# EdwardSmith1884/GEOMetrics

Measured on AMD Instinct MI355X. Metric: meshes/sec (sample+Chamfer+tri_dist+0N-GCN fwd+bwd), 2562 verts/3000 pts, higher is better.
Workload: dtype f32; 1 GPU; BASELINE config 5 shard: 8 independent 2562-vert/5120-face meshes per GPU, full loss (face sampling 3000 pts + Chamfer NN vs 3000 GT pts + tri_distance 3000x5120 + point-to-surface) on top of a 3-layer 0N-GCN 963-192-192-192, fwd+bwd, single process (no collective), Adam step; meshes_per_gpu=8, global_batch=8, parallelism=dp1, launch=hipgraph, gemm_selection=tunableop file

## Files before the change

geometrics_amd/aggregation.py:

```python
import torch
import torch.nn.functional as F

from . import _lib
from . import backward_pass as _pass
from . import fused as _fused
from .products import _new_like

ACT_NONE, ACT_RELU, ACT_ELU = 0, 1, 2


def activation_code(activation):
    if activation is F.relu or activation is torch.relu:
        return ACT_RELU
    if activation is F.elu:
        return ACT_ELU
    return ACT_NONE


def relu_mask(s, k):
    words = _lib.lib().geom_zn_gcn_relu_mask_words(*s.shape, k)
    return torch.empty(words, dtype=torch.int16, device=s.device) if words else None


def _table(csr, transposed):
    col, val, over = (csr.ell_col_t, csr.ell_val_t, csr.over_t) if transposed else (csr.ell_col, csr.ell_val, csr.over)
    return (csr.ell_w, _lib.ptr(col), _lib.ptr(val)) + tuple(map(_lib.ptr, over or (None, None, None)))


def _table_took(csr, name, *args):
    code = _lib.status(name, *args) if csr.ell_w else _lib.EUNSUPPORTED
    if code != _lib.EUNSUPPORTED:
        _lib.check(code, name)
    return code != _lib.EUNSUPPORTED


def forward(s, bias_c, csr, k, act, out, want_mask=False, head=None):
    b, nv, c = s.shape
    mask = relu_mask(s, k) if want_mask and act == ACT_RELU and csr.ell_w else None
    operands = (s.data_ptr(), _lib.ptr(bias_c), act, out.data_ptr())
    with torch.cuda.device(s.device):
        if head is not None:
            base, scale, pos = head
            _lib.call("geom_zn_gcn_aggregate_ell_head_fwd_f32", b, nv, c, k, *_table(csr, False), *operands, _lib.ptr(mask),
                      base.data_ptr(), float(scale), pos.data_ptr())
        elif not _table_took(csr, "geom_zn_gcn_aggregate_ell_fwd_f32", b, nv, c, k, *_table(csr, False), *operands, _lib.ptr(mask)):
            mask = None
            _lib.call("geom_zn_gcn_aggregate_fwd_f32", b, nv, c, k, csr.rowptr.data_ptr(), csr.col.data_ptr(), csr.val.data_ptr(),
                      *operands)
    return mask


def takes_product_below(below, csr, c, k, rows, needs_support):
    return bool(below is not None and below.wt is not None and below.wanted and needs_support and _fused.plan(rows)["bwd"]
                and below.wt.dim() == 2 and below.wt.shape[0] == c and _fused.supported(csr, c, k, below.wt.shape[1]))


def backward(g, csr, k, act, out, mask, want_bias, bias=None, arena=None, head=None, below=None):
    grad_pos, scale, (b, nv, c) = head if head is not None else (None, 0.0, g.shape)
    device = g.device if head is None else grad_pos.device
    grad_support = _new_like(g, "grad_support", arena, descending=True) if head is None \
        else torch.empty(b, nv, c, dtype=torch.float32, device=device)
    rows = _fused.partial_rows(b, nv) if below is not None else None
    bg = _pass.NO_BIAS_GRADIENT
    if want_bias:
        scratch = (rows, c) if below is not None else _lib.lib().geom_zn_gcn_bwd_scratch_floats(b, nv, c)
        bg = _pass.bias_gradient(bias, c, device, scratch, opted_in=arena is not None)
    ell_w = csr.ell_w
    results = (grad_support.data_ptr(), _lib.ptr(bg.now), _lib.ptr(bg.scratch))
    with torch.cuda.device(device):
        if below is not None:
            _fused.layer_backward(g, out, mask, csr, k, act, below.wt, g_out=grad_support, grad_in=below.take_dx(b, nv),
                                  colsum_partial=bg.scratch, grad_pos=grad_pos, head_scale=scale, shape=(b, nv, c))
            below.stamp(grad_support)
        elif head is not None:
            _lib.call("geom_zn_gcn_aggregate_ell_head_bwd_f32", b, nv, c, k, *_table(csr, True), grad_pos.data_ptr(), scale,
                      _lib.ptr(mask), act, *results)
        elif not _table_took(csr, "geom_zn_gcn_aggregate_ell_bwd_f32", b, nv, c, k, *_table(csr, True), g.data_ptr(), _lib.ptr(out),
                             _lib.ptr(mask), act, *results):
            ell_w = 0
            _lib.call("geom_zn_gcn_aggregate_bwd_f32", b, nv, c, k, csr.rowptr_t.data_ptr(), csr.col_t.data_ptr(),
                      csr.val_t.data_ptr(), g.data_ptr(), _lib.ptr(out), act, *results)
    if below is not None:
        bg.finish(rows)
    elif bg.defer:
        bg.finish(int(_lib.lib().geom_zn_gcn_bwd_partial_rows(b, nv, c, k, ell_w)))
    return grad_support, bg.out


def narrow_head_forward(s, bias_c, csr, k, act, base, scale, pos, want_sign):
    b, nv, c = s.shape
    sign = torch.empty(b * nv, dtype=torch.int16, device=s.device) if want_sign and act == ACT_RELU else None
    with torch.cuda.device(s.device):
        _lib.call("geom_zn_gcn_narrow_head_fwd_f32", b, nv, c, k, *_table(csr, False), s.data_ptr(), _lib.ptr(bias_c), act,
                  base.data_ptr(), float(scale), pos.data_ptr(), _lib.ptr(sign))
    return sign


def narrow_head_backward(grad_pos, scale, sign, csr, k, act, shape, want_bias, bias=None):
    b, nv, c = shape
    gs4 = torch.empty(b * nv, 4, dtype=torch.float32, device=grad_pos.device)
    rows = int(_lib.lib().geom_zn_gcn_bwd_partial_rows(b, nv, c, k, csr.ell_w))
    bg = _pass.bias_gradient(bias, c, grad_pos.device, (rows, c)) if want_bias else _pass.NO_BIAS_GRADIENT
    with torch.cuda.device(grad_pos.device):
        _lib.call("geom_zn_gcn_narrow_head_bwd_f32", b, nv, c, k, *_table(csr, True), grad_pos.data_ptr(), float(scale),
                  _lib.ptr(sign), act, gs4.data_ptr(), _lib.ptr(bg.scratch))
    bg.finish(rows)
    return gs4, bg.out
```

geometrics_amd/backward_pass.py:

```python
import contextlib
import ctypes
import threading
import types
import weakref
from collections import namedtuple

import torch

from . import _lib
from . import dense as _dense_kernels


_DEFAULTS = {"defer": False,
             "late": False,
             "collect": None}
switches = types.SimpleNamespace(
    ready_hooks=[],
    optimizer=None,
    zero_fill=False,
    **_DEFAULTS)
_entered = []
_entered_lock = threading.Lock()


@contextlib.contextmanager
def _switched(**values):
    with _entered_lock:
        _entered.append(values)
        _apply()
    try:
        yield
    finally:
        with _entered_lock:
            del _entered[next(i for i, entry in enumerate(_entered) if entry is values)]
            _apply()


def _apply():
    current = dict(_DEFAULTS)
    for values in _entered:
        current.update(values)
    for name, value in current.items():
        setattr(switches, name, value)


def deferred_parameter_gradients(enabled=True):
    return _switched(defer=enabled)


@contextlib.contextmanager
def late_input_gradients(on_parameter_gradients=None, enabled=True, collect=None):
    hooks = [on_parameter_gradients] if on_parameter_gradients is not None else []
    switches.ready_hooks.extend(hooks)
    try:
        with _switched(late=enabled, collect=collect):
            yield
    finally:
        for hook in hooks:
            switches.ready_hooks.remove(hook)


def set_optimizer(opt):
    prev, switches.optimizer = switches.optimizer, opt
    return prev


_gradient_targets = {}


def bind_gradient_targets(params, tensors):
    for p, t in zip(params, tensors):
        key = id(p)
        if t is None:
            _gradient_targets.pop(key, None)
            continue
        if t.shape != p.shape or t.dtype != p.dtype or t.device != p.device or not t.is_contiguous():
            raise ValueError("a gradient target must match its parameter's shape, dtype and device and be contiguous")
        _gradient_targets[key] = (weakref.ref(p, lambda _r, k=key: _gradient_targets.pop(k, None)), t)


def _gradient_buffer(param, like):
    hit = _gradient_targets.get(id(param)) if param is not None else None
    if (hit is not None and hit[0]() is param and hit[1].shape == like.shape and param.grad is None
            and _user_count(param) <= 1):
        return hit[1].detach()
    return torch.zeros_like(like) if switches.zero_fill else torch.empty_like(like)


_users = {}


def parameter_ref(param, node, needs_grad):
    if param is None:
        return None
    if needs_grad:
        key = id(param)
        entry = _users.get(key)
        if entry is None or entry[0]() is not param:
            entry = _users[key] = (weakref.ref(param, lambda _ref, k=key: _users.pop(k, None)), weakref.WeakSet())
        entry[1].add(node)
    return weakref.ref(param)


def _user_count(param):
    entry = _users.get(id(param))
    return len(entry[1]) if entry is not None and entry[0]() is param else 0


def _alias(t):
    return torch.empty(0, dtype=t.dtype, device=t.device).set_(t.untyped_storage(), t.storage_offset(), t.size(), t.stride())


def _engine_pass():
    return (hasattr(torch._C, "_current_graph_task_id") and torch._C._current_graph_task_id() >= 0
            and not torch.is_grad_enabled())


def may_defer(param, opted_in=False):
    if not (switches.defer or opted_in) or param is None or not _engine_pass():
        return False
    if not param.is_leaf or _user_count(param) > 1:
        return False
    return param.grad is None and not param._backward_hooks and not getattr(param, "_post_accumulate_grad_hooks", None)


def may_postpone_input_gradient(x):
    if not (switches.late and switches.defer) or not _engine_pass():
        return False
    return x.is_leaf and not x._backward_hooks and not getattr(x, "_post_accumulate_grad_hooks", None)


def _check_landed(param_ref, out):
    param = param_ref() if param_ref is not None else None
    if param is None or param.grad is None or param.grad.data_ptr() == out.data_ptr():
        return
    if param.grad.shape == out.shape or param.grad.numel() == out.numel():
        param.grad.copy_(out.view_as(param.grad))
    else:
        raise RuntimeError("geometrics_amd: a deferred parameter gradient did not reach its parameter (shape %s vs %s)"
                           % (tuple(param.grad.shape), tuple(out.shape)))


_Colsum = namedtuple("_Colsum", "partials rows cols out stream param")
_Reduce = namedtuple("_Reduce", "rows cin c workspace out stream param")
_Product = namedtuple("_Product", "x g out stream param launch_run")
_Late = namedtuple("_Late", "launch out stream leaf")


class _Pass:
    __slots__ = ("colsums", "reduces", "products", "late")

    def __init__(self):
        self.colsums, self.reduces, self.products, self.late = [], [], [], []

    def finish(self):
        colsums, reduces, self.colsums, self.reduces = self.colsums, self.reduces, [], []
        streams = {job.stream for job in colsums + reduces}
        if (reduces and colsums and len(streams) == 1 and all(job.cols % 4 == 0 for job in colsums)
                and 2 * len(reduces) + len(colsums) <= _lib.DENSE_MAX_REDUCE_JOBS):
            _launch_joint(reduces, colsums, streams.pop())
        else:
            _launch_colsums(colsums)
            _launch_reduces(reduces)
        products, self.products = self.products[::-1], []
        if products:
            products[0].launch_run(products)
        for job in reduces + colsums + products:
            _check_landed(job.param, job.out)
        for hook in list(switches.ready_hooks):
            hook()
        late, self.late, launches = self.late, [], []
        for job in late:
            launches.append(_on_stream(job.stream, job.launch))
            x = job.leaf()
            if x is not None and x.grad is None:
                x.grad = job.out.view(x.shape)
            elif x is not None:
                launches.append(_on_stream(job.stream, lambda x=x, out=job.out: x.grad.add_(out.view_as(x.grad))))
        if switches.collect is not None:
            switches.collect.extend(launches)
        else:
            for launch in launches:
                launch()


def _on_stream(stream, fn):
    def launch():
        with torch.cuda.stream(stream), torch.no_grad():
            fn()
    return launch


def _ints(seq):
    return (ctypes.c_int * len(seq))(*seq)


def _ptrs(tensors):
    return (ctypes.c_void_p * len(tensors))(*[t.data_ptr() for t in tensors])


def _colsum_args(jobs):
    return (len(jobs), _ptrs([j.partials for j in jobs]), _ints([j.rows for j in jobs]), _ints([j.cols for j in jobs]),
            _ptrs([j.out for j in jobs]))


def _by_stream(jobs):
    groups = {}
    for job in jobs:
        groups.setdefault(job.stream, []).append(job)
    return groups.items()


def _launch_colsums(jobs):
    for stream, group in _by_stream(jobs):
        with torch.cuda.device(stream.device):
            for c0 in range(0, len(group), _lib.COLSUM_MAX_JOBS):
                _lib.check(_lib.status("geom_colsum_batch_f32", *_colsum_args(group[c0:c0 + _lib.COLSUM_MAX_JOBS]),
                                       stream=stream.cuda_stream), "geom_colsum_batch_f32")


def _launch_reduces(jobs):
    for stream, group in _by_stream(jobs):
        _dense_kernels.reduce([(j.rows, j.cin, j.c, j.workspace, j.out, None) for j in group], stream.cuda_stream)


def _launch_joint(reduces, colsums, stream):
    weights = (len(reduces), _ints([j.rows for j in reduces]), _ints([j.cin for j in reduces]), _ints([j.c for j in reduces]),
               _ptrs([j.workspace for j in reduces]), _ptrs([j.out for j in reduces]))
    biases = _colsum_args(colsums)
    opt = switches.optimizer
    slots = None
    if opt is not None:
        index = {id(p): k for k, p in enumerate(opt.params)}
        slots = [index.get(id(job.param())) if job.param is not None else None for job in reduces + colsums]
        if None in slots or sorted(slots) != list(range(len(opt.params))) or opt.params[0].device != stream.device:
            slots = None
    with torch.cuda.device(stream.device):
        if slots is None:
            _lib.check(_lib.status("geom_dense_reduce2_f32", *weights, None, *biases, stream=stream.cuda_stream),
                       "geom_dense_reduce2_f32")
        else:
            pick = lambda seq, ks: _ptrs([seq[k] for k in ks])
            wk, bk = slots[:len(reduces)], slots[len(reduces):]
            params = [p.data for p in opt.params]
            _lib.check(_lib.status(
                "geom_dense_reduce_adam_f32",
                *weights, pick(params, wk), pick(opt.exp_avg, wk), pick(opt.exp_avg_sq, wk),
                *biases, pick(params, bk), pick(opt.exp_avg, bk), pick(opt.exp_avg_sq, bk), float(opt.lr), float(opt.betas[0]),
                float(opt.betas[1]), float(opt.eps), opt.state.data_ptr(), stream=stream.cuda_stream), "geom_dense_reduce_adam_f32")
            opt._stepped_in_backward = True


_passes = {}
_passes_lock = threading.Lock()


def _current():
    task = torch._C._current_graph_task_id()
    with _passes_lock:
        record = _passes.get(task)
        if record is not None:
            return record
        for stale in [t for t in _passes if t < task - 64]:
            del _passes[stale]
        record = _passes[task] = _Pass()
    torch.autograd.Variable._execution_engine.queue_callback(lambda: _finish(task, record))
    return record


def _finish(task, record):
    try:
        record.finish()
    finally:
        with _passes_lock:
            _passes.pop(task, None)


def pending(*kinds):
    with _passes_lock:
        return sum(len(getattr(record, kind)) for record in _passes.values() for kind in kinds or _Pass.__slots__)


class BiasGradient(namedtuple("BiasGradient", "out scratch defer bias")):
    __slots__ = ()

    @property
    def now(self):
        return None if self.defer else self.out

    def finish(self, rows):
        if self.out is None:
            return
        stream = torch.cuda.current_stream(self.out.device)
        if self.defer:
            _current().colsums.append(_Colsum(self.scratch, rows, self.out.shape[0], _alias(self.out), stream, weakref.ref(self.bias)))
        else:
            _launch_colsums([_Colsum(self.scratch, rows, self.out.shape[0], self.out, stream, None)])


NO_BIAS_GRADIENT = BiasGradient(None, None, False, None)


def bias_gradient(bias, c, device, scratch_shape, opted_in=False):
    out = _gradient_buffer(bias, bias) if bias is not None and bias.shape == (c,) and bias.dtype == torch.float32 \
        else torch.empty(c, dtype=torch.float32, device=device)
    scratch = torch.empty(scratch_shape, dtype=torch.float32, device=device)
    return BiasGradient(out, scratch, may_defer(bias, opted_in), bias)


def weight_gradient(param_ref, w, rows, cin, c, workspace):
    param = param_ref()
    out = _gradient_buffer(param, w)
    if may_defer(param):
        stream = torch.cuda.current_stream(w.device)
        _current().reduces.append(_Reduce(rows, cin, c, workspace, _alias(out).view(cin, c), stream, param_ref))
    else:
        _dense_kernels.reduce([(rows, cin, c, workspace, out.view(cin, c), None)])
    return out


def postpone_weight_product(x, g, out, param_ref, launch_run):
    _current().products.append(_Product(x, g, _alias(out).view(x.shape[1], g.shape[1]), torch.cuda.current_stream(out.device),
                                        param_ref, launch_run))


def postpone_input_gradient(launch, out, leaf):
    _current().late.append(_Late(launch, out, torch.cuda.current_stream(out.device), weakref.ref(leaf)))
```

geometrics_amd/csrc/dense_gemm.hip:

```cpp
#include "buffer_access.h"
#include "adam_math.h"
#include <type_traits>

namespace {

using geom::f32x4;
using geom::f3u;
typedef float f32x2 __attribute__((ext_vector_type(2)));
struct __attribute__((packed, aligned(4))) f4u { float x, y, z, w; };

constexpr int DG_THREADS = 256;
constexpr int DG_WAVES = 4;
constexpr int DG_BK = 32;
constexpr int DG_KS = 8;
constexpr int SPLIT_RB = 6;
constexpr int SPLIT_RB_NARROW = 3;
constexpr int LD_TC = 34;

__host__ __device__ constexpr int ld_rc(int r) { return ((r + 15) / 32) * 32 + 16; }

#ifndef DG_PROBE_NO_FETCH
#define DG_PROBE_NO_FETCH 0
#endif
#ifndef DG_PROBE_NO_ISSUE
#define DG_PROBE_NO_ISSUE 0
#endif
#ifndef DG_PROBE_NO_STORE
#define DG_PROBE_NO_STORE 0
#endif
#ifndef DG_PROBE_NO_BARRIER
#define DG_PROBE_NO_BARRIER 0
#endif
#ifndef DG_PROBE_NO_G
#define DG_PROBE_NO_G 0
#endif
constexpr bool DG_FETCH = !DG_PROBE_NO_FETCH, DG_ISSUE = !DG_PROBE_NO_ISSUE, DG_STORE = !DG_PROBE_NO_STORE,
               DG_BARRIER = !DG_PROBE_NO_BARRIER, DG_G = !DG_PROBE_NO_G;


template <int W>
using ldg_t = std::conditional_t<W == 4, f32x4, std::conditional_t<W == 3, f3u, float>>;
template <int W>
__device__ __forceinline__ ldg_t<W> ldg(const float *base, unsigned byte_off)
{
    const char *p = reinterpret_cast<const char *>(base) + byte_off;
    if constexpr (W == 4) {
        const f4u v = *reinterpret_cast<const f4u *>(p);
        return (f32x4){v.x, v.y, v.z, v.w};
    } else {
        return *reinterpret_cast<const ldg_t<W> *>(p);
    }
}

template <int R, int W>
struct PanelTC {
    static constexpr int WIDTH = W, TPR = 32 / W, ROWS = DG_THREADS / TPR;
    static constexpr int PASSES = (R + ROWS - 1) / ROWS;
    static constexpr bool EXACT = R % ROWS == 0;
    static_assert(W == 4 || EXACT, "the 4-byte form covers whole passes");
    ldg_t<W> v[2][PASSES];
    unsigned off[PASSES];
    template <typename RowOff>
    __device__ __forceinline__ void prepare(RowOff rowoff, unsigned )
    {
#pragma unroll
        for (int p = 0; p < PASSES; ++p) {
            const int r = p * ROWS + threadIdx.x / TPR;
            off[p] = ((unsigned)rowoff(W == 1 || r < R ? r : R - 1) + (threadIdx.x % TPR) * W) * 4u;
        }
    }
    static __device__ __forceinline__ const float *stage_base(const float *g, unsigned , int t0) { return g + t0; }
    static __device__ __forceinline__ unsigned stage_limit(unsigned total, unsigned , int t0) { return (total - W - (unsigned)t0) * 4u; }
    template <int SET>
    __device__ __forceinline__ void issue_pass(int p, const float *base, unsigned limit) { v[SET][p] = ldg<W>(base, min(off[p], limit)); }
    template <bool ZERO, int SET>
    __device__ __forceinline__ void store_pass(int p, float *lds, int t0, int tmax) const
    {
        const int tl = (threadIdx.x % TPR) * W;
        const int r = p * ROWS + threadIdx.x / TPR;
        if (EXACT || r < R) {
            const bool tin = !ZERO || t0 + tl < tmax;
            float *d = lds + r * LD_TC + tl;
            if constexpr (W == 4) {
                reinterpret_cast<float2 *>(d)[0] = make_float2(tin ? v[SET][p][0] : 0.f, tin ? v[SET][p][1] : 0.f);
                reinterpret_cast<float2 *>(d)[1] = make_float2(tin ? v[SET][p][2] : 0.f, tin ? v[SET][p][3] : 0.f);
            } else {
                *d = tin ? v[SET][p] : 0.f;
            }
        }
    }
};

template <int R, int W>
struct PanelRC {
    static constexpr int WIDTH = W, Q = R / W;
    static constexpr int PASSES = (32 * Q + DG_THREADS - 1) / DG_THREADS;
    static constexpr bool EXACT = (32 * Q) % DG_THREADS == 0;
    ldg_t<W> v[2][PASSES];
    unsigned off[PASSES];
    template <typename ColOff>
    __device__ __forceinline__ void prepare(ColOff coloff, unsigned ld)
    {
#pragma unroll
        for (int p = 0; p < PASSES; ++p) {
            const int e = threadIdx.x + p * DG_THREADS;
            const int tl = EXACT ? e / Q : min(e / Q, 31);
            off[p] = ((unsigned)tl * ld + (unsigned)coloff((e % Q) * W)) * 4u;
        }
    }
    static __device__ __forceinline__ const float *stage_base(const float *g, unsigned ld, int t0) { return g + (int64_t)t0 * ld; }
    static __device__ __forceinline__ unsigned stage_limit(unsigned total, unsigned ld, int t0) { return (total - W - (unsigned)t0 * ld) * 4u; }
    template <int SET>
    __device__ __forceinline__ void issue_pass(int p, const float *base, unsigned limit) { v[SET][p] = ldg<W>(base, min(off[p], limit)); }
    template <bool ZERO, int SET>
    __device__ __forceinline__ void store_pass(int p, float *lds, int t0, int tmax) const
    {
        const int e = threadIdx.x + p * DG_THREADS;
        const int tl = EXACT ? e / Q : min(e / Q, 31);
        ldg_t<W> x = v[SET][p];
        if (ZERO && !(t0 + tl < tmax)) x = ldg_t<W>{};
        *reinterpret_cast<ldg_t<W> *>(lds + tl * ld_rc(R) + (e % Q) * W) = x;
    }
};

template <int RB, int NCW, bool EXTRA>
struct Frags {
    float a[2][RB + 1], b[2][NCW + 1];
};

template <int RB, int NCW, bool A_TC, bool B_TC, int RA, int RBW, bool EXTRA>
__device__ __forceinline__ void fetch_frags(Frags<RB, NCW, EXTRA> &f, int buf, const float *la, const float *lb, int s, int wave,
                                            int xcb)
{
    const int x = threadIdx.x & 15, g = (threadIdx.x >> 4) & 3;
    const float *pa = A_TC ? la + x * LD_TC + g : la + g * ld_rc(RA) + x;
    const float *pb = B_TC ? lb + (wave * NCW * 16 + x) * LD_TC + g : lb + g * ld_rc(RBW) + wave * NCW * 16 + x;
#pragma unroll
    for (int i = 0; i < RB; ++i) f.a[buf][i] = A_TC ? pa[i * 16 * LD_TC + 4 * s] : pa[4 * s * ld_rc(RA) + i * 16];
#pragma unroll
    for (int j = 0; j < NCW; ++j) f.b[buf][j] = B_TC ? pb[j * 16 * LD_TC + 4 * s] : pb[4 * s * ld_rc(RBW) + j * 16];
    if (EXTRA) {
        const float *pbx = B_TC ? lb + (xcb * 16 + x) * LD_TC + g : lb + g * ld_rc(RBW) + xcb * 16 + x;
        f.a[buf][RB] = A_TC ? pa[RB * 16 * LD_TC + 4 * s] : pa[4 * s * ld_rc(RA) + RB * 16];
        f.b[buf][NCW] = B_TC ? pbx[4 * s] : pbx[4 * s * ld_rc(RBW)];
    }
}

struct StageIO {
    int st_t0, st_tmax;
    const float *a_base, *b_base;
    unsigned a_limit, b_limit;
};

template <int RB, int NCW, bool A_TC, bool B_TC, int RA, int RBW, bool EXTRA, int A_FLOATS, int SET, class PA, class PB, class Tail>
__device__ __forceinline__ void gemm_stage(const float *cur, float *wr, f32x4 (&acc)[RB][NCW], f32x4 &accx,
                                           Frags<RB, NCW, EXTRA> &f, PA &pa, PB &pb, const StageIO &io, int wave, int xcb,
                                           Tail tail)
{
    constexpr int U = PA::PASSES + PB::PASSES;
#pragma unroll
    for (int s = 0; s < DG_KS; ++s) {
        if (DG_FETCH && s + 1 < DG_KS) fetch_frags<RB, NCW, A_TC, B_TC, RA, RBW, EXTRA>(f, (s + 1) & 1, cur, cur + A_FLOATS, s + 1, wave, xcb);
        else if (DG_FETCH) fetch_frags<RB, NCW, A_TC, B_TC, RA, RBW, EXTRA>(f, 0, wr, wr + A_FLOATS, 0, wave, xcb);
        if (DG_ISSUE && s < 4) {
#pragma unroll
            for (int u = s * U / 4; u < (s + 1) * U / 4; ++u) {
                if (u < PA::PASSES) pa.template issue_pass<SET>(u, io.a_base, io.a_limit);
                else pb.template issue_pass<SET>(u - PA::PASSES, io.b_base, io.b_limit);
            }
        } else if (DG_STORE && s >= 4 && s < 7) {
#pragma unroll
            for (int u = (s - 4) * U / 3; u < (s - 3) * U / 3; ++u) {
                if (u < PA::PASSES) pa.template store_pass<true, SET ^ 1>(u, wr, io.st_t0, io.st_tmax);
                else pb.template store_pass<false, SET ^ 1>(u - PA::PASSES, wr + A_FLOATS, io.st_t0, io.st_tmax);
            }
        }
        if (s == DG_KS - 1) tail();
#pragma unroll
        for (int i = 0; i < RB; ++i)
#pragma unroll
            for (int j = 0; j < NCW; ++j)
                acc[i][j] = __builtin_amdgcn_mfma_f32_16x16x4f32(f.b[s & 1][j], f.a[s & 1][i], acc[i][j], 0, 0, 0);
        if (EXTRA) accx = __builtin_amdgcn_mfma_f32_16x16x4f32(f.b[s & 1][NCW], f.a[s & 1][RB], accx, 0, 0, 0);
#pragma unroll
        for (int m = 0; m < RB * NCW + (EXTRA ? 1 : 0); ++m) {
            __builtin_amdgcn_sched_group_barrier(0x008, 1, 0);
            __builtin_amdgcn_sched_group_barrier(0x100, 1, 0);
            if (s < 4) __builtin_amdgcn_sched_group_barrier(0x020, 1, 0);
            else __builtin_amdgcn_sched_group_barrier(0x200, 1, 0);
            __builtin_amdgcn_sched_group_barrier(0x006, 2, 0);
        }
        __builtin_amdgcn_sched_barrier(0);
        if (s == 6) {
            if (DG_BARRIER) __syncthreads();
            __builtin_amdgcn_sched_barrier(0);
        }
    }
}

enum { EPI_PLAIN = 0, EPI_ZN = 1 };

struct RowArgs {
    const float *a;
    int64_t lda;
    const float *b;
    int64_t ldb;
    float *c;
    int64_t ldc;
    int I, J, T;
    int n_tiles;
    int left_rb;
    int n_chunks;
    int ksplit;
    float *sup;
    const float *bias;
    unsigned short *mask;
};

template <int RB, int NCW, bool B_TC, bool A_VEC, int EPI, bool HAS_X>
__device__ __forceinline__ void rows_body(const RowArgs &q, float *lds, const int w, const int G)
{
    constexpr int RA = (RB + 1) * 16;
    constexpr int RAL = HAS_X ? RA : RB * 16;
    constexpr int CW = NCW * 64;
    constexpr int A_FLOATS = RA * LD_TC;
    constexpr int B_FLOATS = B_TC ? CW * LD_TC : 32 * ld_rc(CW);
    constexpr int BUF = A_FLOATS + B_FLOATS;
    const int wave = threadIdx.x >> 6;
    const int xrow0 = HAS_X ? (q.n_tiles * RB + w / NCW) * 16 : 0;
    const int xcb = (w % NCW) * DG_WAVES + wave;
    const int nst = (q.T + DG_BK - 1) / DG_BK;
    int my_tiles = w < q.n_tiles ? (q.n_tiles - 1 - w) / G + 1 : 0;
    if (my_tiles == 0 && HAS_X) my_tiles = 1;
    const int total = my_tiles * q.n_chunks * nst;
    if (total == 0) return;

    typedef PanelTC<RAL, A_VEC ? 4 : 1> PA;
    typedef typename std::conditional<B_TC, PanelTC<CW, 4>, PanelRC<CW, 4>>::type PB;
    PA pa;
    PB pb;
    const unsigned a_total = (unsigned)q.I * (unsigned)q.lda;
    const unsigned b_total = B_TC ? (unsigned)q.J * (unsigned)q.ldb : (unsigned)q.T * (unsigned)q.ldb;
    int l_tile = w, l_chunk = 0, l_st = 0, l_count = 0;
    auto prepare_a = [&]() {
        const int tile = l_tile;
        pa.prepare([=](int r) -> unsigned {
            int row = r < RB * 16 ? (tile < q.n_tiles ? tile : 0) * RB * 16 + r : xrow0 + (r - RB * 16);
            row = row < q.I ? row : q.I - 1;
            return (unsigned)row * (unsigned)q.lda;
        }, (unsigned)q.lda);
    };
    auto prepare_b = [&]() {
        const int j0 = l_chunk * CW;
        if constexpr (B_TC) {
            pb.prepare([=](int r) -> unsigned { const int j = j0 + r; return (unsigned)(j < q.J ? j : q.J - 1) * (unsigned)q.ldb; }, (unsigned)q.ldb);
        } else {
            pb.prepare([=](int r) -> unsigned { const int j = j0 + r; return (unsigned)(j < q.J ? j : q.J - 4); }, (unsigned)q.ldb);
        }
    };
    StageIO io;
    auto aim = [&]() {
        io.a_base = PA::stage_base(q.a, (unsigned)q.lda, l_st * DG_BK);
        io.a_limit = PA::stage_limit(a_total, (unsigned)q.lda, l_st * DG_BK);
        io.b_base = PB::stage_base(q.b, (unsigned)q.ldb, l_st * DG_BK);
        io.b_limit = PB::stage_limit(b_total, (unsigned)q.ldb, l_st * DG_BK);
    };
    bool wrapped = false;
    auto step = [&]() {
        const int more = l_count + 1 < total ? 1 : 0;
        l_count += more;
        const int nl = l_st + more;
        wrapped = nl == nst;
        l_st = wrapped ? 0 : nl;
    };
    auto rewire = [&]() {
        if (!wrapped) return;
        if (++l_chunk == q.n_chunks) {
            l_chunk = 0, l_tile += G;
            prepare_a();
        }
        if (q.n_chunks > 1) prepare_b();
    };
    auto advance = [&]() { step(); rewire(); };
    prepare_a();
    prepare_b();
    aim();
#pragma unroll
    for (int p = 0; p < PA::PASSES; ++p) pa.template issue_pass<0>(p, io.a_base, io.a_limit);
#pragma unroll
    for (int p = 0; p < PB::PASSES; ++p) pb.template issue_pass<0>(p, io.b_base, io.b_limit);
    advance();
    aim();
    io.st_t0 = l_st * DG_BK;
#pragma unroll
    for (int p = 0; p < PA::PASSES; ++p) pa.template issue_pass<1>(p, io.a_base, io.a_limit);
#pragma unroll
    for (int p = 0; p < PB::PASSES; ++p) pb.template issue_pass<1>(p, io.b_base, io.b_limit);
#pragma unroll
    for (int p = 0; p < PA::PASSES; ++p) pa.template store_pass<true, 0>(p, lds, 0, q.T);
#pragma unroll
    for (int p = 0; p < PB::PASSES; ++p) pb.template store_pass<false, 0>(p, lds + A_FLOATS, 0, q.T);
    advance();
    aim();
    io.st_tmax = q.T;
    __syncthreads();
    Frags<RB, NCW, HAS_X> fr;
    fetch_frags<RB, NCW, true, B_TC, RA, CW, HAS_X>(fr, 0, lds, lds + A_FLOATS, 0, wave, xcb);

    const int x = threadIdx.x & 15, g = (threadIdx.x >> 4) & 3;
    f32x4 acc[RB][NCW], accx = {0.f, 0.f, 0.f, 0.f};
#pragma unroll
    for (int i = 0; i < RB; ++i)
#pragma unroll
        for (int j = 0; j < NCW; ++j) acc[i][j] = (f32x4){0.f, 0.f, 0.f, 0.f};
    int c_tile = w, c_chunk = 0, c_st = 0, c_pass = 0;
    int buf = 0;

    auto after_stage = [&]() {
        rewire();
        if (++c_st < nst) return;
        c_st = 0;
        const int j0 = c_chunk * CW;
        auto emit = [&](const f32x4 &val, int row, int cb) {
            const int j = j0 + cb * 16 + 4 * g;
            if (row >= q.I || j >= q.J) return;
            f32x4 v = val;
            if (EPI == EPI_ZN) {
                if (j < q.ksplit) {
                    *reinterpret_cast<f32x4 *>(q.sup + (int64_t)row * q.ksplit + j) = v;
                    return;
                }
                const f32x4 bb = q.bias ? *reinterpret_cast<const f32x4 *>(q.bias + j) : (f32x4){0.f, 0.f, 0.f, 0.f};
                unsigned bits = 0u;
#pragma unroll
                for (int r = 0; r < 4; ++r) {
                    const float t = v[r] + bb[r];
                    v[r] = t > 0.f ? t : 0.f;
                    bits |= (t > 0.f ? 1u : 0u) << r;
                }
                if (q.mask) {
                    unsigned m = bits << (4 * g);
                    m |= __shfl_xor(m, 16);
                    m |= __shfl_xor(m, 32);
                    if (g == 0) q.mask[(int64_t)row * (q.J >> 4) + (j >> 4)] = (unsigned short)m;
                }
            }
            float *dst = q.c + (int64_t)row * q.ldc + j;
            if (j + 3 < q.J) {
                *reinterpret_cast<f4u *>(dst) = f4u{v[0], v[1], v[2], v[3]};
            } else {
#pragma unroll
                for (int r = 0; r < 4; ++r)
                    if (j + r < q.J) dst[r] = v[r];
            }
        };
        if (c_tile < q.n_tiles) {
#pragma unroll
            for (int i = 0; i < RB; ++i)
#pragma unroll
                for (int jj = 0; jj < NCW; ++jj) emit(acc[i][jj], (c_tile * RB + i) * 16 + x, wave * NCW + jj);
        }
        if (HAS_X && c_pass == 0) emit(accx, xrow0 + x, xcb);
#pragma unroll
        for (int i = 0; i < RB; ++i)
#pragma unroll
            for (int jj = 0; jj < NCW; ++jj) acc[i][jj] = (f32x4){0.f, 0.f, 0.f, 0.f};
        accx = (f32x4){0.f, 0.f, 0.f, 0.f};
        if (++c_chunk == q.n_chunks) c_chunk = 0, c_tile += G, ++c_pass;
    };

    for (int it = 0; it < total; it += 2) {
        {
            const float *cur = lds + buf * BUF;
            float *wr = lds + (buf ^ 1) * BUF;
            gemm_stage<RB, NCW, true, B_TC, RA, CW, HAS_X, A_FLOATS, 0>(cur, wr, acc, accx, fr, pa, pb, io, wave, xcb, [&]() {
                io.st_t0 = l_st * DG_BK;
                step();
                aim();
                buf ^= 1;
            });
            after_stage();
        }
        if (it + 1 < total) {
            const float *cur = lds + buf * BUF;
            float *wr = lds + (buf ^ 1) * BUF;
            gemm_stage<RB, NCW, true, B_TC, RA, CW, HAS_X, A_FLOATS, 1>(cur, wr, acc, accx, fr, pa, pb, io, wave, xcb, [&]() {
                io.st_t0 = l_st * DG_BK;
                step();
                aim();
                buf ^= 1;
            });
            after_stage();
        }
    }
}

template <int RB, int NCW, bool B_TC, bool A_VEC, int EPI>
__global__ __launch_bounds__(DG_THREADS) void dense_rows_kernel(RowArgs q)
{
    constexpr int RA = (RB + 1) * 16;
    constexpr int CW = NCW * 64;
    __shared__ __attribute__((aligned(16))) float lds[2 * (RA * LD_TC + (B_TC ? CW * LD_TC : 32 * ld_rc(CW)))];
    if ((int)blockIdx.x < q.left_rb * NCW) rows_body<RB, NCW, B_TC, A_VEC, EPI, true>(q, lds, blockIdx.x, gridDim.x);
    else rows_body<RB, NCW, B_TC, A_VEC, EPI, false>(q, lds, blockIdx.x, gridDim.x);
}

struct SplitArgs {
    const float *a;
    int64_t lda;
    const float *b;
    int64_t ldb;
    float *part;
    int I, J, T;
    int full_tiles, s_full, left_rb, s_left;
    float *colsum;
};

template <int RB>
__device__ __forceinline__ int split_row(int i, int x)
{
    constexpr int N4 = RB / 4, N2 = (RB % 4) / 2;
    if (i < 4 * N4) return 64 * (i >> 2) + 4 * x + (i & 3);
    if (i < 4 * N4 + 2 * N2) return 64 * N4 + 2 * x + (i - 4 * N4);
    return 64 * N4 + 32 * N2 + x;
}

template <int RB>
__device__ __forceinline__ void split_frags(float (&f)[RB], const float *row, int x)
{
    constexpr int N4 = RB / 4, N2 = (RB % 4) / 2, N1 = RB % 2;
#pragma unroll
    for (int q = 0; q < N4; ++q) {
        const f32x4 v = *reinterpret_cast<const f32x4 *>(row + 64 * q + 4 * x);
        f[4 * q] = v[0], f[4 * q + 1] = v[1], f[4 * q + 2] = v[2], f[4 * q + 3] = v[3];
    }
    if constexpr (N2 == 1) {
        const f32x2 v = *reinterpret_cast<const f32x2 *>(row + 64 * N4 + 2 * x);
        f[4 * N4] = v[0], f[4 * N4 + 1] = v[1];
    }
    if constexpr (N1 == 1) f[RB - 1] = row[64 * N4 + 32 * N2 + x];
}

template <int RB, int RA, int A_FLOATS, int SET, class PA, class Tail>
__device__ __forceinline__ void split_stage(const float *cur, float *wr, f32x4 (&acc)[RB][3], float (&fa)[2][RB], f3u (&bq)[2][DG_KS],
                                            PA &pa, const StageIO &io, unsigned b_lane, unsigned b_step, Tail tail)
{
    constexpr int U = PA::PASSES;
    constexpr int KS = DG_KS;
    constexpr int LOADS = KS / 2;
    constexpr int STORES = KS - 1 - LOADS;
    const int x = threadIdx.x & 15, g = (threadIdx.x >> 4) & 3;
    const float *b_base = io.b_base;
    const unsigned b_limit = io.b_limit;
#pragma unroll
    for (int s = 0; s < KS; ++s) {
        if (DG_FETCH) {
            const float *src = s + 1 < KS ? cur : wr;
            const int sn = s + 1 < KS ? s + 1 : 0;
            split_frags<RB>(fa[(s + 1) & 1], src + (4 * sn + g) * ld_rc(RA), x);
        }
        if (DG_ISSUE && s < LOADS) {
#pragma unroll
            for (int u = s * U / LOADS; u < (s + 1) * U / LOADS; ++u) pa.template issue_pass<SET>(u, io.a_base, io.a_limit);
        } else if (DG_STORE && s >= LOADS && s < KS - 1) {
#pragma unroll
            for (int u = (s - LOADS) * U / STORES; u < (s - LOADS + 1) * U / STORES; ++u)
                pa.template store_pass<true, SET ^ 1>(u, wr, io.st_t0, io.st_tmax);
        }
        if (s == KS - 1) tail();
        const f3u b = bq[SET][s];
#pragma unroll
        for (int i = 0; i < RB; ++i) {
            acc[i][0] = __builtin_amdgcn_mfma_f32_16x16x4f32(b.x, fa[s & 1][i], acc[i][0], 0, 0, 0);
            acc[i][1] = __builtin_amdgcn_mfma_f32_16x16x4f32(b.y, fa[s & 1][i], acc[i][1], 0, 0, 0);
            acc[i][2] = __builtin_amdgcn_mfma_f32_16x16x4f32(b.z, fa[s & 1][i], acc[i][2], 0, 0, 0);
        }
        if (DG_G) bq[SET][s] = ldg<3>(b_base, min(b_lane + (unsigned)s * b_step, b_limit));
#pragma unroll
        for (int m = 0; m < RB * 3; ++m) {
            __builtin_amdgcn_sched_group_barrier(0x008, 1, 0);
            __builtin_amdgcn_sched_group_barrier(0x100, 1, 0);
            if (s < LOADS) __builtin_amdgcn_sched_group_barrier(0x020, 1, 0);
            else __builtin_amdgcn_sched_group_barrier(0x200, 1, 0);
            __builtin_amdgcn_sched_group_barrier(0x006, 2, 0);
        }
        __builtin_amdgcn_sched_barrier(0);
        if (s == KS - 2) {
            if (DG_BARRIER) __syncthreads();
            __builtin_amdgcn_sched_barrier(0);
        }
    }
}

template <int RB, int RBP, bool A_VEC>
__device__ __forceinline__ void split_body(const SplitArgs &q, float *lds, int i0, int split, int nsplit, int slot, bool want_cs)
{
    constexpr int RA = RB * 16;
    constexpr int CW = 192;
    constexpr int A_FLOATS = 32 * ld_rc(RA);
    constexpr int BUF = A_FLOATS;
    constexpr int KS = DG_KS;
    const int wave = threadIdx.x >> 6;
    const int x = threadIdx.x & 15, g = (threadIdx.x >> 4) & 3;
    const int n4 = (q.T + 3) / 4;
    const int t_begin = (int)((int64_t)n4 * split / nsplit) * 4;
    const int t_end = min((int)((int64_t)n4 * (split + 1) / nsplit) * 4, q.T);
    const int nst = (t_end - t_begin + DG_BK - 1) / DG_BK;

    f32x4 acc[RB][3];
#pragma unroll
    for (int i = 0; i < RB; ++i)
#pragma unroll
        for (int j = 0; j < 3; ++j) acc[i][j] = (f32x4){0.f, 0.f, 0.f, 0.f};
    float cs0 = 0.f, cs1 = 0.f, cs2 = 0.f;

    typedef PanelRC<RA, A_VEC ? 4 : 1> PA;
    PA pa;
    if (nst > 0) {
        pa.prepare([=](int r) -> unsigned { const int i = i0 + r; return (unsigned)(i + PA::WIDTH - 1 < q.I ? i : q.I - PA::WIDTH); }, (unsigned)q.lda);
        const unsigned a_total = (unsigned)q.T * (unsigned)q.lda, b_total = (unsigned)q.T * (unsigned)q.ldb;
        const int jc = min(wave * 48 + 3 * x, q.J - 3);
        const unsigned b_step = 4u * (unsigned)q.ldb * 4u;
        const unsigned b_lane = ((unsigned)g * (unsigned)q.ldb + (unsigned)jc) * 4u;
        StageIO io;
        int l_st = 0;
        auto aim = [&]() {
            const int t0 = t_begin + l_st * DG_BK;
            io.a_base = PA::stage_base(q.a, (unsigned)q.lda, t0);
            io.a_limit = PA::stage_limit(a_total, (unsigned)q.lda, t0);
            io.b_base = q.b + (int64_t)t0 * q.ldb;
            io.b_limit = (b_total - 3u - (unsigned)t0 * (unsigned)q.ldb) * 4u;
        };
        auto advance = [&]() { l_st = l_st + 1 < nst ? l_st + 1 : l_st; };
        f3u bq[2][KS];
        float fa[2][RB];
        aim();
#pragma unroll
        for (int p = 0; p < PA::PASSES; ++p) pa.template issue_pass<0>(p, io.a_base, io.a_limit);
#pragma unroll
        for (int s = 0; s < KS; ++s) bq[0][s] = ldg<3>(io.b_base, min(b_lane + (unsigned)s * b_step, io.b_limit));
        advance();
        aim();
        io.st_t0 = t_begin + l_st * DG_BK;
#pragma unroll
        for (int p = 0; p < PA::PASSES; ++p) pa.template issue_pass<1>(p, io.a_base, io.a_limit);
#pragma unroll
        for (int s = 0; s < KS; ++s) bq[1][s] = ldg<3>(io.b_base, min(b_lane + (unsigned)s * b_step, io.b_limit));
#pragma unroll
        for (int p = 0; p < PA::PASSES; ++p) pa.template store_pass<true, 0>(p, lds, t_begin, t_end);
        advance();
        aim();
        io.st_tmax = t_end;
        __syncthreads();
        split_frags<RB>(fa[0], lds + g * ld_rc(RA), x);
        int buf = 0;
        auto tail = [&]() {
            io.st_t0 = t_begin + l_st * DG_BK;
            advance();
            aim();
            buf ^= 1;
        };
        auto colsum_stage = [&](const f3u (&b)[KS], int st) {
            const int t0 = t_begin + st * DG_BK + g;
#pragma unroll
            for (int s = 0; s < KS; ++s) {
                const bool in = t0 + 4 * s < t_end;
                cs0 += in ? b[s].x : 0.f, cs1 += in ? b[s].y : 0.f, cs2 += in ? b[s].z : 0.f;
            }
        };
        for (int st = 0; st < nst; st += 2) {
            {
                const float *cur = lds + buf * BUF;
                float *wr = lds + (buf ^ 1) * BUF;
                if (want_cs) colsum_stage(bq[0], st);
                split_stage<RB, RA, A_FLOATS, 0>(cur, wr, acc, fa, bq, pa, io, b_lane, b_step, tail);
            }
            if (st + 1 < nst) {
                const float *cur = lds + buf * BUF;
                float *wr = lds + (buf ^ 1) * BUF;
                if (want_cs) colsum_stage(bq[1], st + 1);
                split_stage<RB, RA, A_FLOATS, 1>(cur, wr, acc, fa, bq, pa, io, b_lane, b_step, tail);
            }
        }
    }
    float *dst = q.part + (int64_t)slot * (RBP * 16) * CW;
    const int j0 = wave * 48 + 12 * g;
#pragma unroll
    for (int i = 0; i < RB; ++i) {
        float e[12];
#pragma unroll
        for (int r = 0; r < 4; ++r)
#pragma unroll
            for (int u = 0; u < 3; ++u) e[3 * r + u] = acc[i][u][r];
        f32x4 *d = reinterpret_cast<f32x4 *>(dst + split_row<RB>(i, x) * CW + j0);
        d[0] = (f32x4){e[0], e[1], e[2], e[3]};
        d[1] = (f32x4){e[4], e[5], e[6], e[7]};
        d[2] = (f32x4){e[8], e[9], e[10], e[11]};
    }
    if (want_cs) {
        float t0 = cs0, t1 = cs1, t2 = cs2;
#pragma unroll
        for (int k = 1; k < 4; ++k) {
            t0 += __shfl(cs0, x + 16 * k), t1 += __shfl(cs1, x + 16 * k), t2 += __shfl(cs2, x + 16 * k);
        }
        const int j = wave * 48 + 3 * x;
        if (g == 0 && j + 2 < q.J) {
            float *o = q.colsum + (int64_t)split * q.J + j;
            o[0] = t0, o[1] = t1, o[2] = t2;
        }
    }
}

template <int RB, int NCW, bool A_VEC>
__device__ __forceinline__ void split_dispatch(const SplitArgs &q, float *lds, const int w)
{
    static_assert(NCW == 3, "the split body owns 48 columns per wave");
    const int nfull = q.full_tiles * q.s_full;
    if (w < nfull) {
        const int tile = w % q.full_tiles, split = w / q.full_tiles;
        split_body<RB, RB, true>(q, lds, tile * RB * 16, split, q.s_full, tile * q.s_full + split, q.colsum != nullptr && tile == 0);
    } else {
        const int e = (w - nfull) / q.s_left, split = (w - nfull) % q.s_left;
        split_body<1, RB, A_VEC>(q, lds, (q.full_tiles * RB + e) * 16, split, q.s_left, w, false);
    }
}

template <int RB, int NCW, bool A_VEC>
__global__ __launch_bounds__(DG_THREADS) void dense_split_kernel(SplitArgs q)
{
    __shared__ __attribute__((aligned(16))) float lds[2 * 32 * ld_rc(RB * 16)];
    split_dispatch<RB, NCW, A_VEC>(q, lds, blockIdx.x);
}

template <int RB, int SRB, bool X_VEC>
__global__ __launch_bounds__(DG_THREADS, 2) void dense_bwd_pair_kernel(RowArgs r, SplitArgs q, int n_row)
{
    constexpr int LDS_ROWS = 2 * ((RB + 1) * 16 * LD_TC + 192 * LD_TC);
    constexpr int LDS_SPLIT = 2 * 32 * ld_rc(SRB * 16);
    __shared__ __attribute__((aligned(16))) float lds[LDS_ROWS > LDS_SPLIT ? LDS_ROWS : LDS_SPLIT];
    const int w = blockIdx.x;
    if (w < n_row) {
        if (w < r.left_rb * 3) rows_body<RB, 3, true, true, EPI_PLAIN, true>(r, lds, w, n_row);
        else rows_body<RB, 3, true, true, EPI_PLAIN, false>(r, lds, w, n_row);
    } else {
        split_dispatch<SRB, 3, X_VEC>(q, lds, w - n_row);
    }
}

constexpr int NP_CW = 192;
constexpr int NP_RA = SPLIT_RB_NARROW * 16;
constexpr int NP_CHUNK = 128;
constexpr int NP_DX_ROWS = 64;
struct NarrowPairArgs {
    const float *x;
    const float *g4;
    const float *w;
    float *grad_x;
    float *part;
    int rows, full_tiles, s_full;
};

__device__ __forceinline__ void narrow_dw_role(const NarrowPairArgs &q, const int w)
{
    constexpr int XP = NP_CHUNK * (NP_RA / 4) / DG_THREADS;
    static_assert(NP_CHUNK * (NP_RA / 4) % DG_THREADS == 0 && NP_CHUNK <= DG_THREADS, "whole staging passes");
    __shared__ __attribute__((aligned(16))) float xs[2][NP_CHUNK * NP_RA];
    __shared__ f32x4 gs[2][NP_CHUNK];
    const int tid = threadIdx.x;
    const int tile = w % q.full_tiles, split = w / q.full_tiles;
    const int slot = tile * q.s_full + split, i0 = tile * NP_RA;
    const int n4 = (q.rows + 3) / 4;
    const int t_begin = (int)((int64_t)n4 * split / q.s_full) * 4;
    const int t_end = min((int)((int64_t)n4 * (split + 1) / q.s_full) * 4, q.rows);
    const int nch = (t_end - t_begin + NP_CHUNK - 1) / NP_CHUNK;
    float *dst = q.part + (int64_t)slot * NP_RA * NP_CW;

    f32x4 xr[XP], gr = {0.f, 0.f, 0.f, 0.f};
    auto load = [&](int ch) {
        const int t0 = t_begin + ch * NP_CHUNK;
#pragma unroll
        for (int p = 0; p < XP; ++p) {
            const int e = p * DG_THREADS + tid;
            const int t = min(t0 + e / (NP_RA / 4), q.rows - 1);
            xr[p] = *reinterpret_cast<const f32x4 *>(q.x + (int64_t)t * NP_CW + i0 + (e % (NP_RA / 4)) * 4);
        }
        if (tid < NP_CHUNK) gr = *reinterpret_cast<const f32x4 *>(q.g4 + (int64_t)min(t0 + tid, q.rows - 1) * 4);
    };
    if (nch > 0) load(0);
    for (int e = tid; e < NP_RA * (NP_CW / 4); e += DG_THREADS)
        if (e % (NP_CW / 4) != 0) *reinterpret_cast<f32x4 *>(dst + (int64_t)e * 4) = (f32x4){0.f, 0.f, 0.f, 0.f};
    float a0 = 0.f, a1 = 0.f, a2 = 0.f;
    for (int ch = 0; ch < nch; ++ch) {
        const int buf = ch & 1;
#pragma unroll
        for (int p = 0; p < XP; ++p) {
            const int e = p * DG_THREADS + tid;
            *reinterpret_cast<f32x4 *>(&xs[buf][(e / (NP_RA / 4)) * NP_RA + (e % (NP_RA / 4)) * 4]) = xr[p];
        }
        if (tid < NP_CHUNK) gs[buf][tid] = gr;
        __syncthreads();
        if (ch + 1 < nch) load(ch + 1);
        if (tid < NP_RA) {
            const int n = min(NP_CHUNK, t_end - (t_begin + ch * NP_CHUNK));
#pragma unroll 8
            for (int t = 0; t < n; ++t) {
                const float xv = xs[buf][t * NP_RA + tid];
                const f32x4 gv = gs[buf][t];
                a0 = __builtin_fmaf(xv, gv[0], a0);
                a1 = __builtin_fmaf(xv, gv[1], a1);
                a2 = __builtin_fmaf(xv, gv[2], a2);
            }
        }
    }
    if (tid < NP_RA) *reinterpret_cast<f32x4 *>(dst + (int64_t)tid * NP_CW) = (f32x4){a0, a1, a2, 0.f};
}

__device__ __forceinline__ void narrow_dx_role(const NarrowPairArgs &q, const int w)
{
    constexpr int GROUPS = NP_CW / 4;
    constexpr int PASSES = NP_DX_ROWS * GROUPS / DG_THREADS;
    constexpr int CLASSES = 3;
    static_assert((DG_THREADS * CLASSES) % GROUPS == 0 && PASSES % CLASSES == 0, "the column groups of a thread repeat every 3 passes");
    const int tid = threadIdx.x;
    const int64_t row0 = (int64_t)w * NP_DX_ROWS;
    float wr[CLASSES][4][3];
#pragma unroll
    for (int cl = 0; cl < CLASSES; ++cl) {
        const int cg = (cl * DG_THREADS + tid) % GROUPS;
#pragma unroll
        for (int i = 0; i < 4; ++i) {
            const f32x4 v = *reinterpret_cast<const f32x4 *>(q.w + (int64_t)(4 * cg + i) * NP_CW);
            wr[cl][i][0] = v[0], wr[cl][i][1] = v[1], wr[cl][i][2] = v[2];
        }
    }
#pragma unroll
    for (int p = 0; p < PASSES; ++p) {
        const int e = p * DG_THREADS + tid;
        const int64_t row = row0 + e / GROUPS;
        const int cg = e % GROUPS;
        if (row < q.rows) {
            const f32x4 gv = *reinterpret_cast<const f32x4 *>(q.g4 + row * 4);
            f32x4 o;
#pragma unroll
            for (int i = 0; i < 4; ++i) {
                const float *wi = wr[p % CLASSES][i];
                o[i] = __builtin_fmaf(gv[2], wi[2], __builtin_fmaf(gv[1], wi[1], __builtin_fmaf(gv[0], wi[0], 0.f)));
            }
            *reinterpret_cast<f32x4 *>(q.grad_x + row * NP_CW + 4 * cg) = o;
        }
    }
}

__global__ __launch_bounds__(DG_THREADS) void dense_bwd_narrow_kernel(NarrowPairArgs q, int n_split)
{
    const int w = blockIdx.x;
    if (w < n_split) narrow_dw_role(q, w);
    else narrow_dx_role(q, w - n_split);
}

struct ReduceJob {
    const float *part;
    float *out;
    int I, J, RA, CW, full_tiles, s_full, s_left;
    int outs;
};
struct ReduceJobs {
    ReduceJob job[GEOM_DENSE_MAX_REDUCE_JOBS];
    int first[GEOM_DENSE_MAX_REDUCE_JOBS + 1];
    int n;
};
struct ReduceAdam {
    float *p[GEOM_DENSE_MAX_REDUCE_JOBS], *m[GEOM_DENSE_MAX_REDUCE_JOBS], *v[GEOM_DENSE_MAX_REDUCE_JOBS];
    float lr, b1, b2, eps;
    float *state;
    int vec;
};

constexpr int RED_THREADS = 256;
inline int reduce_outs(int slots) { return slots <= 32 ? 64 : slots <= 64 ? 32 : slots <= 128 ? 16 : slots <= 256 ? 8 : 4; }
__device__ __forceinline__ void reduce_body(const ReduceJobs &jobs, const ReduceAdam &adam, const int block, const int nblocks,
                                            f32x4 *part, float *st)
{
    float *const state = adam.state;
    int jb = 0;
    while (jb + 1 < jobs.n && block >= jobs.first[jb + 1]) ++jb;
    const ReduceJob q = jobs.job[jb];
    const int bx = block - jobs.first[jb];
    const int jq = q.J >> 2;
    const int outs = q.outs, groups = RED_THREADS / outs;
    float s_t = 0.f, s_b1 = 0.f, s_b2 = 0.f;
    if (state && threadIdx.x == 0) {
        s_t = __hip_atomic_load(state + 0, __ATOMIC_RELAXED, __HIP_MEMORY_SCOPE_AGENT);
        s_b1 = __hip_atomic_load(state + 1, __ATOMIC_RELAXED, __HIP_MEMORY_SCOPE_AGENT);
        s_b2 = __hip_atomic_load(state + 2, __ATOMIC_RELAXED, __HIP_MEMORY_SCOPE_AGENT);
    }
    const int o = threadIdx.x % outs, sg = threadIdx.x / outs;
    const int e = bx * outs + o;
    const bool live = e < q.I * jq;
    f32x4 t = {0.f, 0.f, 0.f, 0.f};
    int i = 0, j = 0;
    if (live) {
        i = e / jq, j = (e % jq) * 4;
        int tile = i / q.RA, il = i % q.RA;
        const bool full = tile < q.full_tiles;
        const int n = full ? q.s_full : q.s_left;
        int slot0 = tile * q.s_full;
        if (!full) {
            const int r = i - q.full_tiles * q.RA;
            slot0 = q.full_tiles * q.s_full + (r >> 4) * q.s_left, il = r & 15;
        }
        const int64_t pitch = (int64_t)q.RA * q.CW;
        const float *p = q.part + ((int64_t)slot0 * q.RA + il) * q.CW + j;
        const int s0 = (int)((int64_t)n * sg / groups), s1 = (int)((int64_t)n * (sg + 1) / groups);
        for (int s = s0; s < s1; s += 8) {
            f32x4 a[8];
#pragma unroll
            for (int k = 0; k < 8; ++k)
                if (s + k < s1) a[k] = *reinterpret_cast<const f32x4 *>(p + (int64_t)(s + k) * pitch);
#pragma unroll
            for (int k = 0; k < 8; ++k)
                if (s + k < s1) t = t + a[k];
        }
    }
    const int64_t at = (int64_t)i * q.J + j;
    float *pp = state ? adam.p[jb] : nullptr;
    const bool vec = pp && adam.vec;
    f32x4 a = {0.f, 0.f, 0.f, 0.f}, bm = a, cv = a;
    if (vec && sg == 0 && live) {
        a = *reinterpret_cast<const f32x4 *>(pp + at);
        bm = *reinterpret_cast<const f32x4 *>(adam.m[jb] + at);
        cv = *reinterpret_cast<const f32x4 *>(adam.v[jb] + at);
    }
    part[sg * outs + o] = t;
    if (state && threadIdx.x == 0) st[0] = s_t, st[1] = s_b1, st[2] = s_b2;
    __syncthreads();
    geom::AdamStep as{};
    if (state) as = geom::adam_step_from(st, adam.lr, adam.b1, adam.b2);
    if (sg == 0 && live) {
        f32x4 r = part[o];
        for (int k = 1; k < groups; ++k) r = r + part[k * outs + o];
        float *dst = q.out + at;
        if (vec) {
            f32x4 *p4 = reinterpret_cast<f32x4 *>(pp + at), *m4 = reinterpret_cast<f32x4 *>(adam.m[jb] + at),
                  *v4 = reinterpret_cast<f32x4 *>(adam.v[jb] + at);
#pragma unroll
            for (int k = 0; k < 4; ++k) {
                float pa = a[k], pb = bm[k], pc = cv[k];
                geom::adam_update(pa, r[k], pb, pc, adam.b1, adam.b2, adam.eps, 1.f, as.step_size, as.bc2_sqrt);
                a[k] = pa, bm[k] = pb, cv[k] = pc;
            }
            *reinterpret_cast<f32x4 *>(dst) = r;
            *m4 = bm, *v4 = cv, *p4 = a;
        } else {
            dst[0] = r[0], dst[1] = r[1], dst[2] = r[2], dst[3] = r[3];
            if (pp) {
                float *pm = adam.m[jb] + at, *pv = adam.v[jb] + at;
                pp += at;
#pragma unroll
                for (int k = 0; k < 4; ++k) {
                    float a = pp[k], b = pm[k], c = pv[k];
                    geom::adam_update(a, r[k], b, c, adam.b1, adam.b2, adam.eps, 1.f, as.step_size, as.bc2_sqrt);
                    pm[k] = b, pv[k] = c, pp[k] = a;
                }
            }
        }
    }
    if (state) geom::adam_arrive(state, as, block, nblocks);
}

__global__ __launch_bounds__(RED_THREADS) void dense_reduce_kernel(ReduceJobs jobs, ReduceAdam adam)
{
    __shared__ f32x4 part[RED_THREADS];
    __shared__ float st[3];
    reduce_body(jobs, adam, blockIdx.x, gridDim.x, part, st);
}


int num_cus()
{
    static int cus = 0;
    if (!cus) {
        int dev = 0;
        hipDeviceProp_t prop;
        if (hipGetDevice(&dev) == hipSuccess && hipGetDeviceProperties(&prop, dev) == hipSuccess) cus = prop.multiProcessorCount;
        if (cus <= 0) cus = 256;
    }
    return cus;
}

struct RowGeo {
    int rb, n_tiles, left_rb, grid;
};
RowGeo row_geometry(int rows, int ncw, int cus)
{
    const int n_rb = (rows + 15) / 16;
    RowGeo best{0, 0, 0, 0};
    long best_cost = -1;
    const int cand[] = {5, 6, 4, 3, 2, 1};
    for (int rb : cand) {
        int n_tiles = n_rb / rb, left = n_rb % rb;
        if (left * ncw > cus || (n_tiles == 0 && left == 0)) continue;
        const int grid = n_tiles < cus ? (n_tiles > left * ncw ? n_tiles : left * ncw) : cus;
        if (grid <= 0) continue;
        const int passes = (n_tiles + grid - 1) / grid;
        const long cost = (long)(passes > 0 ? passes : 1) * rb * ncw + (left ? 1 : 0);
        if (best_cost < 0 || cost < best_cost) best = RowGeo{rb, n_tiles, left, grid}, best_cost = cost;
    }
    return best;
}

template <int LO, int HI, class Launch>
int dispatch_rb(int rb, Launch launch)
{
    if constexpr (LO <= HI) {
        if (rb != LO) return dispatch_rb<LO + 1, HI>(rb, launch);
        launch(std::integral_constant<int, LO>{});
        return geom::launch_status();
    } else {
        return GEOM_EINVAL;
    }
}

template <int NCW, bool B_TC, bool A_VEC, int EPI>
int launch_rows_rb(const RowArgs &q, const RowGeo &geo, hipStream_t s)
{
    return dispatch_rb<1, 6>(geo.rb, [&](auto rb) {
        hipLaunchKernelGGL((dense_rows_kernel<decltype(rb)::value, NCW, B_TC, A_VEC, EPI>), dim3(geo.grid), dim3(DG_THREADS), 0, s, q);
    });
}

inline bool aligned16(const void *p) { return ((uintptr_t)p & 15) == 0; }

RowArgs input_gradient_args(int rows, int cin, int c, const float *g, const float *w, float *grad_x, int ncw, const RowGeo &geo)
{
    return RowArgs{g, c, w, c, grad_x, cin, rows, cin, c, geo.n_tiles, geo.left_rb, (cin + ncw * 64 - 1) / (ncw * 64), 0, nullptr,
                   nullptr, nullptr};
}

struct SplitGeo {
    int rb, full_tiles, left_rb, s_full, s_left, slots;
    int64_t partial_floats() const { return (int64_t)slots * rb * 16 * 192; }
    int64_t colsum_offset() const { return partial_floats(); }
};
inline int split_rb(int cin) { return cin <= 192 ? SPLIT_RB_NARROW : SPLIT_RB; }
SplitGeo split_geometry(int cin, int rows, int cus)
{
    SplitGeo g;
    g.rb = split_rb(cin);
    const int ra = g.rb * 16;
    g.full_tiles = cin / ra;
    g.left_rb = (cin % ra + 15) / 16;
    const int n4 = (rows + 3) / 4;
    g.s_full = g.full_tiles ? (int)((int64_t)cus * g.rb / (g.full_tiles * g.rb + g.left_rb)) : 0;
    if (g.full_tiles && g.s_full < 1) g.s_full = 1;
    g.s_left = 0;
    if (g.left_rb) {
        const int rest = cus - g.full_tiles * g.s_full;
        g.s_left = rest / g.left_rb > 0 ? rest / g.left_rb : 1;
    }
    if (g.s_full > n4) g.s_full = n4;
    if (g.s_left > n4) g.s_left = n4;
    g.slots = g.full_tiles * g.s_full + g.left_rb * g.s_left;
    return g;
}

SplitArgs split_args(int rows, int cin, int c, const float *x, const float *g, float *workspace, bool want_colsum, const SplitGeo &geo)
{
    return SplitArgs{x, cin, g, c, workspace, cin, c, rows, geo.full_tiles, geo.s_full, geo.left_rb, geo.s_left,
                     want_colsum ? workspace + geo.colsum_offset() : nullptr};
}

int check_backward(bool dx, bool dw, int rows, int cin, int c, const float *x, const float *g, const float *w, const float *grad_x,
                   const float *workspace)
{
    if (rows < (dw ? 1 : 0) || cin <= 0 || c <= 0) return GEOM_EINVAL;
    if ((dw ? c % 12 != 0 || c > 192 : c % 4 != 0) || (int64_t)rows * (cin > c ? cin : c) >= (1LL << 30)) return GEOM_EUNSUPPORTED;
    if (rows == 0) return 0;
    if (!g || !aligned16(g)) return GEOM_EINVAL;
    if (dx && (!w || !grad_x || !aligned16(w))) return GEOM_EINVAL;
    if (dw && (!x || !workspace || !aligned16(workspace))) return GEOM_EINVAL;
    return 0;
}

}

extern "C" int geom_dense_fwd_f32(int rows, int cin, int c, const float *x, const float *w, int ksplit, const float *bias,
                                  float *out, float *sup, uint16_t *mask, void *stream)
{
    if (rows < 0 || cin <= 0 || c <= 0) return GEOM_EINVAL;
    if (c % 16 != 0 || c > 192 || (int64_t)rows * cin >= (1LL << 30)) return GEOM_EUNSUPPORTED;
    if (rows == 0) return 0;
    if (!x || !w || !out || !aligned16(w) || !aligned16(out)) return GEOM_EINVAL;
    const bool zn = ksplit > 0;
    if (zn && (ksplit % 16 != 0 || ksplit >= c || !sup || !aligned16(sup) || (bias && !aligned16(bias)))) return GEOM_EINVAL;
    const RowGeo geo = row_geometry(rows, 3, num_cus());
    RowArgs q{x, cin, w, c, out, c, rows, c, cin, geo.n_tiles, geo.left_rb, 1, zn ? ksplit : 0, sup, bias, mask};
    hipStream_t s = static_cast<hipStream_t>(stream);
    const bool avec = cin % 4 == 0 && aligned16(x);
    if (zn) return avec ? launch_rows_rb<3, false, true, EPI_ZN>(q, geo, s) : launch_rows_rb<3, false, false, EPI_ZN>(q, geo, s);
    return avec ? launch_rows_rb<3, false, true, EPI_PLAIN>(q, geo, s) : launch_rows_rb<3, false, false, EPI_PLAIN>(q, geo, s);
}

extern "C" int geom_dense_bwd_input_f32(int rows, int cin, int c, const float *g, const float *w, float *grad_x, void *stream)
{
    const int code = check_backward(true, false, rows, cin, c, nullptr, g, w, grad_x, nullptr);
    if (code || rows == 0) return code;
    hipStream_t s = static_cast<hipStream_t>(stream);
    const int ncw = cin > 192 ? 4 : 3;
    const RowGeo geo = row_geometry(rows, ncw, num_cus());
    const RowArgs q = input_gradient_args(rows, cin, c, g, w, grad_x, ncw, geo);
    return ncw == 4 ? launch_rows_rb<4, true, true, EPI_PLAIN>(q, geo, s) : launch_rows_rb<3, true, true, EPI_PLAIN>(q, geo, s);
}

extern "C" int64_t geom_dense_bwd_weight_workspace_floats(int rows, int cin, int c)
{
    if (rows <= 0 || cin <= 0 || c <= 0 || c > 192) return 0;
    const SplitGeo g = split_geometry(cin, rows, num_cus());
    return g.partial_floats() + (int64_t)(g.s_full > 0 ? g.s_full : g.s_left) * c;
}

extern "C" int geom_dense_bwd_weight_f32(int rows, int cin, int c, const float *x, const float *g, float *workspace,
                                         int want_colsum, void *stream)
{
    const int code = check_backward(false, true, rows, cin, c, x, g, nullptr, nullptr, workspace);
    if (code) return code;
    const SplitGeo geo = split_geometry(cin, rows, num_cus());
    if (want_colsum && geo.full_tiles == 0) return GEOM_EUNSUPPORTED;
    const SplitArgs q = split_args(rows, cin, c, x, g, workspace, want_colsum != 0, geo);
    const dim3 grid(geo.slots), block(DG_THREADS);
    hipStream_t s = static_cast<hipStream_t>(stream);
    const bool xvec = cin % 4 == 0 && aligned16(x);
    if (geo.rb == SPLIT_RB_NARROW) {
        if (xvec) hipLaunchKernelGGL((dense_split_kernel<SPLIT_RB_NARROW, 3, true>), grid, block, 0, s, q);
        else hipLaunchKernelGGL((dense_split_kernel<SPLIT_RB_NARROW, 3, false>), grid, block, 0, s, q);
    } else {
        if (xvec) hipLaunchKernelGGL((dense_split_kernel<SPLIT_RB, 3, true>), grid, block, 0, s, q);
        else hipLaunchKernelGGL((dense_split_kernel<SPLIT_RB, 3, false>), grid, block, 0, s, q);
    }
    return geom::launch_status();
}

extern "C" int geom_dense_bwd_f32(int rows, int cin, int c, const float *x, const float *g, const float *w, float *grad_x,
                                  float *workspace, int want_colsum, void *stream)
{
    int code = check_backward(true, true, rows, cin, c, x, g, w, grad_x, workspace);
    if (code) return code;
    const int cus = num_cus();
    const bool xvec = cin % 4 == 0 && aligned16(x);
    const RowGeo rg = row_geometry(rows, 3, cus);
    const SplitGeo sg = split_geometry(cin, rows, cus);
    if (cin > 192 || !xvec || (want_colsum && sg.full_tiles == 0) || rg.rb < 2 || rg.rb > 5) {
        code = geom_dense_bwd_input_f32(rows, cin, c, g, w, grad_x, stream);
        if (code) return code;
        return geom_dense_bwd_weight_f32(rows, cin, c, x, g, workspace, want_colsum, stream);
    }
    const RowArgs r = input_gradient_args(rows, cin, c, g, w, grad_x, 3, rg);
    const SplitArgs q = split_args(rows, cin, c, x, g, workspace, want_colsum != 0, sg);
    hipStream_t s = static_cast<hipStream_t>(stream);
    static_assert(SPLIT_RB_NARROW == 3, "cin <= 192 (the pair mode's range) takes the narrow split tiles");
    return dispatch_rb<2, 5>(rg.rb, [&](auto rb) {
        hipLaunchKernelGGL((dense_bwd_pair_kernel<decltype(rb)::value, SPLIT_RB_NARROW, true>), dim3(rg.grid + sg.slots),
                           dim3(DG_THREADS), 0, s, r, q, rg.grid);
    });
}

extern "C" int geom_dense_bwd_narrow_f32(int rows, int cin, int c, const float *x, const float *g4, const float *w, float *grad_x,
                                         float *workspace, void *stream)
{
    if (rows < 1 || cin <= 0 || c <= 0) return GEOM_EINVAL;
    if (cin != NP_CW || c != NP_CW || (int64_t)rows * NP_CW >= (1LL << 30)) return GEOM_EUNSUPPORTED;
    if (!x || !g4 || !workspace || !aligned16(x) || !aligned16(g4) || !aligned16(workspace)) return GEOM_EINVAL;
    if (grad_x && (!w || !aligned16(w) || !aligned16(grad_x))) return GEOM_EINVAL;
    const SplitGeo sg = split_geometry(cin, rows, num_cus());
    if (sg.rb != SPLIT_RB_NARROW || sg.left_rb != 0 || sg.full_tiles < 1) return GEOM_EUNSUPPORTED;
    const NarrowPairArgs q{x, g4, w, grad_x, workspace, rows, sg.full_tiles, sg.s_full};
    const int n_dx = grad_x ? (rows + NP_DX_ROWS - 1) / NP_DX_ROWS : 0;
    hipLaunchKernelGGL(dense_bwd_narrow_kernel, dim3(sg.slots + n_dx), dim3(DG_THREADS), 0, static_cast<hipStream_t>(stream), q, sg.slots);
    return geom::launch_status();
}

namespace {
void flat_grid(ReduceJobs &jobs, int n)
{
    jobs.n = n;
    jobs.first[0] = 0;
    for (int j = 0; j < n; ++j) {
        ReduceJob &q = jobs.job[j];
        q.outs = reduce_outs(q.s_full > q.s_left ? q.s_full : q.s_left);
        jobs.first[j + 1] = jobs.first[j] + (q.I * (q.J >> 2) + q.outs - 1) / q.outs;
    }
}

inline bool bad_layer(const float *workspace, const float *grad_w, int rows, int cin, int c)
{
    return !workspace || !grad_w || rows <= 0 || cin <= 0 || c <= 0 || c > 192 || c % 4;
}

int build_reduce_jobs(ReduceJobs &jobs, int count, const int *rows, const int *cin, const int *c, const float *const *workspaces,
                      float *const *grad_w, int ncs, const float *const *cs_partials, const int *cs_rows, const int *cs_cols,
                      float *const *cs_outs)
{
    if (count < 0 || ncs < 0) return GEOM_EINVAL;
    if (count && (!rows || !cin || !c || !workspaces || !grad_w)) return GEOM_EINVAL;
    if (ncs && (!cs_partials || !cs_rows || !cs_cols || !cs_outs)) return GEOM_EINVAL;
    if (count + ncs > GEOM_DENSE_MAX_REDUCE_JOBS) return GEOM_ETOOBIG;
    int n = 0;
    for (int l = 0; l < count; ++l) {
        if (bad_layer(workspaces[l], grad_w[l], rows[l], cin[l], c[l])) return GEOM_EINVAL;
        const SplitGeo g = split_geometry(cin[l], rows[l], num_cus());
        jobs.job[n++] = ReduceJob{workspaces[l], grad_w[l], cin[l], c[l], g.rb * 16, 192, g.full_tiles, g.s_full, g.s_left, 0};
    }
    for (int i = 0; i < ncs; ++i) {
        if (!cs_partials[i] || !cs_outs[i] || cs_rows[i] < 0 || cs_cols[i] <= 0 || cs_cols[i] % 4) return GEOM_EINVAL;
        jobs.job[n++] = ReduceJob{cs_partials[i], cs_outs[i], 1, cs_cols[i], 1, cs_cols[i], 1, cs_rows[i], 0, 0};
    }
    flat_grid(jobs, n);
    return 0;
}

int launch_reduce(const ReduceJobs &jobs, const ReduceAdam &adam, void *stream)
{
    hipLaunchKernelGGL(dense_reduce_kernel, dim3(jobs.first[jobs.n]), dim3(RED_THREADS), 0, static_cast<hipStream_t>(stream), jobs, adam);
    return geom::launch_status();
}
}

extern "C" int geom_dense_reduce2_f32(int count, const int *rows, const int *cin, const int *c, const float *const *workspaces,
                                      float *const *grad_w, float *const *grad_bias, int ncs, const float *const *cs_partials,
                                      const int *cs_rows, const int *cs_cols, float *const *cs_outs, void *stream)
{
    if (grad_bias) return GEOM_EINVAL;
    if (count + ncs == 0) return 0;
    ReduceJobs jobs;
    const int code = build_reduce_jobs(jobs, count, rows, cin, c, workspaces, grad_w, ncs, cs_partials, cs_rows, cs_cols, cs_outs);
    return code ? code : launch_reduce(jobs, ReduceAdam{}, stream);
}

extern "C" int geom_dense_reduce_adam_f32(int count, const int *rows, const int *cin, const int *c,
                                          const float *const *workspaces, float *const *grad_w, float *const *w_p,
                                          float *const *w_m, float *const *w_v, int ncs, const float *const *cs_partials,
                                          const int *cs_rows, const int *cs_cols, float *const *cs_outs, float *const *b_p,
                                          float *const *b_m, float *const *b_v, float lr, float beta1, float beta2, float eps,
                                          float *state, void *stream)
{
    if (count + ncs == 0 || !state) return GEOM_EINVAL;
    if ((count && (!w_p || !w_m || !w_v)) || (ncs && (!b_p || !b_m || !b_v))) return GEOM_EINVAL;
    ReduceJobs jobs;
    const int code = build_reduce_jobs(jobs, count, rows, cin, c, workspaces, grad_w, ncs, cs_partials, cs_rows, cs_cols, cs_outs);
    if (code) return code;
    ReduceAdam adam{};
    for (int l = 0; l < count; ++l) {
        adam.p[l] = w_p[l], adam.m[l] = w_m[l], adam.v[l] = w_v[l];
        if (w_p[l] && (!w_m[l] || !w_v[l])) return GEOM_EINVAL;
    }
    for (int i = 0; i < ncs; ++i) {
        adam.p[count + i] = b_p[i], adam.m[count + i] = b_m[i], adam.v[count + i] = b_v[i];
        if (b_p[i] && (!b_m[i] || !b_v[i])) return GEOM_EINVAL;
    }
    adam.lr = lr, adam.b1 = beta1, adam.b2 = beta2, adam.eps = eps, adam.state = state;
    uintptr_t bits = 0;
    for (int j = 0; j < jobs.n; ++j)
        if (adam.p[j]) bits |= (uintptr_t)adam.p[j] | (uintptr_t)adam.m[j] | (uintptr_t)adam.v[j] | (uintptr_t)jobs.job[j].out;
    adam.vec = (bits & 15) == 0;
    return launch_reduce(jobs, adam, stream);
}

extern "C" int geom_dense_reduce_f32(int count, const int *rows, const int *cin, const int *c, const float *const *workspaces,
                                     float *const *grad_w, float *const *grad_bias, void *stream)
{
    constexpr int MAX = GEOM_DENSE_MAX_REDUCE_JOBS / 2;
    if (count < 0 || count > MAX) return GEOM_ETOOBIG;
    if (count == 0) return 0;
    if (!rows || !cin || !c || !workspaces || !grad_w) return GEOM_EINVAL;
    const float *cs_partials[MAX];
    float *cs_outs[MAX];
    int cs_rows[MAX], cs_cols[MAX], ncs = 0;
    for (int l = 0; l < count; ++l) {
        if (bad_layer(workspaces[l], grad_w[l], rows[l], cin[l], c[l])) return GEOM_EINVAL;
        if (!grad_bias || !grad_bias[l]) continue;
        const SplitGeo g = split_geometry(cin[l], rows[l], num_cus());
        if (g.full_tiles == 0) return GEOM_EUNSUPPORTED;
        cs_partials[ncs] = workspaces[l] + g.colsum_offset(), cs_outs[ncs] = grad_bias[l];
        cs_rows[ncs] = g.s_full, cs_cols[ncs] = c[l], ++ncs;
    }
    ReduceJobs jobs;
    const int code = build_reduce_jobs(jobs, count, rows, cin, c, workspaces, grad_w, ncs, cs_partials, cs_rows, cs_cols, cs_outs);
    return code ? code : launch_reduce(jobs, ReduceAdam{}, stream);
}
```

geometrics_amd/csrc/zn_gcn.hip:

```cpp
#include <type_traits>

#include "buffer_access.h"

namespace {

using namespace geom;

constexpr int GCN_THREADS = 256;

struct GcnArgs {
    const int *rowptr, *col;
    const float *val;
    const float *x;
    const float *bias;
    const float *saved;
    float *y;
    int64_t rows;
    int nv, c, k;
};

template <int VEC>
struct PackVector;
template <>
struct PackVector<4> { using type = float4; };
template <>
struct PackVector<2> { using type = float2; };
template <>
struct PackVector<1> { using type = float; };

__device__ __forceinline__ float *elements(float4 &v) { return &v.x; }
__device__ __forceinline__ float *elements(float2 &v) { return &v.x; }
__device__ __forceinline__ float *elements(float &v) { return &v; }
__device__ __forceinline__ const float *elements(const float4 &v) { return &v.x; }
__device__ __forceinline__ const float *elements(const float2 &v) { return &v.x; }
__device__ __forceinline__ const float *elements(const float &v) { return &v; }

template <int VEC>
struct Pack {
    using Vector = typename PackVector<VEC>::type;
    Vector v;
    __device__ __forceinline__ void load(const float *p) { v = *reinterpret_cast<const Vector *>(p); }
    __device__ __forceinline__ void store(float *p) const { *reinterpret_cast<Vector *>(p) = v; }
    __device__ __forceinline__ float &at(int i) { return elements(v)[i]; }
    __device__ __forceinline__ float at(int i) const { return elements(v)[i]; }
    static __device__ __forceinline__ Pack zero()
    {
        Pack p;
#pragma unroll
        for (int i = 0; i < VEC; ++i) p.at(i) = 0.f;
        return p;
    }
    __device__ __forceinline__ void add(const Pack &o)
    {
#pragma unroll
        for (int i = 0; i < VEC; ++i) at(i) += o.at(i);
    }
    __device__ __forceinline__ void add_scaled(float w, const Pack &o)
    {
#pragma unroll
        for (int i = 0; i < VEC; ++i) at(i) += w * o.at(i);
    }
    template <int ACT>
    __device__ __forceinline__ void act_bwd_from(const Pack &out)
    {
#pragma unroll
        for (int i = 0; i < VEC; ++i) at(i) = act_bwd<ACT>(at(i), out.at(i));
    }
    __device__ __forceinline__ void keep_where(unsigned bits)
    {
#pragma unroll
        for (int i = 0; i < VEC; ++i) at(i) = (bits & (1u << i)) ? at(i) : 0.f;
    }
    template <int ACT, bool WIDE = false>
    __device__ __forceinline__ void bias_act(const float *bias, int col)
    {
        if (WIDE) {
            if (bias) {
                Pack b;
                b.load(bias + col);
                add(b);
            }
#pragma unroll
            for (int i = 0; i < VEC; ++i) at(i) = act_fwd<ACT>(at(i));
        } else {
#pragma unroll
            for (int i = 0; i < VEC; ++i) {
                float t = at(i);
                if (bias) t += bias[col + i];
                at(i) = act_fwd<ACT>(t);
            }
        }
    }
    __device__ __forceinline__ unsigned positive_bits() const
    {
        unsigned bits = 0u;
#pragma unroll
        for (int i = 0; i < VEC; ++i) bits |= at(i) > 0.f ? 1u << i : 0u;
        return bits;
    }
    __device__ __forceinline__ void take_from(const Pack &o, int first)
    {
#pragma unroll
        for (int i = 0; i < VEC; ++i)
            if (i >= first) at(i) = o.at(i);
    }
    __device__ __forceinline__ void store_below(float *row, int c0, int k) const
    {
        if (c0 + VEC <= k) {
            store(row + c0);
        } else {
#pragma unroll
            for (int i = 0; i < VEC; ++i)
                if (c0 + i < k) row[c0 + i] = at(i);
        }
    }
    __device__ __forceinline__ void store_from(float *row, int c0, int k) const
    {
        if (c0 >= k) {
            store(row + c0);
        } else {
#pragma unroll
            for (int i = 0; i < VEC; ++i)
                if (c0 + i >= k) row[c0 + i] = at(i);
        }
    }
    __device__ __forceinline__ void store_elements(float *p) const
    {
#pragma unroll
        for (int i = 0; i < VEC; ++i) p[i] = at(i);
    }
};

constexpr int GCN_NB = 8;
constexpr int GCN_BWD_ITERS = 2;

struct Source {
    const float *x;
    const float *saved;
    const unsigned short *mask;
    int kg, j;
    const float *head;
    float head_scale;
    int c;
};

template <int VEC_, int ACT_, bool BACKWARD_, bool MASK_ = false, bool HEAD_ = false>
struct TermKind {
    static_assert((!MASK_ && !HEAD_) || VEC_ == 4, "sign mask and head are the fast kernel's");
    static constexpr int VEC = VEC_, ACT = ACT_;
    static constexpr bool BACKWARD = BACKWARD_, MASK = MASK_, HEAD = HEAD_;
};

template <class KIND, int VEC>
__device__ __forceinline__ void term_load(Pack<VEC> &v, Pack<VEC> &out, unsigned &bits, const Source &s, int64_t row, int col)
{
    if (KIND::BACKWARD && KIND::HEAD) {
        v = Pack<VEC>::zero();
        if (col == 0) {
            const float *gp = s.head + row * 3;
#pragma unroll
            for (int i = 0; i < 3 && i < VEC; ++i) v.at(i) = s.head_scale * gp[i];
        }
    } else {
        v.load(s.x + row * s.c + col);
    }
    if (KIND::BACKWARD && KIND::MASK) bits = s.mask[row * s.kg + s.j];
    else if (KIND::BACKWARD && KIND::ACT != ACT_NONE) out.load(s.saved + row * s.c + col);
}

template <class KIND, int VEC>
__device__ __forceinline__ void term_finish(Pack<VEC> &v, const Pack<VEC> &out, unsigned bits)
{
    if (KIND::BACKWARD && KIND::MASK) v.keep_where(bits);
    else if (KIND::BACKWARD && KIND::ACT != ACT_NONE) v.template act_bwd_from<KIND::ACT>(out);
}

template <class KIND, int VEC>
__device__ __forceinline__ void term_add(Pack<VEC> &acc, float w, Pack<VEC> &v, const Pack<VEC> &out, unsigned bits)
{
    term_finish<KIND>(v, out, bits);
    acc.add_scaled(w, v);
}

template <class KIND, int VEC>
__device__ __forceinline__ void own_element(Pack<VEC> &own, const Source &s, int64_t row, int col)
{
    Pack<VEC> out;
    unsigned bits = 0u;
    term_load<KIND>(own, out, bits, s, row, col);
    term_finish<KIND>(own, out, bits);
}

template <class KIND, int VEC>
__device__ __forceinline__ void add_csr_run(Pack<VEC> &acc, const Source &s, const int *col, const float *val, int e, int e1,
                                            int64_t mesh_row0, int64_t row, int c0)
{
    for (; e < e1; e += GCN_NB) {
        int64_t nb[GCN_NB];
        float w[GCN_NB];
#pragma unroll
        for (int j = 0; j < GCN_NB; ++j) {
            const bool in = e + j < e1;
            nb[j] = in ? mesh_row0 + col[e + j] : row;
            w[j] = in ? val[e + j] : 0.f;
        }
        Pack<VEC> sv[GCN_NB], ov[GCN_NB];
        unsigned bits[GCN_NB] = {};
#pragma unroll
        for (int j = 0; j < GCN_NB; ++j) term_load<KIND>(sv[j], ov[j], bits[j], s, nb[j], c0);
#pragma unroll
        for (int j = 0; j < GCN_NB; ++j)
            if (e + j < e1) term_add<KIND>(acc, w[j], sv[j], ov[j], bits[j]);
    }
}

template <int W>
__device__ __forceinline__ void load_table_row(const int *col, const float *val, int r, int (&nb)[W], float (&w)[W])
{
#pragma unroll
    for (int n = 0; n < W; n += 4) {
        const int4 ci = *reinterpret_cast<const int4 *>(col + (size_t)r * W + n);
        const float4 wi = *reinterpret_cast<const float4 *>(val + (size_t)r * W + n);
        nb[n] = ci.x, nb[n + 1] = ci.y, nb[n + 2] = ci.z, nb[n + 3] = ci.w;
        w[n] = wi.x, w[n + 1] = wi.y, w[n + 2] = wi.z, w[n + 3] = wi.w;
    }
}

template <class KIND, int W, int VEC>
__device__ __forceinline__ void load_table_slots(Pack<VEC> (&sv)[W], Pack<VEC> (&ov)[W], unsigned (&bits)[W], const Source &s,
                                                 const int (&nb)[W], int64_t mesh_row0, int r, int c0)
{
#pragma unroll
    for (int n = 0; n < W; ++n) term_load<KIND>(sv[n], ov[n], bits[n], s, mesh_row0 + (nb[n] >= 0 ? nb[n] : r), c0);
}

template <class KIND, int W, int VEC>
__device__ __forceinline__ void add_table_slots(Pack<VEC> &acc, Pack<VEC> (&sv)[W], const Pack<VEC> (&ov)[W], const unsigned (&bits)[W],
                                                const int (&nb)[W], const float (&w)[W])
{
#pragma unroll
    for (int n = 0; n < W; ++n)
        if (nb[n] >= 0) term_add<KIND>(acc, w[n], sv[n], ov[n], bits[n]);
}

template <int VEC>
__device__ __forceinline__ void write_colsum_partial(float *lds, const Pack<VEC> &colsum, bool active, int rl, int rows_in_flight,
                                                     int c, int c0, float *partial_row)
{
    if (active) colsum.store_elements(lds + rl * c + c0);
    __syncthreads();
    if (active && rl == 0) {
#pragma unroll
        for (int i = 0; i < VEC; ++i) {
            float t = 0.f;
            for (int l = 0; l < rows_in_flight; ++l) t += lds[l * c + c0 + i];
            partial_row[c0 + i] = t;
        }
    }
}

template <int VEC, int ACT, bool BACKWARD>
__global__ __launch_bounds__(GCN_THREADS) void zn_aggregate_kernel(GcnArgs a, int groups, int rows_in_flight,
                                                                    int rows_per_block, float *colsum_partial)
{
    using KIND = TermKind<VEC, ACT, BACKWARD>;
    extern __shared__ float lds_colsum[];
    const int g = threadIdx.x % groups;
    const int rl = threadIdx.x / groups;
    const int c0 = g * VEC;
    const bool active = rl < rows_in_flight;
    const int r_begin = blockIdx.x * rows_per_block;
    const int r_end = min(r_begin + rows_per_block, a.nv);
    const int64_t mesh_row0 = (int64_t)blockIdx.y * a.nv;
    const Source src{.x = a.x, .saved = a.saved, .c = a.c};

    Pack<VEC> colsum = Pack<VEC>::zero();

    if (active) {
        for (int r = r_begin + rl; r < r_end; r += rows_in_flight) {
            const int64_t row = mesh_row0 + r;
            Pack<VEC> acc, own;
            const bool pass = c0 + VEC > a.k;
            if (BACKWARD || pass) own_element<KIND>(own, src, row, c0);
            if (c0 < a.k) {
                acc = Pack<VEC>::zero();
                add_csr_run<KIND>(acc, src, a.col, a.val, a.rowptr[r], a.rowptr[r + 1], mesh_row0, row, c0);
                if (pass) acc.take_from(own, a.k - c0);
            } else {
                acc = own;
            }
            if (BACKWARD) colsum.add(own);
            else acc.template bias_act<ACT>(a.bias, c0);
            acc.store(a.y + row * a.c + c0);
        }
    }

    if (BACKWARD && colsum_partial)
        write_colsum_partial(lds_colsum, colsum, active, rl, rows_in_flight, a.c, c0,
                             colsum_partial + ((size_t)blockIdx.y * gridDim.x + blockIdx.x) * a.c);
}

constexpr int CS_COLS = 16, CS_LANES = 64;
__device__ __forceinline__ void reduce_partials(float (&part)[CS_LANES][CS_COLS], int blocks, int c, const float *partial, float *out)
{
    const int cl = threadIdx.x % CS_COLS, lane = threadIdx.x / CS_COLS;
    const int col = blockIdx.x * CS_COLS + cl;
    float t = 0.f;
    if (col < c) {
#pragma unroll 8
        for (int b = lane; b < blocks; b += CS_LANES) t += partial[(size_t)b * c + col];
    }
    part[lane][cl] = t;
    __syncthreads();
    if (lane == 0 && col < c) {
        float acc = 0.f;
        for (int l = 0; l < CS_LANES; ++l) acc += part[l][cl];
        out[col] = acc;
    }
}

__global__ __launch_bounds__(CS_COLS *CS_LANES) void colsum_final_kernel(int blocks, int c, const float *partial,
                                                                         float *out)
{
    __shared__ float part[CS_LANES][CS_COLS];
    reduce_partials(part, blocks, c, partial, out);
}

struct ColsumJobs {
    const float *partial[GEOM_COLSUM_MAX_JOBS];
    float *out[GEOM_COLSUM_MAX_JOBS];
    int blocks[GEOM_COLSUM_MAX_JOBS], c[GEOM_COLSUM_MAX_JOBS];
};

__global__ __launch_bounds__(CS_COLS *CS_LANES) void colsum_batch_kernel(ColsumJobs jobs)
{
    __shared__ float part[CS_LANES][CS_COLS];
    const int job = blockIdx.y;
    if ((int)blockIdx.x * CS_COLS >= jobs.c[job]) return;
    reduce_partials(part, jobs.blocks[job], jobs.c[job], jobs.partial[job], jobs.out[job]);
}

struct GcnGeometry {
    int groups, rows_in_flight, rows_per_block;
    int chunks;
    int64_t blocks;
};

inline GcnGeometry gcn_geometry(int b, int nv, int c, int vec, bool backward)
{
    GcnGeometry g;
    g.groups = c / vec;
    g.rows_in_flight = g.groups >= GCN_THREADS ? 1 : GCN_THREADS / g.groups;
    g.rows_per_block = g.rows_in_flight * (backward ? GCN_BWD_ITERS : 1);
    g.chunks = (nv + g.rows_per_block - 1) / g.rows_per_block;
    g.blocks = (int64_t)g.chunks * b;
    return g;
}

inline bool gcn_vec4(int c, int ) { return c % 4 == 0; }

inline int check_sizes(int b, int nv, int c, int k) { return (b < 0 || nv < 0 || c < 0 || k < 0 || k > c) ? GEOM_EINVAL : 0; }

template <bool BACKWARD>
int check_gradient_operands(int act, bool has_saved, const float *grad_bias, const float *scratch)
{
    return ((BACKWARD && act != ACT_NONE && !has_saved) || (grad_bias && !scratch)) ? GEOM_EINVAL : 0;
}

inline int finish_launch(bool backward, int64_t blocks, int c, const float *partial, float *grad_bias, hipStream_t s)
{
    if (backward && partial && grad_bias)
        hipLaunchKernelGGL(colsum_final_kernel, dim3((c + CS_COLS - 1) / CS_COLS), dim3(CS_COLS * CS_LANES), 0, s, (int)blocks, c,
                           partial, grad_bias);
    return geom::launch_status();
}

template <int V>
using Const = std::integral_constant<int, V>;

template <class F>
bool with_act(int act, F &&f)
{
    switch (act) {
    case ACT_NONE: f(Const<ACT_NONE>{}); return true;
    case ACT_RELU: f(Const<ACT_RELU>{}); return true;
    case ACT_ELU: f(Const<ACT_ELU>{}); return true;
    default: return false;
    }
}

template <class F>
void with_width(int w, F &&f) { w == 8 ? f(Const<8>{}) : f(Const<16>{}); }

template <class F>
void with_vec(int vec, F &&f) { vec == 4 ? f(Const<4>{}) : vec == 2 ? f(Const<2>{}) : f(Const<1>{}); }

template <int VEC, bool BACKWARD>
int launch(const GcnArgs &a, int act, float *colsum_partial, float *grad_bias, void *stream)
{
    const int meshes = (int)(a.rows / a.nv);
    const GcnGeometry geo = gcn_geometry(meshes, a.nv, a.c, VEC, BACKWARD);
    if (geo.groups > GCN_THREADS) return GEOM_ETOOBIG;
    if (meshes > 65535 || geo.blocks > 0x7fffffffLL) return GEOM_ETOOBIG;
    dim3 grid((unsigned)geo.chunks, (unsigned)meshes), block(GCN_THREADS);
    const size_t lds = (BACKWARD && colsum_partial) ? (size_t)geo.rows_in_flight * a.c * sizeof(float) : 0;
    hipStream_t s = static_cast<hipStream_t>(stream);
    const bool known = with_act(act, [&](auto ACT) {
        hipLaunchKernelGGL((zn_aggregate_kernel<VEC, decltype(ACT)::value, BACKWARD>), grid, block, lds, s, a, geo.groups,
                           geo.rows_in_flight, geo.rows_per_block, colsum_partial);
    });
    return known ? finish_launch(BACKWARD, geo.blocks, a.c, colsum_partial, grad_bias, s) : GEOM_EINVAL;
}

struct EllArgs {
    const int *col;
    const float *val;
    const float *x, *bias, *saved;
    float *y;
    int nv, c, k;
    unsigned short *mask;
    const int *over_ptr, *over_col;
    const float *over_val;
    int b, chunks;
    const float *head_in;
    float *head_out;
    float head_scale;
};

template <int ACT, bool BACKWARD, int W, int NC, bool MASK = false, bool HEAD = false>
__global__ __launch_bounds__(GCN_THREADS) void zn_aggregate_ell_kernel(EllArgs a, int rows_per_block, int iters,
                                                                        float *colsum_partial)
{
    static_assert(!MASK || (ACT == ACT_RELU && NC == 2), "the sign mask is the ReLU / split-3 fast path");
    extern __shared__ float lds_cs[];
    const int kg = a.k >> 2;
    const int j = threadIdx.x % kg;
    const int rl = threadIdx.x / kg;
    int mesh_i, chunk_i;
    if (!geom::xcd_assign(blockIdx.x, a.b, a.chunks, mesh_i, chunk_i)) return;
    const int64_t mesh_row0 = (int64_t)mesh_i * a.nv;
    const int c0 = 4 * j;
    using KIND = TermKind<4, ACT, BACKWARD, MASK, HEAD>;
    const Source src{.x = a.x, .saved = a.saved, .mask = a.mask, .kg = kg, .j = j, .head = a.head_in, .head_scale = a.head_scale, .c = a.c};
    float4 csum[NC + 1];
#pragma unroll
    for (int i = 0; i <= NC; ++i) csum[i] = make_float4(0.f, 0.f, 0.f, 0.f);

    for (int it = 0; it < iters; ++it) {
    const int r = (chunk_i * iters + it) * rows_per_block + rl;
    const bool active = rl < rows_per_block && r < a.nv;
    float4 own[NC + 1];
#pragma unroll
    for (int i = 0; i <= NC; ++i) own[i] = make_float4(0.f, 0.f, 0.f, 0.f);

    if (active) {
        const int64_t row = mesh_row0 + r;
        const float *xrow = a.x + row * a.c;
        int nb[W];
        float w[W];
        load_table_row<W>(a.col, a.val, r, nb, w);
        constexpr int TAIL = (ACT == ACT_NONE && NC == 2) ? 16 : 8;
        int e0 = 0, e1 = 0;
        if (a.over_ptr) e0 = a.over_ptr[r], e1 = a.over_ptr[r + 1];
        unsigned own_bits = 0u;
        if (BACKWARD && MASK) own_bits = a.mask[row * kg + j];
#pragma unroll
        for (int i = BACKWARD ? 0 : 1; i <= NC; ++i) {
            if (BACKWARD && HEAD) {
                if (i == 0 && j == 0) {
                    const float *gp = a.head_in + row * 3;
                    own[0] = make_float4(a.head_scale * gp[0], a.head_scale * gp[1], a.head_scale * gp[2], 0.f);
                }
            } else
            own[i] = *reinterpret_cast<const float4 *>(xrow + c0 + a.k * i);
            if (BACKWARD && MASK) {
                const unsigned m = own_bits >> (4 * i);
                own[i].x = (m & 1u) ? own[i].x : 0.f;
                own[i].y = (m & 2u) ? own[i].y : 0.f;
                own[i].z = (m & 4u) ? own[i].z : 0.f;
                own[i].w = (m & 8u) ? own[i].w : 0.f;
            } else if (BACKWARD && ACT != ACT_NONE) {
                const float4 o = *reinterpret_cast<const float4 *>(a.saved + row * a.c + c0 + a.k * i);
                own[i].x = act_bwd<ACT>(own[i].x, o.x);
                own[i].y = act_bwd<ACT>(own[i].y, o.y);
                own[i].z = act_bwd<ACT>(own[i].z, o.z);
                own[i].w = act_bwd<ACT>(own[i].w, o.w);
            }
        }
        Pack<4> sv[W], ov[W];
        unsigned nbits[W] = {};
        load_table_slots<KIND>(sv, ov, nbits, src, nb, mesh_row0, r, c0);
        int tcol[TAIL];
        float tval[TAIL];
        if (e0 < e1) {
#pragma unroll
            for (int t = 0; t < TAIL; ++t) {
                const int ee = e0 + t < e1 ? e0 + t : e1 - 1;
                tcol[t] = a.over_col[ee];
                tval[t] = a.over_val[ee];
            }
        }
        Pack<4> acc = Pack<4>::zero();
        add_table_slots<KIND>(acc, sv, ov, nbits, nb, w);
        for (int e = e0; e < e1; e += TAIL) {
            int64_t nrow[TAIL];
            float wv[TAIL];
            Pack<4> tv[TAIL], to[TAIL];
            unsigned tb[TAIL] = {};
#pragma unroll
            for (int t = 0; t < TAIL; ++t) {
                nrow[t] = mesh_row0 + tcol[t];
                wv[t] = tval[t];
                term_load<KIND>(tv[t], to[t], tb[t], src, nrow[t], c0);
            }
            if (e + TAIL < e1) {
#pragma unroll
                for (int t = 0; t < TAIL; ++t) {
                    const int ee = e + TAIL + t < e1 ? e + TAIL + t : e1 - 1;
                    tcol[t] = a.over_col[ee];
                    tval[t] = a.over_val[ee];
                }
            }
#pragma unroll
            for (int t = 0; t < TAIL; ++t)
                if (e + t < e1) term_add<KIND>(acc, wv[t], tv[t], to[t], tb[t]);
        }
        float *yrow = a.y + row * a.c;
        unsigned sign_bits = 0u;
#pragma unroll
        for (int i = 0; i <= NC; ++i) {
            Pack<4> v;
            v.v = i == 0 ? acc.v : own[i];
            if (!BACKWARD) {
                v.template bias_act<ACT, true>(a.bias, c0 + a.k * i);
                if (MASK) sign_bits |= v.positive_bits() << (4 * i);
            }
            v.store(yrow + c0 + a.k * i);
            if (!BACKWARD && HEAD && i == 0 && j == 0) {
                const float *bp = a.head_in + row * 3;
                float *pp = a.head_out + row * 3;
#pragma unroll
                for (int e = 0; e < 3; ++e) pp[e] = bp[e] + a.head_scale * v.at(e);
            }
        }
        if (!BACKWARD && MASK) a.mask[row * kg + j] = (unsigned short)sign_bits;
    }
    if (BACKWARD) {
#pragma unroll
        for (int i = 0; i <= NC; ++i)
            csum[i].x += own[i].x, csum[i].y += own[i].y, csum[i].z += own[i].z, csum[i].w += own[i].w;
    }
    }

    if (BACKWARD && colsum_partial) {
        if (rl < rows_per_block) {
#pragma unroll
            for (int i = 0; i <= NC; ++i)
                *reinterpret_cast<float4 *>(lds_cs + rl * a.c + c0 + a.k * i) = csum[i];
        }
        __syncthreads();
        for (int c = threadIdx.x; c < a.c; c += GCN_THREADS) {
            float t = 0.f;
            for (int l = 0; l < rows_per_block; ++l) t += lds_cs[l * a.c + c];
            colsum_partial[((size_t)mesh_i * a.chunks + chunk_i) * a.c + c] = t;
        }
    }
}

enum EllRoute { ELL_NONE, ELL_FAST3, ELL_FAST10, ELL_ANY };

inline int ell_any_vec(int c) { return c % 4 == 0 ? 4 : c % 2 == 0 ? 2 : 1; }
inline int ell_nc(int c, int k) { return (k > 0 && k % 4 == 0 && c % k == 0) ? c / k - 1 : -1; }

inline EllRoute ell_route(int c, int k, int w)
{
    if (w != 8 && w != 16) return ELL_NONE;
    const int nc = ell_nc(c, k);
    if ((nc == 2 || nc == 9) && (k >> 2) <= GCN_THREADS) return nc == 2 ? ELL_FAST3 : ELL_FAST10;
    return (c > 0 && c / ell_any_vec(c) <= GCN_THREADS) ? ELL_ANY : ELL_NONE;
}

struct EllGeometry { int rows_per_block, iters, chunks; int64_t blocks; };

inline EllGeometry ell_geometry(int b, int nv, int k, bool backward)
{
    EllGeometry g;
    g.rows_per_block = GCN_THREADS / (k >> 2);
    g.iters = backward ? 2 : 1;
    g.chunks = (nv + g.rows_per_block * g.iters - 1) / (g.rows_per_block * g.iters);
    g.blocks = (int64_t)g.chunks * b;
    return g;
}

template <int VEC, int ACT, bool BACKWARD, int W>
__global__ __launch_bounds__(GCN_THREADS) void zn_aggregate_ell_any_kernel(EllArgs a, int groups, int rows_in_flight, int rows_per_block,
                                                                            float *colsum_partial)
{
    using KIND = TermKind<VEC, ACT, BACKWARD>;
    extern __shared__ float lds_colsum[];
    const int r_begin = blockIdx.x * rows_per_block;
    const int r_end = min(r_begin + rows_per_block, a.nv);
    const int64_t mesh_row0 = (int64_t)blockIdx.y * a.nv;
    const Source src{.x = a.x, .saved = a.saved, .c = a.c};

    const int kgs = (a.k + VEC - 1) / VEC;
    for (int item = threadIdx.x; item < (r_end - r_begin) * kgs; item += GCN_THREADS) {
        const int r = r_begin + item / kgs, c0 = (item % kgs) * VEC;
        const int64_t row = mesh_row0 + r;
        int nb[W];
        float w[W];
        load_table_row<W>(a.col, a.val, r, nb, w);
        int e0 = 0, e1 = 0;
        if (a.over_ptr) e0 = a.over_ptr[r], e1 = a.over_ptr[r + 1];
        Pack<VEC> sv[W], ov[W];
        unsigned nbits[W] = {};
        load_table_slots<KIND>(sv, ov, nbits, src, nb, mesh_row0, r, c0);
        Pack<VEC> acc = Pack<VEC>::zero();
        add_table_slots<KIND>(acc, sv, ov, nbits, nb, w);
        add_csr_run<KIND>(acc, src, a.over_col, a.over_val, e0, e1, mesh_row0, row, c0);
        if (!BACKWARD) acc.template bias_act<ACT>(a.bias, c0);
        acc.store_below(a.y + row * a.c, c0, a.k);
    }

    const int g = threadIdx.x % groups;
    const int rl = threadIdx.x / groups;
    const int c0 = g * VEC;
    const bool active = rl < rows_in_flight;
    const bool pass = c0 + VEC > a.k;

    Pack<VEC> colsum = Pack<VEC>::zero();

    if (active && (BACKWARD || pass)) {
        for (int r = r_begin + rl; r < r_end; r += rows_in_flight) {
            const int64_t row = mesh_row0 + r;
            Pack<VEC> own;
            own_element<KIND>(own, src, row, c0);
            if (BACKWARD) colsum.add(own);
            else own.template bias_act<ACT>(a.bias, c0);
            own.store_from(a.y + row * a.c, c0, a.k);
        }
    }

    if (BACKWARD && colsum_partial)
        write_colsum_partial(lds_colsum, colsum, active, rl, rows_in_flight, a.c, c0,
                             colsum_partial + ((size_t)blockIdx.y * gridDim.x + blockIdx.x) * a.c);
}

inline GcnGeometry ell_any_geometry(int b, int nv, int c, bool backward)
{
    GcnGeometry g;
    g.groups = c / ell_any_vec(c);
    g.rows_in_flight = GCN_THREADS / g.groups;
    const int64_t tiles = ((int64_t)b * nv + g.rows_in_flight - 1) / g.rows_in_flight;
    int64_t iters = (tiles + 1023) / 1024;
    const int64_t lo = backward ? GCN_BWD_ITERS : 1, hi = 64;
    iters = iters < lo ? lo : iters > hi ? hi : iters;
    g.rows_per_block = g.rows_in_flight * (int)iters;
    g.chunks = (nv + g.rows_per_block - 1) / g.rows_per_block;
    g.blocks = (int64_t)g.chunks * b;
    return g;
}

template <bool BACKWARD>
int dispatch_ell(EllArgs a, int b, int w, int act, float *grad_bias, float *scratch, void *stream)
{
    if (const int code = check_sizes(b, a.nv, a.c, a.k)) return code;
    const EllRoute route = ell_route(a.c, a.k, w);
    const bool fast = route == ELL_FAST3 || route == ELL_FAST10;
    if (route == ELL_NONE || (!fast && (a.head_in || a.mask))) return GEOM_EUNSUPPORTED;
    if (b == 0 || a.nv == 0) return 0;
    if (!a.col || !a.val || !a.y || (!a.x && !(BACKWARD && a.head_in))) return GEOM_EINVAL;
    if (a.head_in && (route != ELL_FAST3 || !((act == ACT_RELU && a.mask) || act == ACT_NONE) || (!BACKWARD && !a.head_out)))
        return GEOM_EUNSUPPORTED;
    if (a.mask && !(act == ACT_RELU && route == ELL_FAST3)) return GEOM_EINVAL;
    if (const int code = check_gradient_operands<BACKWARD>(act, a.saved || a.mask, grad_bias, scratch)) return code;
    if (a.over_ptr && (!a.over_col || !a.over_val)) return GEOM_EINVAL;
    if ((((uintptr_t)a.col | (uintptr_t)a.val) % 16) != 0) return GEOM_EINVAL;
    if ((((uintptr_t)a.x | (uintptr_t)a.y | (uintptr_t)a.saved | (uintptr_t)(fast ? a.bias : nullptr)) % (fast ? 16 : 4 * ell_any_vec(a.c))) != 0)
        return GEOM_EINVAL;
    if (b > 65535) return GEOM_ETOOBIG;
    float *partial = scratch;
    hipStream_t s = static_cast<hipStream_t>(stream);
    if (!fast) {
        const GcnGeometry geo = ell_any_geometry(b, a.nv, a.c, BACKWARD);
        const size_t lds = (BACKWARD && partial) ? (size_t)geo.rows_in_flight * a.c * sizeof(float) : 0;
        const dim3 grid((unsigned)geo.chunks, (unsigned)b);
        const bool known = with_act(act, [&](auto ACT) { with_width(w, [&](auto W) { with_vec(ell_any_vec(a.c), [&](auto VEC) {
            hipLaunchKernelGGL((zn_aggregate_ell_any_kernel<decltype(VEC)::value, decltype(ACT)::value, BACKWARD, decltype(W)::value>),
                               grid, dim3(GCN_THREADS), lds, s, a, geo.groups, geo.rows_in_flight, geo.rows_per_block, partial);
        }); }); });
        return known ? finish_launch(BACKWARD, geo.blocks, a.c, partial, grad_bias, s) : GEOM_EINVAL;
    }
    const EllGeometry geo = ell_geometry(b, a.nv, a.k, BACKWARD);
    const size_t lds = (BACKWARD && partial) ? (size_t)geo.rows_per_block * a.c * sizeof(float) : 0;
    a.b = b, a.chunks = geo.chunks;
    const dim3 grid(geom::xcd_grid(b, geo.chunks));
    const bool known = with_act(act, [&](auto ACT) { with_width(w, [&](auto W) {
        constexpr int A = decltype(ACT)::value;
        auto go = [&](auto NC, auto MASK, auto HEAD) {
            hipLaunchKernelGGL((zn_aggregate_ell_kernel<A, BACKWARD, decltype(W)::value, decltype(NC)::value, decltype(MASK)::value, decltype(HEAD)::value>),
                               grid, dim3(GCN_THREADS), lds, s, a, geo.rows_per_block, geo.iters, partial);
        };
        if constexpr (A == ACT_RELU) {
            if (a.head_in) return go(Const<2>{}, std::true_type{}, std::true_type{});
            if (a.mask) return go(Const<2>{}, std::true_type{}, std::false_type{});
        } else if constexpr (A == ACT_NONE) {
            if (a.head_in) return go(Const<2>{}, std::false_type{}, std::true_type{});
        }
        if (route == ELL_FAST3) go(Const<2>{}, std::false_type{}, std::false_type{});
        else go(Const<9>{}, std::false_type{}, std::false_type{});
    }); });
    return known ? finish_launch(BACKWARD, geo.blocks, a.c, partial, grad_bias, s) : GEOM_EINVAL;
}

constexpr int NARROW_THREADS = 64;
constexpr int NARROW_PARTIAL_ROWS = 32;

struct NarrowHeadArgs {
    const int *col;
    const float *val;
    const int *over_ptr, *over_col;
    const float *over_val;
    const float *support, *bias;
    const float *base;
    float *pos;
    const float *grad_pos;
    unsigned short *sign;
    float *gs;
    float *partial;
    float scale;
    int nv, c, b, chunks;
};

template <int ACT, int W>
__global__ __launch_bounds__(NARROW_THREADS) void zn_narrow_head_fwd_kernel(NarrowHeadArgs a)
{
    int mesh_i, chunk_i;
    if (!geom::xcd_assign(blockIdx.x, a.b, a.chunks, mesh_i, chunk_i)) return;
    const int r = chunk_i * NARROW_THREADS + threadIdx.x;
    if (r >= a.nv) return;
    const int64_t mesh_row0 = (int64_t)mesh_i * a.nv, row = mesh_row0 + r;
    using KIND = TermKind<4, ACT, false>;
    const Source src{.x = a.support, .c = a.c};
    int nb[W];
    float w[W];
    load_table_row<W>(a.col, a.val, r, nb, w);
    int e0 = 0, e1 = 0;
    if (a.over_ptr) e0 = a.over_ptr[r], e1 = a.over_ptr[r + 1];
    Pack<4> sv[W], ov[W];
    unsigned nbits[W] = {};
    load_table_slots<KIND>(sv, ov, nbits, src, nb, mesh_row0, r, 0);
    Pack<4> acc = Pack<4>::zero();
    add_table_slots<KIND>(acc, sv, ov, nbits, nb, w);
    add_csr_run<KIND>(acc, src, a.over_col, a.over_val, e0, e1, mesh_row0, row, 0);
    acc.template bias_act<ACT, true>(a.bias, 0);
    if (ACT == ACT_RELU && a.sign) a.sign[row] = (unsigned short)acc.positive_bits();
    const float *bp = a.base + row * 3;
    float *pp = a.pos + row * 3;
#pragma unroll
    for (int e = 0; e < 3; ++e) pp[e] = bp[e] + a.scale * acc.at(e);
}

template <int ACT, int W>
__global__ __launch_bounds__(NARROW_THREADS) void zn_narrow_head_bwd_kernel(NarrowHeadArgs a)
{
    __shared__ float4 own_lds[NARROW_PARTIAL_ROWS];
    int mesh_i, chunk_i;
    if (!geom::xcd_assign(blockIdx.x, a.b, a.chunks, mesh_i, chunk_i)) return;
    const int rl = threadIdx.x;
    const int r = chunk_i * NARROW_PARTIAL_ROWS + rl;
    const int64_t mesh_row0 = (int64_t)mesh_i * a.nv, row = mesh_row0 + r;
    using KIND = TermKind<4, ACT, true, ACT == ACT_RELU, true>;
    const Source src{.mask = a.sign, .kg = 1, .j = 0, .head = a.grad_pos, .head_scale = a.scale, .c = a.c};
    if (rl < NARROW_PARTIAL_ROWS) {
        Pack<4> own = Pack<4>::zero();
        if (r < a.nv) {
            int nb[W];
            float w[W];
            load_table_row<W>(a.col, a.val, r, nb, w);
            int e0 = 0, e1 = 0;
            if (a.over_ptr) e0 = a.over_ptr[r], e1 = a.over_ptr[r + 1];
            own_element<KIND>(own, src, row, 0);
            Pack<4> sv[W], ov[W];
            unsigned nbits[W] = {};
            load_table_slots<KIND>(sv, ov, nbits, src, nb, mesh_row0, r, 0);
            Pack<4> acc = Pack<4>::zero();
            add_table_slots<KIND>(acc, sv, ov, nbits, nb, w);
            add_csr_run<KIND>(acc, src, a.over_col, a.over_val, e0, e1, mesh_row0, row, 0);
            acc.store(a.gs + row * 4);
        }
        own_lds[rl] = own.v;
    }
    if (!a.partial) return;
    __syncthreads();
    float *prow = a.partial + ((size_t)mesh_i * a.chunks + chunk_i) * a.c;
    for (int col = threadIdx.x; col < a.c; col += NARROW_THREADS) {
        float t = 0.f;
        if (col < 4) {
            constexpr int HALF = NARROW_PARTIAL_ROWS / 2;
            for (int l = 0; l < HALF; ++l) {
                float cs = 0.f;
                cs += elements(own_lds[l])[col];
                cs += elements(own_lds[l + HALF])[col];
                t += cs;
            }
        }
        prow[col] = t;
    }
}

template <bool BACKWARD>
int dispatch_narrow_head(NarrowHeadArgs a, int k, int w, int act, void *stream)
{
    if (const int code = check_sizes(a.b, a.nv, a.c, k)) return code;
    if (ell_route(a.c, k, w) != ELL_FAST3 || (act != ACT_RELU && act != ACT_NONE)) return GEOM_EUNSUPPORTED;
    const EllGeometry wide = ell_geometry(a.b > 0 ? a.b : 1, a.nv > 0 ? a.nv : 1, k, true);
    if (wide.rows_per_block * wide.iters != NARROW_PARTIAL_ROWS) return GEOM_EUNSUPPORTED;
    if (!BACKWARD && (!a.base || !a.pos)) return GEOM_EINVAL;
    if (BACKWARD && !a.grad_pos) return GEOM_EINVAL;
    if (a.b == 0 || a.nv == 0) return 0;
    if (!a.col || !a.val || (BACKWARD ? !a.gs : !a.support)) return GEOM_EINVAL;
    if (BACKWARD && act == ACT_RELU && !a.sign) return GEOM_EINVAL;
    if (act == ACT_NONE && a.sign) return GEOM_EINVAL;
    if (a.over_ptr && (!a.over_col || !a.over_val)) return GEOM_EINVAL;
    if ((((uintptr_t)a.col | (uintptr_t)a.val | (uintptr_t)a.support | (uintptr_t)a.bias | (uintptr_t)a.gs) % 16) != 0) return GEOM_EINVAL;
    if (a.b > 65535) return GEOM_ETOOBIG;
    a.chunks = BACKWARD ? wide.chunks : (a.nv + NARROW_THREADS - 1) / NARROW_THREADS;
    const dim3 grid(geom::xcd_grid(a.b, a.chunks));
    hipStream_t s = static_cast<hipStream_t>(stream);
    with_act(act, [&](auto ACT) { with_width(w, [&](auto W) {
        constexpr int A = decltype(ACT)::value == ACT_RELU ? ACT_RELU : ACT_NONE;
        if (BACKWARD) hipLaunchKernelGGL((zn_narrow_head_bwd_kernel<A, decltype(W)::value>), grid, dim3(NARROW_THREADS), 0, s, a);
        else hipLaunchKernelGGL((zn_narrow_head_fwd_kernel<A, decltype(W)::value>), grid, dim3(NARROW_THREADS), 0, s, a);
    }); });
    return geom::launch_status();
}

template <bool BACKWARD>
int dispatch(GcnArgs a, int b, int act, float *grad_bias, float *scratch, void *stream)
{
    if (const int code = check_sizes(b, a.nv, a.c, a.k)) return code;
    if (b == 0 || a.nv == 0 || a.c == 0) return 0;
    if (!a.rowptr || !a.x || !a.y || (a.k > 0 && (!a.col || !a.val))) return GEOM_EINVAL;
    if (const int code = check_gradient_operands<BACKWARD>(act, a.saved != nullptr, grad_bias, scratch)) return code;
    a.rows = (int64_t)b * a.nv;
    const bool vec4 = gcn_vec4(a.c, a.k);
    if (vec4 && (((uintptr_t)a.x | (uintptr_t)a.y | (uintptr_t)a.saved) % 16 != 0))
        return GEOM_EINVAL;
    if (!vec4 && a.c > GCN_THREADS) return GEOM_ETOOBIG;
    return vec4 ? launch<4, BACKWARD>(a, act, scratch, grad_bias, stream) : launch<1, BACKWARD>(a, act, scratch, grad_bias, stream);
}

}

extern "C" int geom_zn_gcn_aggregate_fwd_f32(int b, int nv, int c, int k, const int *rowptr, const int *col,
                                             const float *val, const float *support, const float *bias,
                                             int act, float *out, void *stream)
{
    GcnArgs a{rowptr, col, val, support, bias, nullptr, out, 0, nv, c, k};
    return dispatch<false>(a, b, act, nullptr, nullptr, stream);
}

extern "C" int64_t geom_zn_gcn_bwd_scratch_floats(int b, int nv, int c)
{
    if (b <= 0 || nv <= 0 || c <= 0) return 0;
    const int64_t b4 = (c % 4 == 0) ? gcn_geometry(b, nv, c, 4, true).blocks : 0;
    const int64_t b1 = gcn_geometry(b, nv, c, 1, true).blocks;
    return (b4 > b1 ? b4 : b1) * c;
}

extern "C" int64_t geom_zn_gcn_bwd_partial_rows(int b, int nv, int c, int k, int ell_w)
{
    if (b <= 0 || nv <= 0 || c <= 0 || k < 0 || k > c) return 0;
    if (!ell_w) return gcn_geometry(b, nv, c, gcn_vec4(c, k) ? 4 : 1, true).blocks;
    const EllRoute route = ell_route(c, k, ell_w);
    if (route == ELL_ANY) return ell_any_geometry(b, nv, c, true).blocks;
    return route == ELL_NONE ? 0 : ell_geometry(b, nv, k, true).blocks;
}

extern "C" int geom_colsum_batch_f32(int count, const float *const *partials, const int *rows, const int *cols,
                                     float *const *outs, void *stream)
{
    if (count < 0 || count > GEOM_COLSUM_MAX_JOBS) return GEOM_ETOOBIG;
    if (count == 0) return 0;
    if (!partials || !rows || !cols || !outs) return GEOM_EINVAL;
    ColsumJobs jobs;
    int widest = 0;
    for (int i = 0; i < count; ++i) {
        if (!partials[i] || !outs[i] || rows[i] < 0 || cols[i] <= 0) return GEOM_EINVAL;
        jobs.partial[i] = partials[i], jobs.out[i] = outs[i], jobs.blocks[i] = rows[i], jobs.c[i] = cols[i];
        widest = cols[i] > widest ? cols[i] : widest;
    }
    hipLaunchKernelGGL(colsum_batch_kernel, dim3((widest + CS_COLS - 1) / CS_COLS, count), dim3(CS_COLS * CS_LANES), 0,
                       static_cast<hipStream_t>(stream), jobs);
    return geom::launch_status();
}

extern "C" int geom_zn_gcn_aggregate_bwd_f32(int b, int nv, int c, int k, const int *rowptrT, const int *colT,
                                             const float *valT, const float *grad_out, const float *out,
                                             int act, float *grad_support, float *grad_bias, float *scratch,
                                             void *stream)
{
    GcnArgs a{rowptrT, colT, valT, grad_out, nullptr, out, grad_support, 0, nv, c, k};
    return dispatch<true>(a, b, act, grad_bias, scratch, stream);
}

extern "C" int geom_zn_gcn_aggregate_ell_fwd_f32(int b, int nv, int c, int k, int w, const int *ell_col,
                                                 const float *ell_val, const int *over_ptr, const int *over_col,
                                                 const float *over_val, const float *support, const float *bias,
                                                 int act, float *out, uint16_t *relu_mask, void *stream)
{
    EllArgs a{.col = ell_col, .val = ell_val, .x = support, .bias = bias, .y = out, .nv = nv, .c = c, .k = k, .mask = relu_mask,
              .over_ptr = over_ptr, .over_col = over_col, .over_val = over_val};
    return dispatch_ell<false>(a, b, w, act, nullptr, nullptr, stream);
}

extern "C" int geom_zn_gcn_aggregate_ell_head_fwd_f32(int b, int nv, int c, int k, int w, const int *ell_col,
                                                      const float *ell_val, const int *over_ptr, const int *over_col,
                                                      const float *over_val, const float *support, const float *bias,
                                                      int act, float *out, uint16_t *relu_mask, const float *base,
                                                      float scale, float *pos, void *stream)
{
    if (!base || !pos) return GEOM_EINVAL;
    EllArgs a{.col = ell_col, .val = ell_val, .x = support, .bias = bias, .y = out, .nv = nv, .c = c, .k = k, .mask = relu_mask,
              .over_ptr = over_ptr, .over_col = over_col, .over_val = over_val, .head_in = base, .head_out = pos, .head_scale = scale};
    return dispatch_ell<false>(a, b, w, act, nullptr, nullptr, stream);
}

extern "C" int64_t geom_zn_gcn_relu_mask_words(int b, int nv, int c, int k)
{
    if (b <= 0 || nv <= 0 || ell_nc(c, k) != 2) return 0;
    return (int64_t)b * nv * (k >> 2);
}

extern "C" int geom_zn_gcn_aggregate_ell_bwd_f32(int b, int nv, int c, int k, int w, const int *ell_colT,
                                                 const float *ell_valT, const int *over_ptrT, const int *over_colT,
                                                 const float *over_valT, const float *grad_out, const float *out,
                                                 const uint16_t *relu_mask, int act, float *grad_support,
                                                 float *grad_bias, float *scratch, void *stream)
{
    EllArgs a{.col = ell_colT, .val = ell_valT, .x = grad_out, .saved = out, .y = grad_support, .nv = nv, .c = c, .k = k,
              .mask = const_cast<uint16_t *>(relu_mask), .over_ptr = over_ptrT, .over_col = over_colT, .over_val = over_valT};
    return dispatch_ell<true>(a, b, w, act, grad_bias, scratch, stream);
}

extern "C" int geom_zn_gcn_aggregate_ell_head_bwd_f32(int b, int nv, int c, int k, int w, const int *ell_colT,
                                                      const float *ell_valT, const int *over_ptrT, const int *over_colT,
                                                      const float *over_valT, const float *grad_pos, float scale,
                                                      const uint16_t *relu_mask, int act, float *grad_support,
                                                      float *grad_bias, float *scratch, void *stream)
{
    if (!grad_pos) return GEOM_EINVAL;
    EllArgs a{.col = ell_colT, .val = ell_valT, .y = grad_support, .nv = nv, .c = c, .k = k, .mask = const_cast<uint16_t *>(relu_mask),
              .over_ptr = over_ptrT, .over_col = over_colT, .over_val = over_valT, .head_in = grad_pos, .head_scale = scale};
    return dispatch_ell<true>(a, b, w, act, grad_bias, scratch, stream);
}

extern "C" int geom_zn_gcn_narrow_head_fwd_f32(int b, int nv, int c, int k, int w, const int *ell_col, const float *ell_val,
                                               const int *over_ptr, const int *over_col, const float *over_val,
                                               const float *support, const float *bias, int act, const float *base,
                                               float scale, float *pos, uint16_t *sign_words, void *stream)
{
    NarrowHeadArgs a{.col = ell_col, .val = ell_val, .over_ptr = over_ptr, .over_col = over_col, .over_val = over_val,
                     .support = support, .bias = bias, .base = base, .pos = pos, .sign = sign_words, .scale = scale,
                     .nv = nv, .c = c, .b = b};
    return dispatch_narrow_head<false>(a, k, w, act, stream);
}

extern "C" int geom_zn_gcn_narrow_head_bwd_f32(int b, int nv, int c, int k, int w, const int *ell_colT, const float *ell_valT,
                                               const int *over_ptrT, const int *over_colT, const float *over_valT,
                                               const float *grad_pos, float scale, const uint16_t *sign_words, int act,
                                               float *grad_support4, float *partials, void *stream)
{
    NarrowHeadArgs a{.col = ell_colT, .val = ell_valT, .over_ptr = over_ptrT, .over_col = over_colT, .over_val = over_valT,
                     .grad_pos = grad_pos, .sign = const_cast<uint16_t *>(sign_words), .gs = grad_support4, .partial = partials,
                     .scale = scale, .nv = nv, .c = c, .b = b};
    return dispatch_narrow_head<true>(a, k, w, act, stream);
}
```

geometrics_amd/dense.py:

```python
import ctypes
import os

import torch

from . import _lib


def supported(cin, c, rows=1):
    return 0 < c <= 192 and c % 16 == 0 and cin > 0 and rows * max(cin, c) < 2 ** 30


def plan(rows, cin, c):
    ok = supported(cin, c, rows)
    pair = ok and cin <= 192 and cin % 4 == 0 and rows >= 512
    ok = ok and c % 48 == 0
    pair = pair and ok
    return {"fwd": "lib", "dx": "mfma" if pair else "lib", "dw": "mfma" if ok and rows >= 512 else "lib", "pair": pair}


WIDE_DX_MIN_ROWS = 16384


def wide_dx_plan(rows, cin, c):
    return c == 192 and cin > 192 and rows >= WIDE_DX_MIN_ROWS


wide_dx = None


def wide_dx_takes(g, w, out=None):
    mode = wide_dx if wide_dx is not None else (os.environ.get("GEOM_WIDE_DX") or None)
    if mode not in (None, "lib", "split"):
        raise ValueError("GEOM_WIDE_DX / dense.wide_dx must be 'lib' or 'split' (got %r)" % (mode,))
    if mode == "lib" or w.dim() != 2 or g.dim() < 2:
        return False
    cin, c = w.shape
    rows = g.numel() // max(c, 1)
    if not (c == 192 and g.shape[-1] == c and cin > 192 and rows >= 1 and rows * max(cin, c) < 2 ** 29):
        return False
    for t in (g, w) + (() if out is None else (out,)):
        if not (t.is_cuda and t.dtype == torch.float32 and t.is_contiguous() and t.device == g.device):
            return False
    if g.data_ptr() % 16 or w.data_ptr() % 16 or (out is not None and tuple(out.shape) != (rows, cin)):
        return False
    return mode == "split" or wide_dx_plan(rows, cin, c)


def wide_dx_planes(w):
    if not (w.is_cuda and w.dtype == torch.float32 and w.dim() == 2 and w.is_contiguous()):
        raise ValueError("wide_dx_planes: a contiguous 2-D float32 tensor on a HIP device")
    cin, c = w.shape
    planes = torch.empty(3 * int(_lib.lib().geom_dense_dx_split_cinpad(cin)) * c, dtype=torch.int16, device=w.device)
    with torch.cuda.device(w.device):
        _lib.call("geom_dense_dx_split_planes_f32", cin, c, w.data_ptr(), planes.data_ptr())
    return planes


def wide_dx_planes_matrix(planes):
    nt = int(_lib.lib().geom_dense_dx_split_cinpad(1)) // 16
    return planes.view(-1, 6, nt, 3, 4, 16, 8).permute(3, 0, 2, 5, 1, 4, 6).reshape(3, -1, 192)


def backward_input_split(g, w, out=None):
    rows, c = g.shape
    cin = w.shape[0]
    if not (g.is_cuda and g.dtype == torch.float32 and g.dim() == 2 and g.is_contiguous()):
        raise ValueError("backward_input_split: g must be a contiguous float32 tensor on a HIP device")
    planes = wide_dx_planes(w)
    out = torch.empty(rows, cin, dtype=torch.float32, device=g.device) if out is None else out
    if not (_row_major(out) and out.dtype == torch.float32 and out.device == g.device and tuple(out.shape) == (rows, cin)):
        raise ValueError("backward_input_split: out must be a float32 [%d, %d] tensor with contiguous rows on g's device" % (rows, cin))
    with torch.cuda.device(g.device):
        _lib.call("geom_dense_dx_split_f32", rows, cin, c, g.data_ptr(), planes.data_ptr(), out.data_ptr(), out.stride(0) if rows > 1 else cin)
    return out


def forward(x, w, out=None):
    rows, cin = x.shape
    c = w.shape[1]
    out = torch.empty(rows, c, dtype=torch.float32, device=x.device) if out is None else out
    with torch.cuda.device(x.device):
        _lib.call("geom_dense_fwd_f32", rows, cin, c, x.data_ptr(), w.data_ptr(), 0, None, out.data_ptr(), None, None)
    return out


def forward_split(x, w, bias, ksplit, out, sup, mask):
    rows, cin = x.shape
    c = w.shape[1]
    with torch.cuda.device(x.device):
        _lib.call("geom_dense_fwd_f32", rows, cin, c, x.data_ptr(), w.data_ptr(), ksplit, _lib.ptr(bias), out.data_ptr(),
                  sup.data_ptr(), _lib.ptr(mask))


def backward_input(g, w, out=None):
    rows, c = g.shape
    cin = w.shape[0]
    out = torch.empty(rows, cin, dtype=torch.float32, device=g.device) if out is None else out
    with torch.cuda.device(g.device):
        _lib.call("geom_dense_bwd_input_f32", rows, cin, c, g.data_ptr(), w.data_ptr(), out.data_ptr())
    return out


def weight_workspace(rows, cin, c, device):
    n = int(_lib.lib().geom_dense_bwd_weight_workspace_floats(rows, cin, c))
    return torch.empty(n, dtype=torch.float32, device=device)


launch_probe = None


def backward_weight_partials(x, g, workspace, want_colsum=False):
    rows, cin = x.shape
    c = g.shape[1]
    probe = launch_probe
    with torch.cuda.device(x.device):
        if probe is not None:
            start, end = torch.cuda.Event(enable_timing=True), torch.cuda.Event(enable_timing=True)
            start.record()
        _lib.call("geom_dense_bwd_weight_f32", rows, cin, c, x.data_ptr(), g.data_ptr(), workspace.data_ptr(),
                  1 if want_colsum else 0)
        if probe is not None:
            end.record()
            probe.append((rows, cin, c, start, end))


def backward_pair(x, g, w, grad_x, workspace, want_colsum=False):
    rows, cin = x.shape
    c = g.shape[1]
    with torch.cuda.device(x.device):
        _lib.call("geom_dense_bwd_f32", rows, cin, c, x.data_ptr(), g.data_ptr(), w.data_ptr(), grad_x.data_ptr(),
                  workspace.data_ptr(), 1 if want_colsum else 0)


def backward_narrow(x, g4, w, grad_x, workspace):
    rows, cin = x.shape
    with torch.cuda.device(x.device):
        _lib.call("geom_dense_bwd_narrow_f32", rows, cin, w.shape[1], x.data_ptr(), g4.data_ptr(), w.data_ptr(), _lib.ptr(grad_x),
                  workspace.data_ptr())


def reduce(jobs, stream=None):
    n = len(jobs)
    if n == 0:
        return
    if n > _lib.DENSE_MAX_LAYERS:
        for i in range(0, n, _lib.DENSE_MAX_LAYERS):
            reduce(jobs[i:i + _lib.DENSE_MAX_LAYERS], stream)
        return
    ints = lambda k: (ctypes.c_int * n)(*[j[k] for j in jobs])
    ptrs = lambda k: (ctypes.c_void_p * n)(*[None if j[k] is None else j[k].data_ptr() for j in jobs])
    dev = jobs[0][3].device
    with torch.cuda.device(dev):
        _lib.check(_lib.status("geom_dense_reduce_f32", n, ints(0), ints(1), ints(2), ptrs(3), ptrs(4), ptrs(5), stream=stream),
                   "geom_dense_reduce_f32")


def backward_weight(x, g, want_bias=False):
    rows, cin = x.shape
    c = g.shape[1]
    ws = weight_workspace(rows, cin, c, x.device)
    backward_weight_partials(x, g, ws, want_bias)
    gw = torch.empty(cin, c, dtype=torch.float32, device=x.device)
    gb = torch.empty(c, dtype=torch.float32, device=x.device) if want_bias else None
    reduce([(rows, cin, c, ws, gw, gb)])
    return gw, gb


def any_supported(rows, cin, c):
    return rows >= 256 and cin > 0 and c > 0 and rows * max(cin, c) * 4 < 2 ** 31 - 1


def _row_major(t):
    return t.dim() == 2 and t.stride(1) == 1 and t.stride(0) >= t.shape[1]


def gemm(a, b, trans_a=False, trans_b=False, out=None, workspace=None):
    if not (_row_major(a) and _row_major(b)):
        raise ValueError("gemm operands must be 2-D with contiguous rows")
    for name, t in (("a", a), ("b", b), ("out", out), ("workspace", workspace)):
        if t is None:
            continue
        if not t.is_cuda or t.dtype != torch.float32:
            raise ValueError("gemm: %s must be a float32 tensor on a HIP device (got %s on %s)" % (name, t.dtype, t.device))
        if t.device != a.device:
            raise ValueError("gemm: %s is on %s, a on %s" % (name, t.device, a.device))
    k, m = (a.shape if trans_a else a.shape[::-1])
    n, kb = (b.shape if trans_b else b.shape[::-1])
    if k != kb:
        raise ValueError("gemm: summed extents differ (%d vs %d)" % (k, kb))
    if out is None:
        out = torch.empty(m, n, dtype=torch.float32, device=a.device)
    elif not _row_major(out) or tuple(out.shape) != (m, n):
        raise ValueError("gemm: out must be [%d, %d] with contiguous rows" % (m, n))
    need = int(_lib.lib().geom_gemm_workspace_floats(m, n, k))
    if need and (workspace is None or workspace.numel() < need):
        workspace = torch.empty(need, dtype=torch.float32, device=a.device)
    with torch.cuda.device(a.device):
        _lib.call("geom_gemm_f32", m, n, k, a.data_ptr(), a.stride(0), 1 if trans_a else 0, b.data_ptr(), b.stride(0),
                  0 if trans_b else 1, out.data_ptr(), out.stride(0), _lib.ptr(workspace) if need else None, need)
    return out


def split_bf16_planes(w):
    if not (w.is_cuda and w.dtype == torch.float32 and w.dim() == 2 and w.is_contiguous()):
        raise ValueError("split_bf16_planes: a contiguous 2-D float32 tensor on a HIP device")
    k, n = w.shape
    kpad = int(_lib.lib().geom_split_bf16_kpad(k))
    planes = torch.empty(3, n, kpad, dtype=torch.int16, device=w.device)
    with torch.cuda.device(w.device):
        _lib.call("geom_split_bf16_planes_f32", k, n, w.data_ptr(), planes.data_ptr())
    return planes


def gemm_split_bf16(a, planes, terms=6, out=None):
    if not (a.is_cuda and a.dtype == torch.float32 and a.dim() == 2 and a.is_contiguous()):
        raise ValueError("gemm_split_bf16: a contiguous 2-D float32 tensor on a HIP device")
    m, k = a.shape
    n = planes.shape[1]
    if planes.shape[2] != int(_lib.lib().geom_split_bf16_kpad(k)):
        raise ValueError("gemm_split_bf16: the planes belong to another k")
    out = torch.empty(m, n, dtype=torch.float32, device=a.device) if out is None else out
    with torch.cuda.device(a.device):
        _lib.call("geom_gemm_split_bf16_f32", m, k, n, a.data_ptr(), planes.data_ptr(), out.data_ptr(), int(terms))
    return out
```

geometrics_amd/layers.py:

```python
import math
import os
import weakref

import torch
import torch.nn.functional as F
from torch import nn
from torch.nn import Module
from torch.nn.parameter import Parameter

from . import _lib
from . import aggregation as _agg
from . import backward_pass as _pass
from . import fused as _fused
from . import products as _products
from .backward_pass import (_alias, _gradient_buffer, bind_gradient_targets, deferred_parameter_gradients,
                            late_input_gradients)
from .products import _dense, _new_like, current_slabs, weight_gradient_batching
from .aggregation import ACT_ELU as _ACT_ELU, ACT_NONE as _ACT_NONE, ACT_RELU as _ACT_RELU
from .aggregation import activation_code as _activation_code, backward as aggregate_backward, forward as aggregate_forward


class _Csr:
    __slots__ = ("rowptr", "col", "val", "rowptr_t", "col_t", "val_t", "nv", "nnz",
                 "ell_w", "ell_col", "ell_val", "ell_col_t", "ell_val_t", "inv_deg", "over", "over_t",
                 "symmetric_structure",
                 "_deform_tail")


_csr_cache = {}


def _to_csr(dense):
    nz = dense.nonzero()
    rows, cols = nz[:, 0], nz[:, 1]
    counts = torch.bincount(rows, minlength=dense.shape[0])
    rowptr = torch.zeros(dense.shape[0] + 1, dtype=torch.int64, device=dense.device)
    rowptr[1:] = torch.cumsum(counts, 0)
    return rowptr.to(torch.int32), cols.to(torch.int32).contiguous(), dense[rows, cols].to(torch.float32).contiguous()


def _to_ell(rowptr, col, val, width):
    nv = rowptr.numel() - 1
    lens = (rowptr[1:] - rowptr[:-1]).long()
    rows = torch.repeat_interleave(torch.arange(nv, device=col.device), lens)
    slot = torch.arange(col.numel(), device=col.device) - rowptr[:-1].long()[rows]
    ell_col = torch.full((nv, width), -1, dtype=torch.int32, device=col.device)
    ell_val = torch.zeros((nv, width), dtype=torch.float32, device=col.device)
    head = slot < width
    ell_col[rows[head], slot[head]] = col[head]
    ell_val[rows[head], slot[head]] = val[head]
    over = None
    if not bool(head.all()):
        over_ptr = torch.zeros(nv + 1, dtype=torch.int64, device=col.device)
        over_ptr[1:] = torch.cumsum((lens - width).clamp_min(0), 0)
        over = (over_ptr.to(torch.int32).contiguous(), col[~head].contiguous(), val[~head].contiguous())
    return ell_col.contiguous(), ell_val.contiguous(), over


def _ell_width(lens_a, lens_b):
    n = max(int(lens_a.numel()), 1)
    for w in (8, 16):
        if max(int((lens_a > w).sum()), int((lens_b > w).sum())) <= 0.05 * n:
            return w
    return 0


def _finish_csr(c):
    c.nv = int(c.rowptr.numel()) - 1
    c.nnz = int(c.col.numel())
    c.inv_deg = (1.0 / ((c.rowptr[1:] - c.rowptr[:-1]).float() - 1.0)).contiguous()
    c.ell_w = _ell_width(c.rowptr[1:] - c.rowptr[:-1], c.rowptr_t[1:] - c.rowptr_t[:-1]) if c.nv else 0
    c.symmetric_structure = bool(torch.equal(c.rowptr, c.rowptr_t) and torch.equal(c.col, c.col_t))
    c.ell_col = c.ell_val = c.ell_col_t = c.ell_val_t = c.over = c.over_t = None
    if c.ell_w:
        c.ell_col, c.ell_val, c.over = _to_ell(c.rowptr, c.col, c.val, c.ell_w)
        c.ell_col_t, c.ell_val_t, c.over_t = _to_ell(c.rowptr_t, c.col_t, c.val_t, c.ell_w)
    return c


def csr_from_parts(rowptr, col, val, rowptr_t, col_t, val_t):
    c = _Csr()
    c.rowptr, c.col, c.val, c.rowptr_t, c.col_t, c.val_t = rowptr, col, val, rowptr_t, col_t, val_t
    with torch.no_grad():
        return _finish_csr(c)


def adjacency_csr(adj):
    if isinstance(adj, _Csr):
        return adj
    if hasattr(adj, "csr") and isinstance(adj.csr, _Csr):
        return adj.csr
    if adj.dim() != 2 or adj.shape[0] != adj.shape[1]:
        raise RuntimeError("adjacency must be a square [V,V] tensor, got %s" % (tuple(adj.shape),))
    key = id(adj)
    hit = _csr_cache.get(key)
    if hit is not None and hit[0]() is adj and hit[1] == adj._version:
        return hit[2]
    if not adj.is_cuda:
        raise RuntimeError("adjacency must live on a HIP device; geometrics_amd has no CPU path")
    with torch.no_grad():
        c = _Csr()
        dense = adj.detach()
        c.rowptr, c.col, c.val = _to_csr(dense)
        c.rowptr_t, c.col_t, c.val_t = _to_csr(dense.t())
        _finish_csr(c)
    _csr_cache[key] = (weakref.ref(adj, lambda _ref, k=key: _csr_cache.pop(k, None)), adj._version, c)
    return c


def _route(activation, t, adj, any_input=False):
    act = _ACT_NONE if activation is None else _activation_code(activation)
    per_mesh = torch.is_tensor(adj) and adj.dim() == 3
    batched = torch.is_tensor(t) and t.dim() == 3 and t.is_cuda and t.dtype == torch.float32 and not per_mesh
    csr = adjacency_csr(adj) if batched or (any_input and not per_mesh) else None
    return act, activation is not None and act == _ACT_NONE, batched, csr


def _split_k(support, layer):
    return support.shape[-1] // layer.split


def _bias_for(ctx):
    wanted = ctx.needs_input_grad[1] and ctx.bias_ref is not None
    return wanted, (ctx.bias_ref() if wanted else None)


class _ZeroNAggregate(torch.autograd.Function):

    @staticmethod
    def forward(ctx, support, bias, csr, k, act):
        s = _lib.require(support, "support", torch.float32, 3)
        if s.shape[1] != csr.nv:
            raise RuntimeError("support has %d vertices but the adjacency has %d" % (s.shape[1], csr.nv))
        bias_c = None if bias is None else _lib.require(bias, "bias", torch.float32, 1)
        ctx.arena = current_slabs()
        out = _new_like(s, "aggregated", ctx.arena)
        mask = _agg.forward(s, bias_c, csr, k, act, out, want_mask=support.requires_grad)
        ctx.csr, ctx.k, ctx.act = csr, k, act
        ctx.bias_ref = _pass.parameter_ref(bias, ctx, ctx.needs_input_grad[1])
        ctx.masked = mask is not None
        if mask is not None:
            ctx.save_for_backward(mask)
        elif act != _ACT_NONE:
            ctx.save_for_backward(out)
        return out

    @staticmethod
    def backward(ctx, grad_out):
        mask = ctx.saved_tensors[0] if ctx.masked else None
        out = ctx.saved_tensors[0] if (ctx.act != _ACT_NONE and not ctx.masked) else None
        grad_support, grad_bias = _agg.backward(grad_out.contiguous(), ctx.csr, ctx.k, ctx.act, out, mask, *_bias_for(ctx),
                                                arena=ctx.arena)
        return (grad_support if ctx.needs_input_grad[0] else None), grad_bias, None, None, None


class _ZeroNAggregateHead(torch.autograd.Function):

    @staticmethod
    def forward(ctx, support, bias, base, csr, k, act, scale, down=None):
        s = _lib.require(support, "support", torch.float32, 3)
        base_c = _lib.require(base, "base", torch.float32, 3, 3)
        ctx.down = down
        bias_c = None if bias is None else _lib.require(bias, "bias", torch.float32, 1)
        pos = torch.empty_like(base_c)
        mask = _agg.forward(s, bias_c, csr, k, act, torch.empty_like(s), want_mask=True, head=(base_c, scale, pos))
        ctx.csr, ctx.k, ctx.act, ctx.scale, ctx.shape = csr, k, act, float(scale), tuple(s.shape)
        ctx.bias_ref = _pass.parameter_ref(bias, ctx, ctx.needs_input_grad[1])
        if mask is not None:
            ctx.save_for_backward(mask)
        return pos

    @staticmethod
    def backward(ctx, grad_pos):
        gp = grad_pos.contiguous()
        b, nv, c = ctx.shape
        mask = ctx.saved_tensors[0] if ctx.saved_tensors else None
        below = ctx.down if _agg.takes_product_below(ctx.down, ctx.csr, c, ctx.k, b * nv, ctx.needs_input_grad[0]) else None
        grad_support, grad_bias = _agg.backward(None, ctx.csr, ctx.k, ctx.act, None, mask, *_bias_for(ctx),
                                                head=(gp, ctx.scale, ctx.shape), below=below)
        return (grad_support if ctx.needs_input_grad[0] else None), grad_bias, \
            (gp if ctx.needs_input_grad[2] else None), None, None, None, None, None


def zero_n_aggregate_head(support, adj, bias, k, activation, base, scale, down=None):
    act, foreign, batched, csr = _route(activation, support, adj)
    if batched and not foreign and act != _ACT_ELU and csr.ell_w and k > 0 and k % 4 == 0 and support.shape[-1] == 3 * k:
        return _ZeroNAggregateHead.apply(support, bias, base, csr, k, act, scale, down)
    from .ops import VertexHead
    return VertexHead.apply(base, zero_n_aggregate(support, adj, bias, k, activation), scale)


def zero_n_aggregate(support, adj, bias, k, activation=None):
    act, foreign, _, csr = _route(activation, support, adj, any_input=True)
    if csr is None:
        out = torch.cat((torch.matmul(adj, support[..., :k]), support[..., k:]), dim=-1)
        if bias is not None:
            out = out + bias
        return out if activation is None else activation(out)
    s3 = support.unsqueeze(0) if support.dim() == 2 else support
    out = _ZeroNAggregate.apply(s3, bias, csr, k, act)
    if support.dim() == 2:
        out = out.squeeze(0)
    return activation(out) if foreign else out


class _StackLink:
    __slots__ = ("wt", "dx", "g_ref", "g_version", "wanted")

    def __init__(self):
        self.wt = self.dx = self.g_ref = None
        self.g_version = -1
        self.wanted = False

    def stamp(self, g):
        self.g_ref, self.g_version = g, g._version

    def claim_dx(self, g):
        dx, ref, ver = self.dx, self.g_ref, self.g_version
        self.dx = self.g_ref = None
        if dx is None or ref is None:
            return None
        same = (g.data_ptr() == ref.data_ptr() and g.shape.numel() == ref.shape.numel() and g._version == ver
                and ref._version == ver)
        return dx if same else None

    def take_dx(self, b, nv):
        self.dx = torch.empty(b, nv, self.wt.shape[1], dtype=torch.float32, device=self.wt.device)
        return self.dx


class _FusedBoundary(torch.autograd.Function):

    @staticmethod
    def forward(ctx, support, bias, w_next, csr, k, act, up, down):
        s = _lib.require(support, "support", torch.float32, 3)
        c = s.shape[-1]
        bias_c = None if bias is None else _lib.require(bias, "bias", torch.float32, 1)
        w2 = w_next.reshape(w_next.shape[-2:])
        need = any(ctx.needs_input_grad[:3])
        mask = _agg.relu_mask(s, k) if need and act == _ACT_RELU else None
        if need:
            up.wt = torch.empty(w2.shape[1], c, dtype=torch.float32, device=s.device)
            up.wanted = bool(ctx.needs_input_grad[0] or ctx.needs_input_grad[1])
        x, s_next = _fused.layer_forward(s, bias_c, csr, k, act, w2, mask=mask, wt_out=up.wt)
        ctx.csr, ctx.k, ctx.act, ctx.up, ctx.down = csr, k, act, up, down
        ctx.bias_ref = _pass.parameter_ref(bias, ctx, ctx.needs_input_grad[1])
        ctx.w_ref = _pass.parameter_ref(w_next, ctx, ctx.needs_input_grad[2])
        ctx.masked = mask is not None
        ctx.save_for_backward(x, w_next, *([mask] if mask is not None else []))
        return s_next

    @staticmethod
    def backward(ctx, grad_next):
        x, w = ctx.saved_tensors[:2]
        mask = ctx.saved_tensors[2] if ctx.masked else None
        b, nv, c = x.shape
        rows = b * nv
        w2 = w.reshape(w.shape[-2:])
        n_out = w2.shape[1]
        g2 = grad_next.reshape(rows, n_out).contiguous()
        need_s, _, need_w = ctx.needs_input_grad[:3]
        need_b, bias = _bias_for(ctx)
        route = _products.route(rows, c, n_out, need_w, w2.is_contiguous(), True, False, _products._own_products_preferred(),
                                _products.use_any_shape_products)
        if route.dx == "any":
            route = route._replace(dx="lib")
        dx, grad_w = _products.product_gradients(x, g2, w, ctx.w_ref, route, need_s or need_b, need_w, dx=ctx.up.claim_dx(g2))
        if not (need_s or need_b):
            return None, None, grad_w, None, None, None, None, None
        below = ctx.down if _agg.takes_product_below(ctx.down, ctx.csr, c, ctx.k, rows, need_s) else None
        out = x if (ctx.act != _ACT_NONE and mask is None) else None
        grad_support, grad_bias = _agg.backward(dx, ctx.csr, ctx.k, ctx.act, out, mask, need_b, bias, below=below)
        return (grad_support if need_s else None), grad_bias, grad_w, None, None, None, None, None


NARROW_HEAD_MIN_ROWS = 4096

narrow_head = None


def _narrow_head_mode():
    mode = narrow_head if narrow_head is not None else (os.environ.get("GEOM_NARROW_HEAD") or None)
    if mode not in (None, "on", "off"):
        raise ValueError("GEOM_NARROW_HEAD / layers.narrow_head must be 'on' or 'off' (got %r)" % (mode,))
    return mode


def _narrow_head_takes(h, layer, adj, activation, base):
    mode = _narrow_head_mode()
    if mode == "off" or current_slabs() is not None:
        return False
    w, bias = layer._weight(), layer.bias
    if not (torch.is_tensor(h) and h.dim() == 3 and layer.split == 3 and w.dim() in (2, 3) and tuple(w.shape[-2:]) == (192, 192)
            and (w.dim() == 2 or w.shape[0] == 1) and h.shape[-1] == 192):
        return False
    for t in (h, w, base) + (() if bias is None else (bias,)):
        if not (torch.is_tensor(t) and t.is_cuda and t.dtype == torch.float32 and t.is_contiguous() and t.device == h.device):
            return False
    if not w.requires_grad or base.shape != h.shape[:-1] + (3,) or (bias is not None and bias.shape != (192,)):
        return False
    act, foreign, batched, csr = _route(activation, h, adj)
    if not batched or foreign or act == _ACT_ELU or not csr.ell_w or csr.nv != h.shape[1]:
        return False
    rows = h.shape[0] * h.shape[1]
    r = _products.route(rows, 192, 192, True, True, True, False, _products._own_products_preferred(), _products.use_any_shape_products)
    return r.dx == "pair" and r.dw == "split" and (mode == "on" or rows >= NARROW_HEAD_MIN_ROWS)


class _NarrowHead(torch.autograd.Function):

    @staticmethod
    def forward(ctx, x, w, bias, base, csr, act, scale, forward_kind):
        w2 = w.reshape(w.shape[-2:])
        x, s = _products._forward(forward_kind, x, w2)
        if s.shape[1] != csr.nv:
            raise RuntimeError("support has %d vertices but the adjacency has %d" % (s.shape[1], csr.nv))
        pos = torch.empty_like(base)
        k = s.shape[-1] // 3
        sign = _agg.narrow_head_forward(s, bias, csr, k, act, base, scale, pos, want_sign=any(ctx.needs_input_grad[:3]))
        ctx.csr, ctx.k, ctx.act, ctx.scale = csr, k, act, float(scale)
        ctx.w_ref = _pass.parameter_ref(w, ctx, ctx.needs_input_grad[1])
        ctx.bias_ref = _pass.parameter_ref(bias, ctx, ctx.needs_input_grad[2])
        ctx.save_for_backward(x, w, *([sign] if sign is not None else []))
        return pos

    @staticmethod
    def backward(ctx, grad_pos):
        gp = grad_pos.contiguous()
        x, w = ctx.saved_tensors[:2]
        sign = ctx.saved_tensors[2] if len(ctx.saved_tensors) > 2 else None
        need_x, need_w, need_b, need_base = ctx.needs_input_grad[:4]
        b, nv, cin = x.shape
        rows, c = b * nv, w.shape[-1]
        dx = grad_w = grad_bias = None
        if need_x or need_w or need_b:
            need_b = need_b and ctx.bias_ref is not None
            gs4, grad_bias = _agg.narrow_head_backward(gp, ctx.scale, sign, ctx.csr, ctx.k, ctx.act, (b, nv, c), need_b,
                                                       ctx.bias_ref() if need_b else None)
        if need_x or need_w:
            ws = _products._dense_kernels.weight_workspace(rows, cin, c, x.device)
            dx = torch.empty_like(x) if need_x else None
            _products._dense_kernels.backward_narrow(x.view(rows, cin), gs4, w.reshape(w.shape[-2:]), None if dx is None else dx.view(rows, cin), ws)
            if need_w:
                grad_w = _pass.weight_gradient(ctx.w_ref, w, rows, cin, c, ws)
        return dx, grad_w, grad_bias, (gp if need_base else None), None, None, None, None


def _narrow_head_positions(h, layer, adj, activation, base, scale):
    act, _, _, csr = _route(activation, h, adj)
    w = layer._weight()
    rows = h.shape[0] * h.shape[1]
    r = _products.route(rows, 192, 192, True, True, True, False, _products._own_products_preferred(), _products.use_any_shape_products)
    return _NarrowHead.apply(h, w, layer.bias, base, csr, act, scale, r.forward)


def _boundary_fuses(rows, csr, prev, layer):
    if not (current_slabs() is None and isinstance(csr, _Csr)):
        return False
    w = layer._weight()
    c = prev._weight().shape[-1]
    if w.dtype != torch.float32 or w.shape[-2] != c or not w.is_contiguous() or prev.split != 3 or c % 3:
        return False
    return _fused.supported(csr, c, c // 3, w.shape[-1]) and _fused.plan(rows)["fwd"]


def _stack_walk(x, adj, stack, activation, base=None):
    act, foreign, _, csr = _route(activation, x, adj)
    if foreign:
        csr = None
    if len(stack) == 1 and base is not None and _narrow_head_takes(x, stack[0], adj, activation, base):
        return x, None, True
    s = _dense(x, stack[0]._weight())
    link = None
    for prev, layer in zip(stack[:-1], stack[1:]):
        if _boundary_fuses(x.numel() // x.shape[-1], csr, prev, layer):
            up = _StackLink()
            s = _FusedBoundary.apply(s, prev.bias, layer._weight(), csr, _split_k(s, prev), act, up, link)
            link = up
        else:
            h = zero_n_aggregate(s, adj, prev.bias, _split_k(s, prev), activation)
            if layer is stack[-1] and base is not None and _narrow_head_takes(h, layer, adj, activation, base):
                return h, None, True
            s = _dense(h, layer._weight())
            link = None
    return s, link, False


def _stack_supports(x, adj, stack, activation):
    return _stack_walk(x, adj, stack, activation)[:2]


def zero_n_stack(x, adj, stack, activation):
    s, _ = _stack_supports(x, adj, stack, activation)
    return zero_n_aggregate(s, adj, stack[-1].bias, _split_k(s, stack[-1]), activation)


def zero_n_stack_positions(x, adj, stack, activation, base, scale):
    s, link, narrow = _stack_walk(x, adj, stack, activation, base)
    if narrow:
        return _narrow_head_positions(s, stack[-1], adj, activation, base, scale)
    return zero_n_aggregate_head(s, adj, stack[-1].bias, _split_k(s, stack[-1]), activation, base, scale, down=link)


def _uniform(t, bound):
    t.data.uniform_(-bound, bound)


class _ZeroNBase(Module):
    split = 10

    def _weight(self):
        raise NotImplementedError

    def forward(self, input, adj, activation):
        support = _dense(input, self._weight())
        return zero_n_aggregate(support, adj, self.bias, _split_k(support, self), activation)

    def forward_positions(self, input, adj, activation, base, scale):
        if _narrow_head_takes(input, self, adj, activation, base):
            return _narrow_head_positions(input, self, adj, activation, base, scale)
        support = _dense(input, self._weight())
        return zero_n_aggregate_head(support, adj, self.bias, _split_k(support, self), activation, base, scale)


class ZERON_GCN(_ZeroNBase):

    def __init__(self, in_features, out_features, bias=True):
        super().__init__()
        self.in_features, self.out_features = in_features, out_features
        self.weight = Parameter(torch.empty(in_features, out_features))
        if bias:
            self.bias = Parameter(torch.empty(out_features))
        else:
            self.register_parameter("bias", None)
        self.reset_parameters()

    def reset_parameters(self):
        _uniform(self.weight, 6.0 / math.sqrt(self.weight.size(0) + self.weight.size(1)))
        if self.bias is not None:
            self.bias.data.zero_()

    def _weight(self):
        return self.weight


class BatchZERON_GCN(ZERON_GCN):
    """Batched [B,V,Cin] input, same parameters and split (reference layers.py:121-152)."""


class Batch_Image_ZERON_GCNGCN(_ZeroNBase):
    split = 3

    def __init__(self, in_features, out_features, bias=True):
        super().__init__()
        self.in_features, self.out_features = in_features, out_features
        self.weight1 = Parameter(torch.empty(1, in_features, out_features))
        if bias:
            self.bias = Parameter(torch.empty(out_features))
        else:
            self.register_parameter("bias", None)
        self.reset_parameters()

    def reset_parameters(self):
        _uniform(self.weight1, 0.3 * 6.0 / math.sqrt(self.weight1.size(1) + self.weight1.size(0)))
        if self.bias is not None:
            _uniform(self.bias, 0.1)

    def _weight(self):
        return self.weight1


class _MaxPoolBase(Module):
    split = 10

    def __init__(self, in_features, print_length):
        super().__init__()
        self.in_features, self.print_length = in_features, print_length
        self.weight_Ws = nn.ParameterList([Parameter(torch.empty(in_features, print_length))])
        self.weight_Bs = nn.ParameterList([Parameter(torch.empty(print_length))])
        self.reset_parameters()

    def reset_parameters(self):
        _uniform(self.weight_Bs[0], 6.0 / math.sqrt(self.weight_Bs[0].size(0)))
        _uniform(self.weight_Ws[0], 6.0 / math.sqrt(self.weight_Ws[0].size(0) + self.weight_Ws[0].size(1)))

    def _pre_activation(self, r_s, adj):
        support = _dense(r_s, self.weight_Ws[0])
        return zero_n_aggregate(support, adj, self.weight_Bs[0], _split_k(support, self))


class GCNMax(_MaxPoolBase):

    def forward(self, r_s, adj, activation):
        support = _dense(r_s, self.weight_Ws[0])
        acted = zero_n_aggregate(support, adj, self.weight_Bs[0], _split_k(support, self), activation)
        if hasattr(adj, "offsets"):
            from .ops import SegmentMax
            return SegmentMax.apply(acted, adj.offsets, adj.max_len)
        return torch.max(acted, dim=0)[0]


class BatchGCNMax(_MaxPoolBase):

    def forward(self, r_s, adj, activation):
        return torch.max(self._pre_activation(r_s, adj), dim=1)[0]
```

include/geom_hip.h:

```cpp
#ifndef GEOM_HIP_H
#define GEOM_HIP_H

#include <stddef.h>
#include <stdint.h>

#ifdef __cplusplus
extern "C" {
#endif

#define GEOM_ABI_VERSION 16

#define GEOM_EINVAL   (-1)
#define GEOM_ETOOBIG  (-2)
#define GEOM_EUNSUPPORTED (-3)

#define GEOM_FLAG_REF_TAIL_TRUNC 1u
#define GEOM_FLAG_FIX_REGION6    2u
#define GEOM_FLAG_TRI_BRUTE_FORCE 4u
#define GEOM_FLAG_NN_FMA 8u

#define GEOM_FLAG_TRI_WS_READY 16u

int geom_abi_version(void);
const char *geom_strerror(int code);

int geom_chamfer_nn_f32(int b, int n, const float *xyz, int m, const float *xyz2,
                        float *result, int *result_i, float *result2, int *result2_i,
                        unsigned flags, void *stream);

int64_t geom_chamfer_nn_culled_workspace_floats(int b, int n, int m);
int geom_chamfer_nn_culled_f32(int b, int n, const float *xyz, int m, const float *xyz2, const int *order1, const int *order2,
                               float *result, int *result_i, float *result2, int *result2_i, unsigned flags, float *workspace,
                               void *stream);

int geom_tri_distance_f32(int b, int n, const float *xyz, int m,
                          const float *tri1, const float *tri2, const float *tri3,
                          float *dist, int *point, int *index, unsigned flags, void *stream);

int geom_tri_distance_indexed_f32(int b, int n, const float *xyz, int nv, const float *verts,
                                  int nf, const int64_t *faces,
                                  float *dist, int *point, int *index, unsigned flags, void *stream);

size_t geom_tri_distance_workspace_bytes(int b, int n, int m);
int geom_tri_distance_ws_f32(int b, int n, const float *xyz, int m,
                             const float *tri1, const float *tri2, const float *tri3, const int *order,
                             float *dist, int *point, int *index, unsigned flags,
                             void *workspace, size_t workspace_bytes, void *stream);
int geom_tri_distance_indexed_ws_f32(int b, int n, const float *xyz, int nv, const float *verts,
                                     int nf, const int64_t *faces, const int *order,
                                     float *dist, int *point, int *index, unsigned flags,
                                     void *workspace, size_t workspace_bytes, void *stream);

int geom_tri_surface_fwd_f32(int b, int n, const float *xyz, int nv, const float *verts, int nf,
                             const int64_t *faces, const int *order, float *dist, int *point, int *index,
                             float *sqdist, float *closest, float *weights, unsigned flags, void *workspace,
                             size_t workspace_bytes, void *stream);

int geom_face_areas_f32(int b, int nv, const float *verts, int nf, const int64_t *faces,
                        float *areas, void *stream);
int geom_draw_samples_f32(int b, int nv, const float *verts, int nf, const int64_t *faces, int num,
                          const float *uniforms, int64_t *choices, float *u, float *v, void *stream);
int geom_draw_samples_rng_f32(int b, int nv, const float *verts, int nf, const int64_t *faces, int num,
                              uint64_t *rng_state, int64_t *choices, float *u, float *v, float *points,
                              void *stream);
int geom_sample_faces_fwd_f32(int b, int nv, const float *verts, int nf, const int64_t *faces,
                              int num, const int64_t *choices, const float *u, const float *v,
                              float *points, void *stream);
int geom_sample_faces_bwd_f32(int b, int nv, int nf, const int64_t *faces,
                              int num, const int64_t *choices, const float *u, const float *v,
                              const float *grad_points, float *grad_verts, void *stream);

int geom_chamfer_grad_f32(int b, int n, const float *src, int m, const float *dst,
                          const int *idx, const float *coef_dev, float coef_host,
                          float *grad_src, int accumulate, float *grad_dst, void *stream);

int geom_p2tri_loss_fwd_f32(int b, int n, const float *xyz, int nv, const float *verts,
                            int nf, const int64_t *faces, const int *option, const int *index,
                            float *sqdist, float *closest, float *weights, void *stream);
int geom_p2tri_loss_bwd_f32(int b, int n, const float *xyz, int nv, int nf, const int64_t *faces,
                            const int *index, const float *closest, const float *weights,
                            const float *coef_dev, float coef_host, float *grad_verts, void *stream);

int geom_sum_f32(int64_t n, const float *x, float scale, float *out, void *stream);

int geom_sample_chamfer_bwd_f32(int b, int nv, int nf, const int64_t *faces, int num,
                                const int64_t *choices, const float *u, const float *v,
                                const float *points, int n_other, const float *other,
                                const int *idx, int via_nn, const float *coef_dev, float coef_host,
                                float *grad_verts, void *stream);
int geom_surface_loss_bwd_f32(int b, int nv, int nf, const int64_t *faces, int num, const int64_t *choices,
                              const float *u, const float *v, const float *points, int n_gt, const float *gt,
                              const int *idx_g, const int *index, const float *closest, const float *weights,
                              const float *coef_dev, float coef_sample, float coef_tri, float *grad_verts,
                              void *stream);

int geom_zn_gcn_aggregate_fwd_f32(int b, int nv, int c, int k, const int *rowptr, const int *col,
                                  const float *val, const float *support, const float *bias,
                                  int act, float *out, void *stream);
int64_t geom_zn_gcn_bwd_scratch_floats(int b, int nv, int c);
int64_t geom_zn_gcn_bwd_partial_rows(int b, int nv, int c, int k, int ell_w);
#define GEOM_COLSUM_MAX_JOBS 32
int geom_colsum_batch_f32(int count, const float *const *partials, const int *rows, const int *cols,
                          float *const *outs, void *stream);
int geom_zn_gcn_aggregate_bwd_f32(int b, int nv, int c, int k, const int *rowptrT, const int *colT,
                                  const float *valT, const float *grad_out, const float *out,
                                  int act, float *grad_support, float *grad_bias, float *scratch,
                                  void *stream);

int64_t geom_zn_gcn_relu_mask_words(int b, int nv, int c, int k);
int geom_zn_gcn_aggregate_ell_fwd_f32(int b, int nv, int c, int k, int w, const int *ell_col,
                                      const float *ell_val, const int *over_ptr, const int *over_col,
                                      const float *over_val, const float *support, const float *bias,
                                      int act, float *out, uint16_t *relu_mask, void *stream);
int geom_zn_gcn_aggregate_ell_bwd_f32(int b, int nv, int c, int k, int w, const int *ell_colT,
                                      const float *ell_valT, const int *over_ptrT, const int *over_colT,
                                      const float *over_valT, const float *grad_out, const float *out,
                                      const uint16_t *relu_mask, int act, float *grad_support,
                                      float *grad_bias, float *scratch, void *stream);

#define GEOM_DENSE_MAX_LAYERS 8
#define GEOM_DENSE_MAX_REDUCE_JOBS 32
int geom_dense_fwd_f32(int rows, int cin, int c, const float *x, const float *w, int ksplit, const float *bias,
                       float *out, float *sup, uint16_t *mask, void *stream);
int geom_dense_bwd_input_f32(int rows, int cin, int c, const float *g, const float *w, float *grad_x, void *stream);
int64_t geom_dense_bwd_weight_workspace_floats(int rows, int cin, int c);
int geom_dense_bwd_weight_f32(int rows, int cin, int c, const float *x, const float *g, float *workspace,
                              int want_colsum, void *stream);
int geom_dense_bwd_f32(int rows, int cin, int c, const float *x, const float *g, const float *w, float *grad_x,
                       float *workspace, int want_colsum, void *stream);
int geom_dense_bwd_narrow_f32(int rows, int cin, int c, const float *x, const float *g4, const float *w, float *grad_x,
                              float *workspace, void *stream);
int geom_dense_reduce2_f32(int count, const int *rows, const int *cin, const int *c, const float *const *workspaces,
                           float *const *grad_w, float *const *grad_bias, int ncs, const float *const *cs_partials,
                           const int *cs_rows, const int *cs_cols, float *const *cs_outs, void *stream);
int geom_dense_reduce_adam_f32(int count, const int *rows, const int *cin, const int *c, const float *const *workspaces,
                               float *const *grad_w, float *const *w_p, float *const *w_m, float *const *w_v, int ncs,
                               const float *const *cs_partials, const int *cs_rows, const int *cs_cols, float *const *cs_outs,
                               float *const *b_p, float *const *b_m, float *const *b_v, float lr, float beta1, float beta2,
                               float eps, float *state, void *stream);
int geom_dense_reduce_f32(int count, const int *rows, const int *cin, const int *c, const float *const *workspaces,
                          float *const *grad_w, float *const *grad_bias, void *stream);

int geom_zn_gcn_aggregate_ell_head_fwd_f32(int b, int nv, int c, int k, int w, const int *ell_col,
                                           const float *ell_val, const int *over_ptr, const int *over_col,
                                           const float *over_val, const float *support, const float *bias,
                                           int act, float *out, uint16_t *relu_mask, const float *base,
                                           float scale, float *pos, void *stream);
int geom_zn_gcn_aggregate_ell_head_bwd_f32(int b, int nv, int c, int k, int w, const int *ell_colT,
                                           const float *ell_valT, const int *over_ptrT, const int *over_colT,
                                           const float *over_valT, const float *grad_pos, float scale,
                                           const uint16_t *relu_mask, int act, float *grad_support,
                                           float *grad_bias, float *scratch, void *stream);

int geom_zn_gcn_narrow_head_fwd_f32(int b, int nv, int c, int k, int w, const int *ell_col, const float *ell_val,
                                    const int *over_ptr, const int *over_col, const float *over_val,
                                    const float *support, const float *bias, int act, const float *base,
                                    float scale, float *pos, uint16_t *sign_words, void *stream);
int geom_zn_gcn_narrow_head_bwd_f32(int b, int nv, int c, int k, int w, const int *ell_colT, const float *ell_valT,
                                    const int *over_ptrT, const int *over_colT, const float *over_valT,
                                    const float *grad_pos, float scale, const uint16_t *sign_words, int act,
                                    float *grad_support4, float *partials, void *stream);

int64_t geom_zn_layer_partial_rows(int b, int nv);
int geom_zn_layer_fwd_f32(int b, int nv, int c, int k, int ell_w, const int *ell_col, const float *ell_val,
                          const float *s_prev, const float *bias_prev, int act, const float *w, int n_out,
                          float *x_out, uint16_t *relu_mask, float *s_out, float *wt_out, void *stream);
int geom_zn_layer_bwd_f32(int b, int nv, int c, int k, int ell_w, const int *ell_col_t, const float *ell_val_t,
                          const float *grad_out, const float *out, const uint16_t *relu_mask, int act,
                          const float *grad_pos, float head_scale, const float *wt, int n_in, float *g_out,
                          float *grad_in, float *colsum_partial, void *stream);

typedef struct geom_deform_fwd {
    int b, nv, c, k, ell_w;
    const float *s_in, *bias;
    const int *ell_col; const float *ell_val;
    const int *tail_col; const float *tail_val;
    const float *bn_w, *bn_b;
    float *run_mean, *run_var;
    int training; float momentum, eps;
    int relu;
    const float *res; int res_ld; float scale;
    float *z_out, *x_out, *save_mean, *save_invstd;
    const float *w_next; float *s_out;
    const float *w_head; float *s_head;
    int vpx;
} geom_deform_fwd;
typedef struct geom_deform_bwd {
    int b, nv, c, k, ell_w;
    const float *dz_up;
    const int *ell_col_t; const float *ell_val_t;
    const int *tail_col_t; const float *tail_val_t;
    float *ds_up; const float *wt_up;
    const float *g, *g2;
    int g_ld, g2_ld;
    const float *z, *bn_w, *bn_b, *save_mean, *save_invstd;
    int relu, has_res; float scale;
    float *grad_res, *dz, *grad_bn_w, *grad_bn_b, *colsum;
    const float *ds_head, *w_head, *x_top; float *dw_head;
    int vpx;
} geom_deform_bwd;
#define GEOM_DEFORM_CHAIN_MAX 13
int geom_deform_chain_fits(int nv);
int geom_deform_chain_fwd_f32(int count, const geom_deform_fwd *layers, int *done, void *stream);
int geom_deform_chain_bwd_f32(int count, const geom_deform_bwd *layers, int *done, float *ds_first, void *stream);
int geom_deform_pack_weights_zero_f32(int count, const float *const *w, float *fwd, float *bwd, int *zero, int zero_words,
                                      void *stream);
typedef struct geom_deform_infer {
    int b, nv, c, k, ell_w;
    const float *s_in, *bias;
    const int *ell_col; const float *ell_val;
    const int *tail_col; const float *tail_val;
    const float *bn_w, *bn_b;
    const float *run_mean, *run_var;
    float eps;
    int relu;
    const float *res; int res_ld; float scale;
    float *x_out;
    const float *w_next; float *s_out;
    const float *w_head; float *s_head;
} geom_deform_infer;
int geom_deform_infer_fwd_f32(const geom_deform_infer *args, void *stream);
int geom_split_bf16_kpad(int k);
int geom_split_bf16_planes_f32(int k, int n, const float *w, uint16_t *planes, void *stream);
int geom_gemm_split_bf16_f32(int m, int k, int n, const float *a, const uint16_t *planes, float *c, int terms, void *stream);
int geom_dense_dx_split_cinpad(int cin);
int geom_dense_dx_split_planes_f32(int cin, int c, const float *w, uint16_t *planes, void *stream);
int geom_dense_dx_split_f32(int rows, int cin, int c, const float *g, const uint16_t *planes, float *dx, int ldx, void *stream);

int64_t geom_stage_regularisers_blocks(int b, int nv, int nf);
int geom_stage_regularisers_fwd_f32(int b, int nv, const float *prev, int prev_batched, const float *cur, int nf,
                                    const int64_t *faces, const int *rowptr, const int *col, const float *inv_deg,
                                    float c_lap, float c_move, float c_edge, float *lapd, float *partial, void *stream);
int geom_stage_regularisers_bwd_f32(int b, int nv, const float *prev, int prev_batched, const float *cur, int nf,
                                    const int64_t *faces, const int *rowptr, const int *col, const float *inv_deg,
                                    const int *vf_ptr, const int *vf_item, float c_lap, float c_move, float c_edge,
                                    const float *lapd, const float *gout, float *grad_prev, float *grad_cur, void *stream);

#define GEOM_SUM_MAX_TENSORS 8
int geom_sum_tensors_f32(int count, const float *const *tensors, int64_t n, float *out, void *stream);
int geom_sum_tensors_rows_f32(int count, const float *const *tensors, const int64_t *lds, int64_t rows, int width, float *out,
                              void *stream);

int geom_camera_info_f32(int b, const float *param, float *cam_mat, float *cam_pos, void *stream);

#define GEOM_DEFORM_MAX_PACK 16
#define GEOM_DEFORM_TAIL 32
int geom_deform_pack_weights_f32(int count, const float *const *w, float *fwd, float *bwd, void *stream);
int geom_deform_layer_fwd_f32(const geom_deform_fwd *args, void *stream);
int geom_deform_layer_bwd_f32(const geom_deform_bwd *args, void *stream);
#define GEOM_DEFORM_WIDE_MAX_B 64
int geom_deform_layer_wide_fwd_f32(const geom_deform_fwd *args, void *stream);
int geom_deform_layer_wide_bwd_f32(const geom_deform_bwd *args, void *stream);

int64_t geom_gemm_workspace_floats(int m, int n, int k);
int geom_gemm_f32(int m, int n, int k, const float *a, int64_t lda, int a_km, const float *b, int64_t ldb, int b_kn,
                  float *c, int64_t ldc, float *workspace, int64_t workspace_floats, void *stream);

int geom_vertex_head_fwd_f32(int64_t rows, int c, const float *base, const float *feat, float scale,
                             float *pos, void *stream);
int geom_vertex_head_bwd_f32(int64_t rows, int c, const float *grad_pos, float scale, float *grad_feat,
                             void *stream);

int geom_laplacian_f32(int b, int nv, const int *rowptr, const int *col, const float *inv_deg,
                       const float *x, int transpose, float *out, void *stream);
int geom_edge_sqlen_fwd_f32(int b, int nv, const float *verts, int nf, const int64_t *faces,
                            float *per_face, void *stream);
int geom_edge_sqlen_bwd_f32(int b, int nv, const float *verts, int nf, const int64_t *faces,
                            const float *coef_dev, float coef_host, float *grad_verts, void *stream);

int geom_vertex_bn_fwd_f32(int b, int nv, int c, const float *x, const float *weight, const float *bias,
                           float *running_mean, float *running_var, int training, float momentum, float eps,
                           int relu, const float *residual, int residual_ld, float scale,
                           float *out, float *save_mean, float *save_invstd, void *stream);
int geom_vertex_bn_bwd_f32(int b, int nv, int c, const float *x, const float *grad_out, const float *weight,
                           const float *bias, const float *save_mean, const float *save_invstd, int relu,
                           int has_residual, float scale, float *grad_x, float *grad_residual,
                           float *grad_weight, float *grad_bias, const float *grad_out2, void *stream);

size_t geom_pool_features_bwd_workspace_bytes(int b, int nv, int levels, const int *dims);
#define GEOM_POOL_MAX_LEVELS 8
int geom_pool_features_fwd_ld_f32(int b, int nv, const float *verts, const float *cam_mat, const float *cam_pos, int levels,
                                  const float *const *blocks, const int *channels, const int *dims, float *out, int64_t out_ld,
                                  void *stream);
int geom_pool_features_fwd_fronts_f32(int b, int nv, const float *verts, const float *cam_mat, const float *cam_pos, int levels,
                                      const float *const *blocks, const int *channels, const int *dims, float *out,
                                      int64_t out_ld, int n_fronts, const float *const *fronts, const int *widths,
                                      const int *cols, float *buf, void *stream);
int geom_pool_features_bwd_ld_f32(int b, int nv, const float *verts, const float *cam_mat, const float *cam_pos, int levels,
                                  const float *const *blocks, const int *channels, const int *dims, const float *grad_out,
                                  int64_t grad_ld, float *const *grad_blocks, float *grad_verts, void *workspace,
                                  size_t workspace_bytes, void *stream);

typedef struct geom_surface_cull {
    const int *gt_order;
    const float *gt_index;
    float *sample_index;
    const int *faces_in_order;
} geom_surface_cull;
int64_t geom_nn_cull_index_floats(int b, int n);
int geom_nn_cull_index_f32(int b, int n, const float *xyz, const int *order, float *index, void *stream);

int geom_surface_prepare_f32(int b, int nv, const float *verts, int nf, const int64_t *faces, int num,
                             uint64_t *rng_state, int64_t *choices, float *u, float *v, float *points, int n_gt,
                             const int *tri_order, unsigned flags, void *workspace, size_t workspace_bytes,
                             int *prepared, const geom_surface_cull *cull, void *stream);

size_t geom_surface_tail_counters_offset(int b, int n_gt, int nf);
typedef struct geom_surface_tail {
    const int64_t *choices;
    float scale_sample, scale_other;
    int want_order;
    float *loss;
    int finalized;
} geom_surface_tail;
int geom_surface_scan_f32(int b, int n_gt, const float *gt, int num, const float *points, float *sq_gt, int *idx_p,
                          float *sq_pred, int *idx_g, int nv, const float *verts, int nf, const int64_t *faces,
                          const int *tri_order, float *tri_dist, int *option, int *index, float *sq, float *closest,
                          float *weights, const float *u, const float *v, float coef_sample, float coef_other,
                          int *order_scratch, unsigned flags, void *workspace, size_t workspace_bytes,
                          int *records_written, const geom_surface_cull *cull, geom_surface_tail *tail, void *stream);

int64_t geom_surface_order_words(int b, int nf, int num, int n_gt);
int geom_surface_finalize_f32(int b, int nf, int num, const int64_t *choices, const float *u, const float *v,
                              const float *points, int n_gt, const float *gt, const int *idx_g, const int *idx_p,
                              const int *index, const float *closest, const float *weights, const float *sq_sample,
                              const float *sq_other, float scale_sample, float scale_other, float coef_sample,
                              float coef_other, int want_order, int records_ready, int *order, float *loss,
                              void *stream);
int geom_surface_gather_f32(int b, int nv, int nf, const int *vf_ptr, const int *vf_item, int num, int n_gt,
                            int has_other, const int *order, const float *grad, float *grad_verts, void *stream);
int geom_surface_finalize_w_f32(int b, int nf, int num, const int64_t *choices, const float *u, const float *v,
                                const float *points, int n_gt, const float *gt, const int *idx_g, const int *idx_p,
                                const int *index, const float *closest, const float *weights, const float *sq_sample,
                                const float *sq_other, float scale_sample, float scale_other, float coef_sample,
                                float coef_other, int want_order, int records_ready, int *order, float *loss,
                                const float *mesh_weight, void *stream);
int geom_surface_gather_w_f32(int b, int nv, int nf, const int *vf_ptr, const int *vf_item, int num, int n_gt,
                              int has_other, const int *order, const float *grad, const float *mesh_weight,
                              float *grad_verts, void *stream);

int64_t geom_segment_max_workspace_bytes(int nseg, int c, int64_t max_len);
int geom_segment_max_fwd_f32(int nseg, const int64_t *offsets, int64_t max_len, int c, const float *x,
                             float *out, int *arg, void *workspace, int64_t workspace_bytes, void *stream);
int geom_segment_max_bwd_f32(int nseg, const int64_t *offsets, int64_t total_rows, int c,
                             const float *grad_out, const int *arg, float *grad_x, void *stream);

int geom_encoder_layer_fwd_f32(int b, int nv, int c, int k, int n, const int *rowptr, const int *col, const float *val,
                               const float *s, int64_t lds, const float *bias, int act, const float *w, int64_t ldw,
                               float *out, int64_t ldo, float *x_out, int64_t ldx, void *stream);
int geom_encoder_layer_bwd_f32(int b, int nv, int c, int k, int n, const int *rowptrT, const int *colT, const float *valT,
                               const float *g, int64_t ldg, const float *x_saved, int64_t ldx, int act, const float *w,
                               int64_t ldw, float *out, int64_t ldo, float *t_out, int64_t ldt, void *stream);
int geom_latent_l1_fwd_f32(int b, int l, const float *pred, const float *target, const float *on, float weight, float *loss,
                           void *stream);
int geom_latent_l1_bwd_f32(int b, int l, const float *pred, const float *target, const float *on, float weight,
                           const float *grad_loss, float *grad_pred, void *stream);

#define GEOM_ADAM_MAX_TENSORS 64
#define GEOM_ADAM_STATE_WORDS 2112
int geom_adam_step_f32(int count, float *const *params, const float *const *grads, float *const *exp_avg,
                       float *const *exp_avg_sq, const int64_t *sizes, float lr, float beta1, float beta2,
                       float eps, float grad_scale, float *state, int advance, void *stream);
int64_t geom_adam_table_bytes(int count, int64_t total_blocks);
int geom_adam_table_step_f32(int count, const void *table, int64_t total_blocks, const float *lr, float beta1, float beta2,
                             float eps, float grad_scale, float *state, int advance, void *stream);

#ifdef __cplusplus
}
#endif
#endif
```

Baseline: 20390 meshes/s.

## Fold narrow head weight product into aggregation backward and shrink narrow workspace

```diff
diff --git a/geometrics_amd/aggregation.py b/geometrics_amd/aggregation.py
--- a/geometrics_amd/aggregation.py
+++ b/geometrics_amd/aggregation.py
@@ -55,10 +55,10 @@
                 and below.wt.dim() == 2 and below.wt.shape[0] == c and _fused.supported(csr, c, k, below.wt.shape[1]))
 
 
-def backward(g, csr, k, act, out, mask, want_bias, bias=None, arena=None, head=None, below=None):
-    grad_pos, scale, (b, nv, c) = head if head is not None else (None, 0.0, g.shape)
-    device = g.device if head is None else grad_pos.device
-    grad_support = _new_like(g, "grad_support", arena, descending=True) if head is None \
+def backward(g, csr, k, act, out, mask, want_bias, bias=None, arena=None, head=None, below=None, fold=None):
+    grad_pos, scale, (b, nv, c) = head if head is not None else (None, 0.0, fold[2] if fold is not None else g.shape)
+    device = grad_pos.device if head is not None else fold[0].device if fold is not None else g.device
+    grad_support = _new_like(g, "grad_support", arena, descending=True) if head is None and fold is None \
         else torch.empty(b, nv, c, dtype=torch.float32, device=device)
     rows = _fused.partial_rows(b, nv) if below is not None else None
     bg = _pass.NO_BIAS_GRADIENT
@@ -72,6 +72,10 @@
             _fused.layer_backward(g, out, mask, csr, k, act, below.wt, g_out=grad_support, grad_in=below.take_dx(b, nv),
                                   colsum_partial=bg.scratch, grad_pos=grad_pos, head_scale=scale, shape=(b, nv, c))
             below.stamp(grad_support)
+        elif fold is not None:
+            gs4, w = fold[:2]
+            _lib.call("geom_zn_gcn_aggregate_ell_fold_bwd_f32", b, nv, c, k, *_table(csr, True), gs4.data_ptr(), w.data_ptr(),
+                      w.stride(0), _lib.ptr(mask), act, *results)
         elif head is not None:
             _lib.call("geom_zn_gcn_aggregate_ell_head_bwd_f32", b, nv, c, k, *_table(csr, True), grad_pos.data_ptr(), scale,
                       _lib.ptr(mask), act, *results)
diff --git a/geometrics_amd/backward_pass.py b/geometrics_amd/backward_pass.py
--- a/geometrics_amd/backward_pass.py
+++ b/geometrics_amd/backward_pass.py
@@ -142,7 +142,7 @@
 
 
 _Colsum = namedtuple("_Colsum", "partials rows cols out stream param")
-_Reduce = namedtuple("_Reduce", "rows cin c workspace out stream param")
+_Reduce = namedtuple("_Reduce", "rows cin c workspace out stream param live", defaults=(0,))
 _Product = namedtuple("_Product", "x g out stream param launch_run")
 _Late = namedtuple("_Late", "launch out stream leaf")
 
@@ -221,13 +221,15 @@
 
 def _launch_reduces(jobs):
     for stream, group in _by_stream(jobs):
-        _dense_kernels.reduce([(j.rows, j.cin, j.c, j.workspace, j.out, None) for j in group], stream.cuda_stream)
+        _dense_kernels.reduce([(j.rows, j.cin, j.c, j.workspace, j.out, None, j.live) for j in group], stream.cuda_stream)
 
 
 def _launch_joint(reduces, colsums, stream):
     weights = (len(reduces), _ints([j.rows for j in reduces]), _ints([j.cin for j in reduces]), _ints([j.c for j in reduces]),
                _ptrs([j.workspace for j in reduces]), _ptrs([j.out for j in reduces]))
     biases = _colsum_args(colsums)
+    live = (_ints([j.live for j in reduces]),) if any(j.live for j in reduces) else ()
+    suffix = "_live_f32" if live else "_f32"
     opt = switches.optimizer
     slots = None
     if opt is not None:
@@ -237,17 +239,18 @@
             slots = None
     with torch.cuda.device(stream.device):
         if slots is None:
-            _lib.check(_lib.status("geom_dense_reduce2_f32", *weights, None, *biases, stream=stream.cuda_stream),
-                       "geom_dense_reduce2_f32")
+            _lib.check(_lib.status("geom_dense_reduce2" + suffix, *weights, None, *biases, *live, stream=stream.cuda_stream),
+                       "geom_dense_reduce2" + suffix)
         else:
             pick = lambda seq, ks: _ptrs([seq[k] for k in ks])
             wk, bk = slots[:len(reduces)], slots[len(reduces):]
             params = [p.data for p in opt.params]
             _lib.check(_lib.status(
-                "geom_dense_reduce_adam_f32",
+                "geom_dense_reduce_adam" + suffix,
                 *weights, pick(params, wk), pick(opt.exp_avg, wk), pick(opt.exp_avg_sq, wk),
                 *biases, pick(params, bk), pick(opt.exp_avg, bk), pick(opt.exp_avg_sq, bk), float(opt.lr), float(opt.betas[0]),
-                float(opt.betas[1]), float(opt.eps), opt.state.data_ptr(), stream=stream.cuda_stream), "geom_dense_reduce_adam_f32")
+                float(opt.betas[1]), float(opt.eps), opt.state.data_ptr(), *live, stream=stream.cuda_stream),
+                "geom_dense_reduce_adam" + suffix)
             opt._stepped_in_backward = True
 
 
@@ -308,14 +311,14 @@
     return BiasGradient(out, scratch, may_defer(bias, opted_in), bias)
 
 
-def weight_gradient(param_ref, w, rows, cin, c, workspace):
+def weight_gradient(param_ref, w, rows, cin, c, workspace, live=0):
     param = param_ref()
     out = _gradient_buffer(param, w)
     if may_defer(param):
         stream = torch.cuda.current_stream(w.device)
-        _current().reduces.append(_Reduce(rows, cin, c, workspace, _alias(out).view(cin, c), stream, param_ref))
+        _current().reduces.append(_Reduce(rows, cin, c, workspace, _alias(out).view(cin, c), stream, param_ref, live))
     else:
-        _dense_kernels.reduce([(rows, cin, c, workspace, out.view(cin, c), None)])
+        _dense_kernels.reduce([(rows, cin, c, workspace, out.view(cin, c), None, live)])
     return out
 
 
diff --git a/geometrics_amd/csrc/dense_gemm.hip b/geometrics_amd/csrc/dense_gemm.hip
--- a/geometrics_amd/csrc/dense_gemm.hip
+++ b/geometrics_amd/csrc/dense_gemm.hip
@@ -651,6 +651,7 @@
 constexpr int NP_RA = SPLIT_RB_NARROW * 16;
 constexpr int NP_CHUNK = 128;
 constexpr int NP_DX_ROWS = 64;
+constexpr int NP_LIVE = 4;
 struct NarrowPairArgs {
     const float *x;
     const float *g4;
@@ -673,7 +674,7 @@
     const int t_begin = (int)((int64_t)n4 * split / q.s_full) * 4;
     const int t_end = min((int)((int64_t)n4 * (split + 1) / q.s_full) * 4, q.rows);
     const int nch = (t_end - t_begin + NP_CHUNK - 1) / NP_CHUNK;
-    float *dst = q.part + (int64_t)slot * NP_RA * NP_CW;
+    float *dst = q.part + (int64_t)slot * NP_RA * NP_LIVE;
 
     f32x4 xr[XP], gr = {0.f, 0.f, 0.f, 0.f};
     auto load = [&](int ch) {
@@ -687,8 +688,6 @@
         if (tid < NP_CHUNK) gr = *reinterpret_cast<const f32x4 *>(q.g4 + (int64_t)min(t0 + tid, q.rows - 1) * 4);
     };
     if (nch > 0) load(0);
-    for (int e = tid; e < NP_RA * (NP_CW / 4); e += DG_THREADS)
-        if (e % (NP_CW / 4) != 0) *reinterpret_cast<f32x4 *>(dst + (int64_t)e * 4) = (f32x4){0.f, 0.f, 0.f, 0.f};
     float a0 = 0.f, a1 = 0.f, a2 = 0.f;
     for (int ch = 0; ch < nch; ++ch) {
         const int buf = ch & 1;
@@ -712,7 +711,7 @@
             }
         }
     }
-    if (tid < NP_RA) *reinterpret_cast<f32x4 *>(dst + (int64_t)tid * NP_CW) = (f32x4){a0, a1, a2, 0.f};
+    if (tid < NP_RA) *reinterpret_cast<f32x4 *>(dst + (int64_t)tid * NP_LIVE) = (f32x4){a0, a1, a2, 0.f};
 }
 
 __device__ __forceinline__ void narrow_dx_role(const NarrowPairArgs &q, const int w)
@@ -763,6 +762,7 @@
     float *out;
     int I, J, RA, CW, full_tiles, s_full, s_left;
     int outs;
+    int live;
 };
 struct ReduceJobs {
     ReduceJob job[GEOM_DENSE_MAX_REDUCE_JOBS];
@@ -801,6 +801,8 @@
     int i = 0, j = 0;
     if (live) {
         i = e / jq, j = (e % jq) * 4;
+    }
+    if (live && !(q.live && j >= q.live)) {
         int tile = i / q.RA, il = i % q.RA;
         const bool full = tile < q.full_tiles;
         const int n = full ? q.s_full : q.s_left;
@@ -1017,6 +1019,13 @@
     if (rows <= 0 || cin <= 0 || c <= 0 || c > 192) return 0;
     const SplitGeo g = split_geometry(cin, rows, num_cus());
     return g.partial_floats() + (int64_t)(g.s_full > 0 ? g.s_full : g.s_left) * c;
+}
+
+extern "C" int64_t geom_dense_bwd_narrow_workspace_floats(int rows, int cin, int c)
+{
+    if (rows <= 0 || cin != NP_CW || c != NP_CW) return 0;
+    const SplitGeo g = split_geometry(cin, rows, num_cus());
+    return (int64_t)g.slots * NP_RA * NP_LIVE;
 }
 
 extern "C" int geom_dense_bwd_weight_f32(int rows, int cin, int c, const float *x, const float *g, float *workspace,
@@ -1098,7 +1107,7 @@
 
 int build_reduce_jobs(ReduceJobs &jobs, int count, const int *rows, const int *cin, const int *c, const float *const *workspaces,
                       float *const *grad_w, int ncs, const float *const *cs_partials, const int *cs_rows, const int *cs_cols,
-                      float *const *cs_outs)
+                      float *const *cs_outs, const int *live = nullptr)
 {
     if (count < 0 || ncs < 0) return GEOM_EINVAL;
     if (count && (!rows || !cin || !c || !workspaces || !grad_w)) return GEOM_EINVAL;
@@ -1108,11 +1117,13 @@
     for (int l = 0; l < count; ++l) {
         if (bad_layer(workspaces[l], grad_w[l], rows[l], cin[l], c[l])) return GEOM_EINVAL;
         const SplitGeo g = split_geometry(cin[l], rows[l], num_cus());
-        jobs.job[n++] = ReduceJob{workspaces[l], grad_w[l], cin[l], c[l], g.rb * 16, 192, g.full_tiles, g.s_full, g.s_left, 0};
+        const int lv = live ? live[l] : 0;
+        if (lv < 0 || lv % 4 || lv > c[l]) return GEOM_EINVAL;
+        jobs.job[n++] = ReduceJob{workspaces[l], grad_w[l], cin[l], c[l], g.rb * 16, lv ? lv : 192, g.full_tiles, g.s_full, g.s_left, 0, lv};
     }
     for (int i = 0; i < ncs; ++i) {
         if (!cs_partials[i] || !cs_outs[i] || cs_rows[i] < 0 || cs_cols[i] <= 0 || cs_cols[i] % 4) return GEOM_EINVAL;
-        jobs.job[n++] = ReduceJob{cs_partials[i], cs_outs[i], 1, cs_cols[i], 1, cs_cols[i], 1, cs_rows[i], 0, 0};
+        jobs.job[n++] = ReduceJob{cs_partials[i], cs_outs[i], 1, cs_cols[i], 1, cs_cols[i], 1, cs_rows[i], 0, 0, 0};
     }
     flat_grid(jobs, n);
     return 0;
@@ -1123,17 +1134,54 @@
     hipLaunchKernelGGL(dense_reduce_kernel, dim3(jobs.first[jobs.n]), dim3(RED_THREADS), 0, static_cast<hipStream_t>(stream), jobs, adam);
     return geom::launch_status();
 }
+}
+
+extern "C" int geom_dense_reduce2_live_f32(int count, const int *rows, const int *cin, const int *c, const float *const *workspaces,
+                                           float *const *grad_w, float *const *grad_bias, int ncs, const float *const *cs_partials,
+                                           const int *cs_rows, const int *cs_cols, float *const *cs_outs, const int *live, void *stream)
+{
+    if (grad_bias) return GEOM_EINVAL;
+    if (count + ncs == 0) return 0;
+    ReduceJobs jobs;
+    const int code = build_reduce_jobs(jobs, count, rows, cin, c, workspaces, grad_w, ncs, cs_partials, cs_rows, cs_cols, cs_outs, live);
+    return code ? code : launch_reduce(jobs, ReduceAdam{}, stream);
 }
 
 extern "C" int geom_dense_reduce2_f32(int count, const int *rows, const int *cin, const int *c, const float *const *workspaces,
                                       float *const *grad_w, float *const *grad_bias, int ncs, const float *const *cs_partials,
                                       const int *cs_rows, const int *cs_cols, float *const *cs_outs, void *stream)
 {
-    if (grad_bias) return GEOM_EINVAL;
-    if (count + ncs == 0) return 0;
+    return geom_dense_reduce2_live_f32(count, rows, cin, c, workspaces, grad_w, grad_bias, ncs, cs_partials, cs_rows, cs_cols, cs_outs,
+                                       nullptr, stream);
+}
+
+extern "C" int geom_dense_reduce_adam_live_f32(int count, const int *rows, const int *cin, const int *c,
+                                               const float *const *workspaces, float *const *grad_w, float *const *w_p,
+                                               float *const *w_m, float *const *w_v, int ncs, const float *const *cs_partials,
+                                               const int *cs_rows, const int *cs_cols, float *const *cs_outs, float *const *b_p,
+                                               float *const *b_m, float *const *b_v, float lr, float beta1, float beta2, float eps,
+                                               float *state, const int *live, void *stream)
+{
+    if (count + ncs == 0 || !state) return GEOM_EINVAL;
+    if ((count && (!w_p || !w_m || !w_v)) || (ncs && (!b_p || !b_m || !b_v))) return GEOM_EINVAL;
     ReduceJobs jobs;
-    const int code = build_reduce_jobs(jobs, count, rows, cin, c, workspaces, grad_w, ncs, cs_partials, cs_rows, cs_cols, cs_outs);
-    return code ? code : launch_reduce(jobs, ReduceAdam{}, stream);
+    const int code = build_reduce_jobs(jobs, count, rows, cin, c, workspaces, grad_w, ncs, cs_partials, cs_rows, cs_cols, cs_outs, live);
+    if (code) return code;
+    ReduceAdam adam{};
+    for (int l = 0; l < count; ++l) {
+        adam.p[l] = w_p[l], adam.m[l] = w_m[l], adam.v[l] = w_v[l];
+        if (w_p[l] && (!w_m[l] || !w_v[l])) return GEOM_EINVAL;
+    }
+    for (int i = 0; i < ncs; ++i) {
+        adam.p[count + i] = b_p[i], adam.m[count + i] = b_m[i], adam.v[count + i] = b_v[i];
+        if (b_p[i] && (!b_m[i] || !b_v[i])) return GEOM_EINVAL;
+    }
+    adam.lr = lr, adam.b1 = beta1, adam.b2 = beta2, adam.eps = eps, adam.state = state;
+    uintptr_t bits = 0;
+    for (int j = 0; j < jobs.n; ++j)
+        if (adam.p[j]) bits |= (uintptr_t)adam.p[j] | (uintptr_t)adam.m[j] | (uintptr_t)adam.v[j] | (uintptr_t)jobs.job[j].out;
+    adam.vec = (bits & 15) == 0;
+    return launch_reduce(jobs, adam, stream);
 }
 
 extern "C" int geom_dense_reduce_adam_f32(int count, const int *rows, const int *cin, const int *c,
@@ -1143,30 +1191,12 @@
                                           float *const *b_m, float *const *b_v, float lr, float beta1, float beta2, float eps,
                                           float *state, void *stream)
 {
-    if (count + ncs == 0 || !state) return GEOM_EINVAL;
-    if ((count && (!w_p || !w_m || !w_v)) || (ncs && (!b_p || !b_m || !b_v))) return GEOM_EINVAL;
-    ReduceJobs jobs;
-    const int code = build_reduce_jobs(jobs, count, rows, cin, c, workspaces, grad_w, ncs, cs_partials, cs_rows, cs_cols, cs_outs);
-    if (code) return code;
-    ReduceAdam adam{};
-    for (int l = 0; l < count; ++l) {
-        adam.p[l] = w_p[l], adam.m[l] = w_m[l], adam.v[l] = w_v[l];
-        if (w_p[l] && (!w_m[l] || !w_v[l])) return GEOM_EINVAL;
-    }
-    for (int i = 0; i < ncs; ++i) {
-        adam.p[count + i] = b_p[i], adam.m[count + i] = b_m[i], adam.v[count + i] = b_v[i];
-        if (b_p[i] && (!b_m[i] || !b_v[i])) return GEOM_EINVAL;
-    }
-    adam.lr = lr, adam.b1 = beta1, adam.b2 = beta2, adam.eps = eps, adam.state = state;
-    uintptr_t bits = 0;
-    for (int j = 0; j < jobs.n; ++j)
-        if (adam.p[j]) bits |= (uintptr_t)adam.p[j] | (uintptr_t)adam.m[j] | (uintptr_t)adam.v[j] | (uintptr_t)jobs.job[j].out;
-    adam.vec = (bits & 15) == 0;
-    return launch_reduce(jobs, adam, stream);
-}
-
-extern "C" int geom_dense_reduce_f32(int count, const int *rows, const int *cin, const int *c, const float *const *workspaces,
-                                     float *const *grad_w, float *const *grad_bias, void *stream)
+    return geom_dense_reduce_adam_live_f32(count, rows, cin, c, workspaces, grad_w, w_p, w_m, w_v, ncs, cs_partials, cs_rows, cs_cols,
+                                           cs_outs, b_p, b_m, b_v, lr, beta1, beta2, eps, state, nullptr, stream);
+}
+
+extern "C" int geom_dense_reduce_live_f32(int count, const int *rows, const int *cin, const int *c, const float *const *workspaces,
+                                          float *const *grad_w, float *const *grad_bias, const int *live, void *stream)
 {
     constexpr int MAX = GEOM_DENSE_MAX_REDUCE_JOBS / 2;
     if (count < 0 || count > MAX) return GEOM_ETOOBIG;
@@ -1178,12 +1208,19 @@
     for (int l = 0; l < count; ++l) {
         if (bad_layer(workspaces[l], grad_w[l], rows[l], cin[l], c[l])) return GEOM_EINVAL;
         if (!grad_bias || !grad_bias[l]) continue;
+        if (live && live[l]) return GEOM_EUNSUPPORTED;
         const SplitGeo g = split_geometry(cin[l], rows[l], num_cus());
         if (g.full_tiles == 0) return GEOM_EUNSUPPORTED;
         cs_partials[ncs] = workspaces[l] + g.colsum_offset(), cs_outs[ncs] = grad_bias[l];
         cs_rows[ncs] = g.s_full, cs_cols[ncs] = c[l], ++ncs;
     }
     ReduceJobs jobs;
-    const int code = build_reduce_jobs(jobs, count, rows, cin, c, workspaces, grad_w, ncs, cs_partials, cs_rows, cs_cols, cs_outs);
+    const int code = build_reduce_jobs(jobs, count, rows, cin, c, workspaces, grad_w, ncs, cs_partials, cs_rows, cs_cols, cs_outs, live);
     return code ? code : launch_reduce(jobs, ReduceAdam{}, stream);
 }
+
+extern "C" int geom_dense_reduce_f32(int count, const int *rows, const int *cin, const int *c, const float *const *workspaces,
+                                     float *const *grad_w, float *const *grad_bias, void *stream)
+{
+    return geom_dense_reduce_live_f32(count, rows, cin, c, workspaces, grad_w, grad_bias, nullptr, stream);
+}
diff --git a/geometrics_amd/csrc/zn_gcn.hip b/geometrics_amd/csrc/zn_gcn.hip
--- a/geometrics_amd/csrc/zn_gcn.hip
+++ b/geometrics_amd/csrc/zn_gcn.hip
@@ -144,11 +144,23 @@
     int c;
 };
 
-template <int VEC_, int ACT_, bool BACKWARD_, bool MASK_ = false, bool HEAD_ = false>
+struct FoldSource {
+    Source s;
+    const float *gs4;
+    float fw[4][3];
+};
+
+__device__ __forceinline__ float fold_dx(const float4 &g, float w0, float w1, float w2)
+{
+    return __builtin_fmaf(g.z, w2, __builtin_fmaf(g.y, w1, __builtin_fmaf(g.x, w0, 0.f)));
+}
+
+template <int VEC_, int ACT_, bool BACKWARD_, bool MASK_ = false, bool HEAD_ = false, bool FOLD_ = false>
 struct TermKind {
-    static_assert((!MASK_ && !HEAD_) || VEC_ == 4, "sign mask and head are the fast kernel's");
+    static_assert((!MASK_ && !HEAD_ && !FOLD_) || VEC_ == 4, "sign mask, head and fold are the fast kernel's");
+    static_assert(!FOLD_ || (BACKWARD_ && !HEAD_), "the fold is a backward operand, and the head synthesises its own");
     static constexpr int VEC = VEC_, ACT = ACT_;
-    static constexpr bool BACKWARD = BACKWARD_, MASK = MASK_, HEAD = HEAD_;
+    static constexpr bool BACKWARD = BACKWARD_, MASK = MASK_, HEAD = HEAD_, FOLD = FOLD_;
 };
 
 template <class KIND, int VEC>
@@ -166,6 +178,16 @@
     }
     if (KIND::BACKWARD && KIND::MASK) bits = s.mask[row * s.kg + s.j];
     else if (KIND::BACKWARD && KIND::ACT != ACT_NONE) out.load(s.saved + row * s.c + col);
+}
+
+template <class KIND, int VEC>
+__device__ __forceinline__ void term_load(Pack<VEC> &v, Pack<VEC> &, unsigned &bits, const FoldSource &f, int64_t row, int)
+{
+    static_assert(KIND::FOLD, "a FoldSource is the FOLD backward's");
+    const float4 g = *reinterpret_cast<const float4 *>(f.gs4 + row * 4);
+#pragma unroll
+    for (int i = 0; i < VEC; ++i) v.at(i) = fold_dx(g, f.fw[i][0], f.fw[i][1], f.fw[i][2]);
+    if (KIND::MASK) bits = f.s.mask[row * f.s.kg + f.s.j];
 }
 
 template <class KIND, int VEC>
@@ -226,8 +248,8 @@
     }
 }
 
-template <class KIND, int W, int VEC>
-__device__ __forceinline__ void load_table_slots(Pack<VEC> (&sv)[W], Pack<VEC> (&ov)[W], unsigned (&bits)[W], const Source &s,
+template <class KIND, int W, int VEC, class SRC>
+__device__ __forceinline__ void load_table_slots(Pack<VEC> (&sv)[W], Pack<VEC> (&ov)[W], unsigned (&bits)[W], const SRC &s,
                                                  const int (&nb)[W], int64_t mesh_row0, int r, int c0)
 {
 #pragma unroll
@@ -425,14 +447,18 @@
     const float *head_in;
     float *head_out;
     float head_scale;
+    const float *fold_gs4, *fold_w;
+    int fold_pitch;
 };
 
-template <int ACT, bool BACKWARD, int W, int NC, bool MASK = false, bool HEAD = false>
+template <int ACT, bool BACKWARD, int W, int NC, bool MASK = false, bool HEAD = false, bool FOLD = false>
 __global__ __launch_bounds__(GCN_THREADS) void zn_aggregate_ell_kernel(EllArgs a, int rows_per_block, int iters,
                                                                         float *colsum_partial)
 {
     static_assert(!MASK || (ACT == ACT_RELU && NC == 2), "the sign mask is the ReLU / split-3 fast path");
+    static_assert(!FOLD || (BACKWARD && NC == 2 && !HEAD), "the fold is the split-3 backward's");
     extern __shared__ float lds_cs[];
+    float *const lds_sums = FOLD ? lds_cs + 4 * a.c : lds_cs;
     const int kg = a.k >> 2;
     const int j = threadIdx.x % kg;
     const int rl = threadIdx.x / kg;
@@ -440,8 +466,21 @@
     if (!geom::xcd_assign(blockIdx.x, a.b, a.chunks, mesh_i, chunk_i)) return;
     const int64_t mesh_row0 = (int64_t)mesh_i * a.nv;
     const int c0 = 4 * j;
-    using KIND = TermKind<4, ACT, BACKWARD, MASK, HEAD>;
-    const Source src{.x = a.x, .saved = a.saved, .mask = a.mask, .kg = kg, .j = j, .head = a.head_in, .head_scale = a.head_scale, .c = a.c};
+    using KIND = TermKind<4, ACT, BACKWARD, MASK, HEAD, FOLD>;
+    const Source plain{.x = a.x, .saved = a.saved, .mask = a.mask, .kg = kg, .j = j, .head = a.head_in, .head_scale = a.head_scale, .c = a.c};
+    std::conditional_t<FOLD, FoldSource, const Source &> src{plain};
+    const float4 *const fold_lds = reinterpret_cast<const float4 *>(lds_cs);
+    if constexpr (FOLD) {
+        src.gs4 = a.fold_gs4;
+        float4 *wl = reinterpret_cast<float4 *>(lds_cs);
+        for (int i = threadIdx.x; i < a.c; i += GCN_THREADS) wl[i] = *reinterpret_cast<const float4 *>(a.fold_w + (size_t)i * a.fold_pitch);
+        __syncthreads();
+#pragma unroll
+        for (int e = 0; e < 4; ++e) {
+            const float4 t = fold_lds[c0 + e];
+            src.fw[e][0] = t.x, src.fw[e][1] = t.y, src.fw[e][2] = t.z;
+        }
+    }
     float4 csum[NC + 1];
 #pragma unroll
     for (int i = 0; i <= NC; ++i) csum[i] = make_float4(0.f, 0.f, 0.f, 0.f);
@@ -464,8 +503,19 @@
         if (a.over_ptr) e0 = a.over_ptr[r], e1 = a.over_ptr[r + 1];
         unsigned own_bits = 0u;
         if (BACKWARD && MASK) own_bits = a.mask[row * kg + j];
+        float4 fold_g = make_float4(0.f, 0.f, 0.f, 0.f);
+        if (FOLD) fold_g = *reinterpret_cast<const float4 *>(a.fold_gs4 + row * 4);
 #pragma unroll
         for (int i = BACKWARD ? 0 : 1; i <= NC; ++i) {
+            if (FOLD) {
+                float o[4];
+#pragma unroll
+                for (int e = 0; e < 4; ++e) {
+                    const float4 t = fold_lds[c0 + a.k * i + e];
+                    o[e] = fold_dx(fold_g, t.x, t.y, t.z);
+                }
+                own[i] = make_float4(o[0], o[1], o[2], o[3]);
+            } else
             if (BACKWARD && HEAD) {
                 if (i == 0 && j == 0) {
                     const float *gp = a.head_in + row * 3;
@@ -556,12 +606,12 @@
         if (rl < rows_per_block) {
 #pragma unroll
             for (int i = 0; i <= NC; ++i)
-                *reinterpret_cast<float4 *>(lds_cs + rl * a.c + c0 + a.k * i) = csum[i];
+                *reinterpret_cast<float4 *>(lds_sums + rl * a.c + c0 + a.k * i) = csum[i];
         }
         __syncthreads();
         for (int c = threadIdx.x; c < a.c; c += GCN_THREADS) {
             float t = 0.f;
-            for (int l = 0; l < rows_per_block; ++l) t += lds_cs[l * a.c + c];
+            for (int l = 0; l < rows_per_block; ++l) t += lds_sums[l * a.c + c];
             colsum_partial[((size_t)mesh_i * a.chunks + chunk_i) * a.c + c] = t;
         }
     }
@@ -668,8 +718,12 @@
     const EllRoute route = ell_route(a.c, a.k, w);
     const bool fast = route == ELL_FAST3 || route == ELL_FAST10;
     if (route == ELL_NONE || (!fast && (a.head_in || a.mask))) return GEOM_EUNSUPPORTED;
+    if (a.fold_gs4 && (!BACKWARD || route != ELL_FAST3 || a.head_in || !((act == ACT_RELU && a.mask) || act == ACT_NONE)))
+        return GEOM_EUNSUPPORTED;
     if (b == 0 || a.nv == 0) return 0;
-    if (!a.col || !a.val || !a.y || (!a.x && !(BACKWARD && a.head_in))) return GEOM_EINVAL;
+    if (!a.col || !a.val || !a.y || (!a.x && !(BACKWARD && (a.head_in || a.fold_gs4)))) return GEOM_EINVAL;
+    if (a.fold_gs4 && (!a.fold_w || a.fold_pitch < 4 || a.fold_pitch % 4 != 0 || (((uintptr_t)a.fold_gs4 | (uintptr_t)a.fold_w) % 16) != 0))
+        return GEOM_EINVAL;
     if (a.head_in && (route != ELL_FAST3 || !((act == ACT_RELU && a.mask) || act == ACT_NONE) || (!BACKWARD && !a.head_out)))
         return GEOM_EUNSUPPORTED;
     if (a.mask && !(act == ACT_RELU && route == ELL_FAST3)) return GEOM_EINVAL;
@@ -692,7 +746,7 @@
         return known ? finish_launch(BACKWARD, geo.blocks, a.c, partial, grad_bias, s) : GEOM_EINVAL;
     }
     const EllGeometry geo = ell_geometry(b, a.nv, a.k, BACKWARD);
-    const size_t lds = (BACKWARD && partial) ? (size_t)geo.rows_per_block * a.c * sizeof(float) : 0;
+    const size_t lds = ((BACKWARD && partial) ? (size_t)geo.rows_per_block * a.c * sizeof(float) : 0) + (a.fold_gs4 ? (size_t)a.c * sizeof(float4) : 0);
     a.b = b, a.chunks = geo.chunks;
     const dim3 grid(geom::xcd_grid(b, geo.chunks));
     const bool known = with_act(act, [&](auto ACT) { with_width(w, [&](auto W) {
@@ -701,6 +755,13 @@
             hipLaunchKernelGGL((zn_aggregate_ell_kernel<A, BACKWARD, decltype(W)::value, decltype(NC)::value, decltype(MASK)::value, decltype(HEAD)::value>),
                                grid, dim3(GCN_THREADS), lds, s, a, geo.rows_per_block, geo.iters, partial);
         };
+        if constexpr (BACKWARD && (A == ACT_RELU || A == ACT_NONE)) {
+            if (a.fold_gs4) {
+                hipLaunchKernelGGL((zn_aggregate_ell_kernel<A, true, decltype(W)::value, 2, A == ACT_RELU, false, true>), grid, dim3(GCN_THREADS), lds, s, a, geo.rows_per_block,
+                                   geo.iters, partial);
+                return;
+            }
+        }
         if constexpr (A == ACT_RELU) {
             if (a.head_in) return go(Const<2>{}, std::true_type{}, std::true_type{});
             if (a.mask) return go(Const<2>{}, std::true_type{}, std::false_type{});
@@ -944,6 +1005,19 @@
     return dispatch_ell<true>(a, b, w, act, grad_bias, scratch, stream);
 }
 
+extern "C" int geom_zn_gcn_aggregate_ell_fold_bwd_f32(int b, int nv, int c, int k, int w, const int *ell_colT,
+                                                      const float *ell_valT, const int *over_ptrT, const int *over_colT,
+                                                      const float *over_valT, const float *grad_support4, const float *weight,
+                                                      int weight_pitch, const uint16_t *relu_mask, int act, float *grad_support,
+                                                      float *grad_bias, float *scratch, void *stream)
+{
+    if (!grad_support4 || !weight) return GEOM_EINVAL;
+    EllArgs a{.col = ell_colT, .val = ell_valT, .y = grad_support, .nv = nv, .c = c, .k = k, .mask = const_cast<uint16_t *>(relu_mask),
+              .over_ptr = over_ptrT, .over_col = over_colT, .over_val = over_valT, .fold_gs4 = grad_support4, .fold_w = weight,
+              .fold_pitch = weight_pitch};
+    return dispatch_ell<true>(a, b, w, act, grad_bias, scratch, stream);
+}
+
 extern "C" int geom_zn_gcn_aggregate_ell_head_bwd_f32(int b, int nv, int c, int k, int w, const int *ell_colT,
                                                       const float *ell_valT, const int *over_ptrT, const int *over_colT,
                                                       const float *over_valT, const float *grad_pos, float scale,
diff --git a/geometrics_amd/dense.py b/geometrics_amd/dense.py
--- a/geometrics_amd/dense.py
+++ b/geometrics_amd/dense.py
@@ -132,6 +132,14 @@
                   workspace.data_ptr(), 1 if want_colsum else 0)
 
 
+NARROW_LIVE = 4
+
+
+def narrow_weight_workspace(rows, cin, c, device):
+    n = int(_lib.lib().geom_dense_bwd_narrow_workspace_floats(rows, cin, c))
+    return torch.empty(n, dtype=torch.float32, device=device)
+
+
 def backward_narrow(x, g4, w, grad_x, workspace):
     rows, cin = x.shape
     with torch.cuda.device(x.device):
@@ -150,7 +158,12 @@
     ints = lambda k: (ctypes.c_int * n)(*[j[k] for j in jobs])
     ptrs = lambda k: (ctypes.c_void_p * n)(*[None if j[k] is None else j[k].data_ptr() for j in jobs])
     dev = jobs[0][3].device
+    live = [j[6] if len(j) > 6 else 0 for j in jobs]
     with torch.cuda.device(dev):
+        if any(live):
+            _lib.check(_lib.status("geom_dense_reduce_live_f32", n, ints(0), ints(1), ints(2), ptrs(3), ptrs(4), ptrs(5),
+                                   (ctypes.c_int * n)(*live), stream=stream), "geom_dense_reduce_live_f32")
+            return
         _lib.check(_lib.status("geom_dense_reduce_f32", n, ints(0), ints(1), ints(2), ptrs(3), ptrs(4), ptrs(5), stream=stream),
                    "geom_dense_reduce_f32")
 
diff --git a/geometrics_amd/layers.py b/geometrics_amd/layers.py
--- a/geometrics_amd/layers.py
+++ b/geometrics_amd/layers.py
@@ -338,12 +338,93 @@
             gs4, grad_bias = _agg.narrow_head_backward(gp, ctx.scale, sign, ctx.csr, ctx.k, ctx.act, (b, nv, c), need_b,
                                                        ctx.bias_ref() if need_b else None)
         if need_x or need_w:
-            ws = _products._dense_kernels.weight_workspace(rows, cin, c, x.device)
+            ws = _products._dense_kernels.narrow_weight_workspace(rows, cin, c, x.device)
             dx = torch.empty_like(x) if need_x else None
             _products._dense_kernels.backward_narrow(x.view(rows, cin), gs4, w.reshape(w.shape[-2:]), None if dx is None else dx.view(rows, cin), ws)
             if need_w:
-                grad_w = _pass.weight_gradient(ctx.w_ref, w, rows, cin, c, ws)
+                grad_w = _pass.weight_gradient(ctx.w_ref, w, rows, cin, c, ws, live=_products._dense_kernels.NARROW_LIVE)
         return dx, grad_w, grad_bias, (gp if need_base else None), None, None, None, None
+
+
+narrow_fold = None
+
+
+def _narrow_fold_mode():
+    mode = narrow_fold if narrow_fold is not None else (os.environ.get("GEOM_NARROW_FOLD") or None)
+    if mode not in (None, "on", "off"):
+        raise ValueError("GEOM_NARROW_FOLD / layers.narrow_fold must be 'on' or 'off' (got %r)" % (mode,))
+    return mode
+
+
+def _narrow_fold_takes(s, prev, layer, adj, activation, base):
+    if _narrow_fold_mode() == "off" or not (torch.is_tensor(s) and s.dim() == 3 and s.is_contiguous()):
+        return False
+    if not _narrow_head_takes(s, layer, adj, activation, base):
+        return False
+    bias = prev.bias
+    if bias is not None and not (torch.is_tensor(bias) and bias.is_cuda and bias.dtype == torch.float32 and bias.is_contiguous()
+                                 and bias.device == s.device and bias.shape == (s.shape[-1],)):
+        return False
+    k = _split_k(s, prev)
+    return prev.split == 3 and k > 0 and k % 4 == 0 and s.shape[-1] == 3 * k and (k >> 2) <= 256
+
+
+class _NarrowFold(torch.autograd.Function):
+
+    @staticmethod
+    def forward(ctx, support, bias, w, bias_head, base, csr, act, scale, forward_kind):
+        s = _lib.require(support, "support", torch.float32, 3)
+        if s.shape[1] != csr.nv:
+            raise RuntimeError("support has %d vertices but the adjacency has %d" % (s.shape[1], csr.nv))
+        bias_c = None if bias is None else _lib.require(bias, "bias", torch.float32, 1)
+        k = s.shape[-1] // 3
+        h = torch.empty_like(s)
+        mask = _agg.forward(s, bias_c, csr, k, act, h, want_mask=any(ctx.needs_input_grad[:4]))
+        w2 = w.reshape(w.shape[-2:])
+        x, s_head = _products._forward(forward_kind, h, w2)
+        pos = torch.empty_like(base)
+        k_head = s_head.shape[-1] // 3
+        sign = _agg.narrow_head_forward(s_head, bias_head, csr, k_head, act, base, scale, pos, want_sign=any(ctx.needs_input_grad[:4]))
+        ctx.csr, ctx.k, ctx.k_head, ctx.act, ctx.scale = csr, k, k_head, act, float(scale)
+        ctx.bias_ref = _pass.parameter_ref(bias, ctx, ctx.needs_input_grad[1])
+        ctx.w_ref = _pass.parameter_ref(w, ctx, ctx.needs_input_grad[2])
+        ctx.bias_head_ref = _pass.parameter_ref(bias_head, ctx, ctx.needs_input_grad[3])
+        ctx.has = (mask is not None, sign is not None)
+        ctx.save_for_backward(x, w, *[t for t in (mask, sign) if t is not None])
+        return pos
+
+    @staticmethod
+    def backward(ctx, grad_pos):
+        gp = grad_pos.contiguous()
+        x, w = ctx.saved_tensors[:2]
+        rest = list(ctx.saved_tensors[2:])
+        mask = rest.pop(0) if ctx.has[0] else None
+        sign = rest.pop(0) if ctx.has[1] else None
+        need_s, need_b, need_w, need_bh, need_base = ctx.needs_input_grad[:5]
+        need_b = need_b and ctx.bias_ref is not None
+        need_bh = need_bh and ctx.bias_head_ref is not None
+        b, nv, cin = x.shape
+        rows, c = b * nv, w.shape[-1]
+        w2 = w.reshape(w.shape[-2:])
+        grad_s = grad_b = grad_w = grad_bh = None
+        if need_s or need_b or need_w or need_bh:
+            gs4, grad_bh = _agg.narrow_head_backward(gp, ctx.scale, sign, ctx.csr, ctx.k_head, ctx.act, (b, nv, c), need_bh,
+                                                     ctx.bias_head_ref() if need_bh else None)
+        if need_w:
+            ws = _products._dense_kernels.narrow_weight_workspace(rows, cin, c, x.device)
+            _products._dense_kernels.backward_narrow(x.view(rows, cin), gs4, w2, None, ws)
+            grad_w = _pass.weight_gradient(ctx.w_ref, w, rows, cin, c, ws, live=_products._dense_kernels.NARROW_LIVE)
+        if need_s or need_b:
+            grad_s, grad_b = _agg.backward(None, ctx.csr, ctx.k, ctx.act, None, mask, need_b, ctx.bias_ref() if need_b else None,
+                                           fold=(gs4, w2, (b, nv, cin)))
+        return (grad_s if need_s else None), grad_b, grad_w, grad_bh, (gp if need_base else None), None, None, None, None
+
+
+def _narrow_fold_positions(s, prev, layer, adj, activation, base, scale):
+    act, _, _, csr = _route(activation, s, adj)
+    rows = s.shape[0] * s.shape[1]
+    r = _products.route(rows, 192, 192, True, True, True, False, _products._own_products_preferred(), _products.use_any_shape_products)
+    return _NarrowFold.apply(s, prev.bias, layer._weight(), layer.bias, base, csr, act, scale, r.forward)
 
 
 def _narrow_head_positions(h, layer, adj, activation, base, scale):
@@ -378,6 +459,8 @@
             s = _FusedBoundary.apply(s, prev.bias, layer._weight(), csr, _split_k(s, prev), act, up, link)
             link = up
         else:
+            if layer is stack[-1] and base is not None and csr is not None and _narrow_fold_takes(s, prev, layer, adj, activation, base):
+                return s, None, "fold"
             h = zero_n_aggregate(s, adj, prev.bias, _split_k(s, prev), activation)
             if layer is stack[-1] and base is not None and _narrow_head_takes(h, layer, adj, activation, base):
                 return h, None, True
@@ -397,6 +480,8 @@
 
 def zero_n_stack_positions(x, adj, stack, activation, base, scale):
     s, link, narrow = _stack_walk(x, adj, stack, activation, base)
+    if narrow == "fold":
+        return _narrow_fold_positions(s, stack[-2], stack[-1], adj, activation, base, scale)
     if narrow:
         return _narrow_head_positions(s, stack[-1], adj, activation, base, scale)
     return zero_n_aggregate_head(s, adj, stack[-1].bias, _split_k(s, stack[-1]), activation, base, scale, down=link)
diff --git a/include/geom_hip.h b/include/geom_hip.h
--- a/include/geom_hip.h
+++ b/include/geom_hip.h
@@ -140,6 +140,17 @@
                                float eps, float *state, void *stream);
 int geom_dense_reduce_f32(int count, const int *rows, const int *cin, const int *c, const float *const *workspaces,
                           float *const *grad_w, float *const *grad_bias, void *stream);
+int64_t geom_dense_bwd_narrow_workspace_floats(int rows, int cin, int c);
+int geom_dense_reduce_live_f32(int count, const int *rows, const int *cin, const int *c, const float *const *workspaces,
+                               float *const *grad_w, float *const *grad_bias, const int *live, void *stream);
+int geom_dense_reduce2_live_f32(int count, const int *rows, const int *cin, const int *c, const float *const *workspaces,
+                                float *const *grad_w, float *const *grad_bias, int ncs, const float *const *cs_partials,
+                                const int *cs_rows, const int *cs_cols, float *const *cs_outs, const int *live, void *stream);
+int geom_dense_reduce_adam_live_f32(int count, const int *rows, const int *cin, const int *c, const float *const *workspaces,
+                                    float *const *grad_w, float *const *w_p, float *const *w_m, float *const *w_v, int ncs,
+                                    const float *const *cs_partials, const int *cs_rows, const int *cs_cols, float *const *cs_outs,
+                                    float *const *b_p, float *const *b_m, float *const *b_v, float lr, float beta1, float beta2,
+                                    float eps, float *state, const int *live, void *stream);
 
 int geom_zn_gcn_aggregate_ell_head_fwd_f32(int b, int nv, int c, int k, int w, const int *ell_col,
                                            const float *ell_val, const int *over_ptr, const int *over_col,
@@ -160,6 +171,11 @@
                                     const int *over_ptrT, const int *over_colT, const float *over_valT,
                                     const float *grad_pos, float scale, const uint16_t *sign_words, int act,
                                     float *grad_support4, float *partials, void *stream);
+int geom_zn_gcn_aggregate_ell_fold_bwd_f32(int b, int nv, int c, int k, int w, const int *ell_colT,
+                                           const float *ell_valT, const int *over_ptrT, const int *over_colT,
+                                           const float *over_valT, const float *grad_support4, const float *weight,
+                                           int weight_pitch, const uint16_t *relu_mask, int act, float *grad_support,
+                                           float *grad_bias, float *scratch, void *stream);
 
 int64_t geom_zn_layer_partial_rows(int b, int nv);
 int geom_zn_layer_fwd_f32(int b, int nv, int c, int k, int ell_w, const int *ell_col, const float *ell_val,
```

Result: no change. 20510 meshes/s (median of 6 runs) (+0.6%).
